# Soltanilara/av-aloha

Measured on AMD Instinct MI355X. Metric: env-steps/sec (whole node) at 4096 parallel envs, SlotInsertion-3Arms, higher is better.
Workload: dtype f32

## Files before the change

av_aloha_amd/csrc/avsim_phys.hip.h:

```cpp
#pragma once
#include <hip/hip_runtime.h>

#include <cstddef>
#include <cstring>
#include <string>
#include <type_traits>
#include <vector>

#include "avsim_collide.hip.h"
#include "avsim_dev.h"
#include "avsim_math.hip.h"
#include "avsim_model.h"
#include "avsim_phys_layout.h"

namespace avs {

enum { J_FREE = 0, J_BALL = 1, J_SLIDE = 2, J_HINGE = 3 };
enum { R_EQ = 0, R_FLOSS = 1, R_LIMIT = 2, R_CONTACT = 3 };
constexpr int TREE_W = 8;
constexpr int ROW_W = 2 * TREE_W;
constexpr int ROW_S = ROW_W;
constexpr int CAND_MAX = 256;
constexpr int PROF_W = 26;
constexpr int NEAR_MAX = 512;

#define AVSIM_HEAD_INTS(X)                                                                                                              \
    X(nq) X(nv) X(nu) X(nbody) X(njnt) X(ngeom) X(npair) X(ntree) X(neq) X(nfloss) X(nlimited) X(nment) X(task_id) X(nj) X(msize)        \
    X(noslip_iters) X(noslip_trees) X(qcqp_tridiag) X(newton_early_exit) X(newton_component) X(noslip_per_tree) X(solver) X(newton_iters) \
    X(ls_iterations)
#define AVSIM_BODY_INTS(X) X(nobj) X(hull_ovf)
template <typename real>
struct DevHead {
    int nq, nv, nu, nbody, njnt, ngeom, npair, ntree, neq, nfloss, nlimited, nment, task_id, nj, msize;
    real timestep, gravity[3], impratio, grip_lo, grip_hi;
    int noslip_iters;
    int noslip_trees;
    int qcqp_tridiag;
    int newton_early_exit;
    int newton_component;
    int noslip_per_tree;
    int solver, newton_iters;
    real newton_tol, nscale;
    real ls_tolerance;
    int ls_iterations;
};
template <typename real, typename SPEC>
struct FixedHead {
    int pad_dims_[15];
    real timestep, gravity[3], impratio, grip_lo, grip_hi;
    int pad_flags_[8];
    real newton_tol, nscale;
    real ls_tolerance;
    int pad_tail_;
#define AVS_FIXED_INT(x) static constexpr int x = SPEC::x;
    AVSIM_HEAD_INTS(AVS_FIXED_INT)
#undef AVS_FIXED_INT
};
template <typename real, typename HEAD>
struct DevModelT : HEAD {
    GLB_PTR(const int) body_parent;
    GLB_PTR(const int) body_jntadr;
    GLB_PTR(const int) body_jntnum;
    GLB_PTR(const int) body_dofadr;
    GLB_PTR(const int) body_dofnum;
    GLB_PTR(const int) body_tree;
    GLB_PTR(const int) body_dofmask;
    GLB_PTR(const int) body_last;
    GLB_PTR(const real) body_pos;
    GLB_PTR(const real) body_quat;
    GLB_PTR(const real) body_mass;
    GLB_PTR(const real) body_ipos;
    GLB_PTR(const real) body_inertia;
    GLB_PTR(const real) body_invweight0;
    GLB_PTR(const real) static_xpos;
    GLB_PTR(const real) static_xmat;
    GLB_PTR(const int) tree_bodyadr;
    GLB_PTR(const int) tree_bodylist;
    GLB_PTR(const int) tree_dofadr;
    GLB_PTR(const int) tree_dofnum;
    GLB_PTR(const int) tree_madr;
    GLB_PTR(const int) jnt_type;
    GLB_PTR(const int) jnt_qposadr;
    GLB_PTR(const int) jnt_dofadr;
    GLB_PTR(const int) jnt_actfrclimited;
    GLB_PTR(const int) limited_jnt;
    GLB_PTR(const real) jnt_pos;
    GLB_PTR(const real) jnt_axis;
    GLB_PTR(const real) jnt_range;
    GLB_PTR(const real) jnt_actfrcrange;
    GLB_PTR(const real) jnt_solref;
    GLB_PTR(const real) jnt_solimp;
    GLB_PTR(const real) jnt_margin;
    GLB_PTR(const int) dof_body;
    GLB_PTR(const int) dof_parent;
    GLB_PTR(const int) dof_tree;
    GLB_PTR(const int) dof_jnt;
    GLB_PTR(const int) floss_dof;
    GLB_PTR(const int) ment_i;
    GLB_PTR(const int) ment_j;
    GLB_PTR(const real) dof_armature;
    GLB_PTR(const real) dof_damping;
    GLB_PTR(const real) dof_frictionloss;
    GLB_PTR(const real) dof_invweight0;
    GLB_PTR(const real) dof_solref;
    GLB_PTR(const real) dof_solimp;
    GLB_PTR(const int) act_dof;
    GLB_PTR(const int) act_qposadr;
    GLB_PTR(const int) act_ctrllimited;
    GLB_PTR(const real) act_kp;
    GLB_PTR(const real) act_kv;
    GLB_PTR(const real) act_gear;
    GLB_PTR(const real) act_ctrlrange;
    GLB_PTR(const int) eq_dof1;
    GLB_PTR(const int) eq_dof2;
    GLB_PTR(const int) eq_qpos1;
    GLB_PTR(const int) eq_qpos2;
    GLB_PTR(const real) eq_polycoef;
    GLB_PTR(const real) eq_solref;
    GLB_PTR(const real) eq_solimp;
    GLB_PTR(const real) qpos0;
    GLB_PTR(const real) qpos_home;
    int nobj;
    GLB_PTR(const int) obj_qadr;
    const double* obj_reset;
    GLB_PTR(const int) geom_type;
    GLB_PTR(const int) geom_body;
    GLB_PTR(const int) geom_hull;
    GLB_PTR(const int) geom_class;
    GLB_PTR(const int) geom_static;
    GLB_PTR(const real) geom_pos;
    GLB_PTR(const real) geom_mat;
    GLB_PTR(const real) geom_size;
    GLB_PTR(const real) geom_cpos;
    GLB_PTR(const real) geom_rbound;
    GLB_PTR(const real) geom_xpos0;
    GLB_PTR(const real) geom_xmat0;
    GLB_PTR(const real) geom_cen0;
    GLB_PTR(const real) geom_aabb0;
    GLB_PTR(const real) geom_lbox;
    GLB_PTR(const real) hull_vert;
    int hull_ovf;
    GLB_PTR(const int) pair_geom;
    GLB_PTR(const int) pair_condim;
    GLB_PTR(const real) pair_friction;
    GLB_PTR(const real) pair_solref;
    GLB_PTR(const real) pair_solimp;
    GLB_PTR(const real) pair_margin;
    GLB_PTR(const real) pair_gap;
    real* rJ_glob;
    real* rB_glob;
    real* gA_glob;
    int* near_glob;
    int* cand_glob;
    real* gref_glob;
    real* bxo_glob;
    GLB_PTR(const int) obs_qposadr;
    GLB_PTR(const real) obs_offset;
    GLB_PTR(const real) obs_scale;
};

template <typename real> using DevModel = DevModelT<real, DevHead<real>>;

static_assert(NARROW_SCR_W == 64 * SLOT_W + 4 * 56, "avsim_phys_layout.h: narrow-phase scratch");

template <typename real>
struct KArgs {
    DevModel<real> m;
    Layout lay;
    MOff mo;
};
template <typename real>
using KPtr = const KArgs<real> __attribute__((address_space(4)))*;

struct GenericSpec {};
template <typename SPEC> constexpr bool spec_fixed = !std::is_same<SPEC, GenericSpec>::value;
template <typename real, typename SPEC>
struct KFixed {
    using Model = DevModelT<real, FixedHead<real, SPEC>>;
    using FH = FixedHead<real, SPEC>;
    using DH = DevHead<real>;
    static_assert(sizeof(FH) == sizeof(DH) && alignof(FH) == alignof(DH) && sizeof(Model) == sizeof(DevModel<real>) && offsetof(FH, timestep) == offsetof(DH, timestep) &&
                      offsetof(FH, newton_tol) == offsetof(DH, newton_tol) && offsetof(FH, pad_tail_) == offsetof(DH, ls_iterations),
                  "FixedHead: the words of DevHead");
    KPtr<real> p;
    struct View {
        const Model __attribute__((address_space(4)))& m;
        static constexpr Layout lay = SPEC::lay;
        static constexpr MOff mo = SPEC::mo;
        AVS_DEV const View* operator->() const { return this; }
    };
    AVS_DEV KFixed(KPtr<real> p_) : p(p_) {}
    AVS_DEV explicit KFixed(unsigned long long v) : p((KPtr<real>)v) {}
    AVS_DEV explicit operator unsigned long long() const { return (unsigned long long)p; }
    AVS_DEV View operator->() const { return View{reinterpret_cast<const Model __attribute__((address_space(4)))&>(p->m)}; }
};
template <typename real, typename SPEC> struct KRefOf { using type = KFixed<real, SPEC>; };
template <typename real> struct KRefOf<real, GenericSpec> { using type = KPtr<real>; };
template <typename real, typename SPEC> using KRef = typename KRefOf<real, SPEC>::type;
#define PHASE_LAUNDER()                                                                                \
    do {                                                                                               \
        const unsigned long long p_ = (unsigned long long)ka;                                          \
        unsigned lo_ = __builtin_amdgcn_readfirstlane((unsigned)p_), hi_ = __builtin_amdgcn_readfirstlane((unsigned)(p_ >> 32)); \
        asm volatile("" : "+s"(lo_), "+s"(hi_));                                                       \
        ka = (decltype(ka))(((unsigned long long)hi_ << 32) | lo_);                                    \
    } while (0)
#if defined(__HIP_DEVICE_COMPILE__)
#define AVS_ASSUME_LDS(p) __builtin_assume(__builtin_amdgcn_is_shared((const void*)(p)))
#else
#define AVS_ASSUME_LDS(p) ((void)(p))
#endif
template <typename T>
AVS_DEV T* lds_at(unsigned byte_off) { return (T*)(__attribute__((address_space(3))) T*)(size_t)byte_off; }
#define LDS_BASES()                                                                       \
    real* const r = this->r; AVS_ASSUME_LDS(r);     \
    int* const ii = this->ii; AVS_ASSUME_LDS(ii);   \
    (void)r; (void)ii
#define PHASE_BEGIN() PHASE_LAUNDER(); LDS_BASES()



#ifndef AVS_SYNC_SCOPE
#define AVS_SYNC_SCOPE "workgroup"
#endif
#define GSYNC()                                              \
    do {                                                     \
        __builtin_amdgcn_fence(__ATOMIC_ACQ_REL, AVS_SYNC_SCOPE); \
        __builtin_amdgcn_wave_barrier();                     \
    } while (0)

AVS_DEV float row16_sum(float x) {
    asm volatile("" : "+v"(x));
    x += __builtin_bit_cast(float, __builtin_amdgcn_mov_dpp(__builtin_bit_cast(int, x), 0x128, 0xf, 0xf, true));
    x += __builtin_bit_cast(float, __builtin_amdgcn_mov_dpp(__builtin_bit_cast(int, x), 0x124, 0xf, 0xf, true));
    x += __builtin_bit_cast(float, __builtin_amdgcn_mov_dpp(__builtin_bit_cast(int, x), 0x122, 0xf, 0xf, true));
    x += __builtin_bit_cast(float, __builtin_amdgcn_mov_dpp(__builtin_bit_cast(int, x), 0x121, 0xf, 0xf, true));
    return x;
}
AVS_DEV double row16_sum(double x) {
    x += __shfl_xor(x, 8, 16);
    x += __shfl_xor(x, 4, 16);
    x += __shfl_xor(x, 2, 16);
    x += __shfl_xor(x, 1, 16);
    return x;
}

AVS_DEV float wave_sum(float x) {
    x = row16_sum(x);
    int xi = __builtin_bit_cast(int, x);
    x += __builtin_bit_cast(float, __builtin_amdgcn_update_dpp(0, xi, 0x142, 0xa, 0xf, false));
    xi = __builtin_bit_cast(int, x);
    x += __builtin_bit_cast(float, __builtin_amdgcn_update_dpp(0, xi, 0x143, 0xc, 0xf, false));
    return __builtin_bit_cast(float, __builtin_amdgcn_readlane(__builtin_bit_cast(int, x), 63));
}
AVS_DEV double wave_sum(double x) {
    for (int o = 32; o > 0; o >>= 1) x += __shfl_xor(x, o, 64);
    return x;
}

#define LDS_PTR(T) __attribute__((address_space(3))) T*

template <typename real>
struct RowS {
    real aref, R, inv, invn, lo, hi, f, muinv;
};

AVS_DEV float oct_sum(float x) {
    asm volatile("" : "+v"(x));
    x += __builtin_bit_cast(float, __builtin_amdgcn_mov_dpp(__builtin_bit_cast(int, x), 0xB1, 0xf, 0xf, true));
    x += __builtin_bit_cast(float, __builtin_amdgcn_mov_dpp(__builtin_bit_cast(int, x), 0x4E, 0xf, 0xf, true));
    x += __builtin_bit_cast(float, __builtin_amdgcn_mov_dpp(__builtin_bit_cast(int, x), 0x141, 0xf, 0xf, true));
    return x;
}
AVS_DEV double oct_sum(double x) {
    x += __shfl_xor(x, 1, 8);
    x += __shfl_xor(x, 2, 8);
    x += __shfl_xor(x, 4, 8);
    return x;
}
template <int J>
AVS_DEV int oct_bcast_i(int x) {
    constexpr int q = J & 3, ctrl = q | (q << 2) | (q << 4) | (q << 6);
    const int a = __builtin_amdgcn_mov_dpp(x, ctrl, 0xf, 0xf, true);
    const int b = __builtin_amdgcn_mov_dpp(a, 0x141, 0xf, 0xf, true);
    const bool hi = (threadIdx.x & 4) != 0;
    return hi == (J >= 4) ? a : b;
}
template <int J> AVS_DEV float oct_bcast(float x) { return __builtin_bit_cast(float, oct_bcast_i<J>(__builtin_bit_cast(int, x))); }
template <int J> AVS_DEV double oct_bcast(double x) {
    const long long b = __builtin_bit_cast(long long, x);
    const unsigned lo = (unsigned)oct_bcast_i<J>((int)(unsigned)b), hi = (unsigned)oct_bcast_i<J>((int)(unsigned)(b >> 32));
    return __builtin_bit_cast(double, ((long long)hi << 32) | (long long)lo);
}
template <typename T>
AVS_DEV T oct_bcast_n(T x, int j) {
    switch (j & 7) {
        case 0: return oct_bcast<0>(x); case 1: return oct_bcast<1>(x); case 2: return oct_bcast<2>(x); case 3: return oct_bcast<3>(x);
        case 4: return oct_bcast<4>(x); case 5: return oct_bcast<5>(x); case 6: return oct_bcast<6>(x); default: return oct_bcast<7>(x);
    }
}
AVS_DEV float lane_get(float x, int l) { return __builtin_bit_cast(float, __builtin_amdgcn_readlane(__builtin_bit_cast(int, x), l)); }
AVS_DEV double lane_get(double x, int l) {
    const long long b = __builtin_bit_cast(long long, x);
    const unsigned lo = (unsigned)__builtin_amdgcn_readlane((int)(unsigned)b, l), hi = (unsigned)__builtin_amdgcn_readlane((int)(unsigned)(b >> 32), l);
    return __builtin_bit_cast(double, ((long long)hi << 32) | (long long)lo);
}

constexpr int GRP_MAX = 6;
constexpr int GA_W = 64, GA_Q = 16, GA_QW = 6;
template <typename T> AVS_DEV T qdiv(T t, T d, T dinv) { return sizeof(T) == 4 ? t * dinv : t / d; }
AVS_DEV float qrsqrt(float x) { return __builtin_amdgcn_rsqf(x); }
AVS_DEV double qrsqrt(double x) { return 1.0 / sqrt(x); }
template <typename T> struct QTol;
template <> struct QTol<double> { static constexpr double abs = 1e-10, rel = 0.0; };
template <> struct QTol<float> { static constexpr float abs = 1e-10f, rel = 2e-6f; };

template <bool B> struct BoolTag { static constexpr bool value = B; };

template <typename real>
struct NoslipLead {
    LDS_PTR(const real) Minv;
    LDS_PTR(const int) tadr;
    LDS_PTR(const int) tnum;
    LDS_PTR(const int) floss_dof;
    LDS_PTR(int) dmap;
    LDS_PTR(int) prof;
    int tridiag;
    int ntree, nv, neq, nfloss, nlg;
};

typedef int nl_v4 __attribute__((ext_vector_type(4)));
#define NL_PARAMS nl_v4 nl_a_, nl_v4 nl_b_, nl_v4 nl_c_
#define NL_ARGS(nl) nl_pack_a(nl), nl_pack_b(nl), nl_pack_c(nl)
#define NL_UNPACK(real) NoslipLead<real> nl = nl_unpack<real>(nl_a_, nl_b_, nl_c_)
template <typename real> AVS_DEV nl_v4 nl_pack_a(const NoslipLead<real>& n) {
    return nl_v4{(int)(__SIZE_TYPE__)n.Minv, (int)(__SIZE_TYPE__)n.tadr, (int)(__SIZE_TYPE__)n.tnum, (int)(__SIZE_TYPE__)n.floss_dof};
}
template <typename real> AVS_DEV nl_v4 nl_pack_b(const NoslipLead<real>& n) { return nl_v4{(int)(__SIZE_TYPE__)n.dmap, (int)(__SIZE_TYPE__)n.prof, n.tridiag, n.ntree}; }
template <typename real> AVS_DEV nl_v4 nl_pack_c(const NoslipLead<real>& n) { return nl_v4{n.nv, n.neq, n.nfloss, n.nlg}; }
template <typename real> AVS_DEV NoslipLead<real> nl_unpack(nl_v4 a, nl_v4 b, nl_v4 c) {
    NoslipLead<real> n;
    n.Minv = (LDS_PTR(const real))(__SIZE_TYPE__)(unsigned)a.x; n.tadr = (LDS_PTR(const int))(__SIZE_TYPE__)(unsigned)a.y; n.tnum = (LDS_PTR(const int))(__SIZE_TYPE__)(unsigned)a.z;
    n.floss_dof = (LDS_PTR(const int))(__SIZE_TYPE__)(unsigned)a.w; n.dmap = (LDS_PTR(int))(__SIZE_TYPE__)(unsigned)b.x; n.prof = (LDS_PTR(int))(__SIZE_TYPE__)(unsigned)b.y;
    n.tridiag = b.z; n.ntree = b.w; n.nv = c.x; n.neq = c.y; n.nfloss = c.z; n.nlg = c.w;
    return n;
}

template <typename T> AVS_DEV LDS_PTR(T) uni_lds(LDS_PTR(T) p) {
    return (LDS_PTR(T))(unsigned long long)(unsigned)__builtin_amdgcn_readfirstlane((int)(unsigned)(unsigned long long)p);
}
template <typename T> AVS_DEV GLB_PTR(T) uni_glb(GLB_PTR(T) p) {
    const unsigned long long v = (unsigned long long)p;
    return (GLB_PTR(T))(((unsigned long long)(unsigned)__builtin_amdgcn_readfirstlane((int)(unsigned)(v >> 32)) << 32) | (unsigned)__builtin_amdgcn_readfirstlane((int)(unsigned)v));
}

template <typename T> AVS_DEV T secular_step(T val, T r2, T r, T yw) {
    const T yy = val + r2, ny = sqrt(yy);
    return val * yy / ((ny + r) * r * yw);
}

template <typename real>
__device__ AVS_OUTLINE_2 void pgs_groups(LDS_PTR(real) rowS, LDS_PTR(const int) rowI, GLB_PTR(const real) rJ, GLB_PTR(const real) rB,
                                                     LDS_PTR(real) q, LDS_PTR(const int) gI, GLB_PTR(const real) gA, int ngrp, int iters,
                                                     int noslip_iters, real noslip_tol_scaled, NL_PARAMS) {
    NL_UNPACK(real);
    const long long tent = __builtin_readcyclecounter();
    rowS = uni_lds(rowS); rowI = uni_lds(rowI); q = uni_lds(q); gI = uni_lds(gI);
    rJ = uni_glb(rJ); rB = uni_glb(rB); gA = uni_glb(gA);
    ngrp = __builtin_amdgcn_readfirstlane(ngrp); iters = __builtin_amdgcn_readfirstlane(iters); noslip_iters = __builtin_amdgcn_readfirstlane(noslip_iters);
    noslip_tol_scaled = lane_get(noslip_tol_scaled, 0);
    nl.Minv = uni_lds(nl.Minv); nl.tadr = uni_lds(nl.tadr); nl.tnum = uni_lds(nl.tnum); nl.floss_dof = uni_lds(nl.floss_dof); nl.dmap = uni_lds(nl.dmap); nl.prof = uni_lds(nl.prof);
    nl.ntree = __builtin_amdgcn_readfirstlane(nl.ntree); nl.nv = __builtin_amdgcn_readfirstlane(nl.nv); nl.neq = __builtin_amdgcn_readfirstlane(nl.neq);
    nl.nfloss = __builtin_amdgcn_readfirstlane(nl.nfloss); nl.nlg = __builtin_amdgcn_readfirstlane(nl.nlg); nl.tridiag = __builtin_amdgcn_readfirstlane(nl.tridiag);
    const int lane = threadIdx.x & 63, d = lane >> 3, k8 = lane & 7, dr = d < GRP_MAX ? d : 0;
    const int lr = lane < GRP_MAX ? lane : 0;
    const int tri = lr * (lr - 1) / 2;
    if (ngrp <= 0) return;
    const bool fl = noslip_iters > 0 && nl.nlg >= 0;
    const int ft = lane >> 3, fi = lane & 7, fgb = lane & ~7;
    bool fm = false;
    int fdof = 0, frow = -1;
    real mrow[TREE_W], faref = 0, finv = 0, fdiag = 0, flo = 0, fhi = 0;
#pragma unroll
    for (int s = 0; s < TREE_W; s++) mrow[s] = 0;
    if (fl) {
        for (int k = lane; k < nl.nv; k += 64) nl.dmap[k] = -1;
        __builtin_amdgcn_fence(__ATOMIC_ACQ_REL, "wavefront");
        __builtin_amdgcn_wave_barrier();
        for (int r = lane; r < nl.nfloss; r += 64) nl.dmap[nl.floss_dof[r]] = nl.neq + r;
        __builtin_amdgcn_fence(__ATOMIC_ACQ_REL, "wavefront");
        __builtin_amdgcn_wave_barrier();
        fm = ft < nl.ntree && fi < nl.tnum[ft < nl.ntree ? ft : 0];
        fdof = fm ? nl.tadr[ft] + fi : 0;
        frow = fm ? nl.dmap[fdof] : -1;
        if (fm) {
#pragma unroll
            for (int s = 0; s < TREE_W; s++) mrow[s] = nl.Minv[64 * ft + 8 * fi + s];
        }
        LDS_PTR(const real) FS = rowS + RS_S * (frow >= 0 ? frow : 0);
        faref = FS[0]; finv = frow >= 0 ? FS[3] : real(0); flo = FS[4]; fhi = FS[5];
        fdiag = finv != 0 ? real(1) / finv : real(0);
    }
    real imp = 0, imp_c = 0;
#ifdef AVSIM_PROBE_ROWS
    LDS_PTR(int) prof = (LDS_PTR(int))nullptr;
#else
    LDS_PTR(int) prof = nl.prof;
#endif
    const long long tq0 = prof ? __builtin_readcyclecounter() : 0;
    int nstep = 0, nsweep = 0;
    auto floss_sweep = [&]() {
        const long long tf0 = prof ? __builtin_readcyclecounter() : 0;
        real x = fm ? q[fdof] : real(0);
        LDS_PTR(real) FS = rowS + RS_S * (frow >= 0 ? frow : 0);
        real f = frow >= 0 ? FS[6] : real(0);
#pragma unroll
        for (int s = 0; s < TREE_W; s++) {
            const real res = x - faref;
            const real fs = tmin(tmax(f - res * finv, flo), fhi);
            const real dl_ = fs - f, ch = dl_ * (real(0.5) * dl_ * fdiag + res);
            const bool take = frow >= 0 && fi == s && !(ch > real(1e-10));
            if (take) { imp -= ch; f = fs; }
            const real ds = oct_bcast_n(take ? dl_ : real(0), s);
            x += mrow[s] * ds;
        }
        if (fm) q[fdof] = x;
        if (frow >= 0) FS[6] = f;
        __builtin_amdgcn_fence(__ATOMIC_ACQ_REL, "wavefront");
        __builtin_amdgcn_wave_barrier();
        nsweep++;
    };
    const int first_ns = fl ? nl.nlg : 0;
    const int per_ns = ngrp - first_ns;
    const int noslip_only = (fl && per_ns <= 0) ? noslip_iters : 0;
    if (noslip_only) noslip_iters = 0;
    auto jb_load = [&](int hdr, int win, real& ja, real& jb, real& ba, real& bb) {
        const int st = hdr & 0xffff, cn = (hdr >> 16) & 15;
        const bool in = d < cn;
        const int rw = st + (in ? d : 0);
        const bool a = in && k8 < ((win >> 6) & 15), b = in && k8 < ((win >> 19) & 15);
        GLB_PTR(const real) Jr = rJ + ROW_S * rw + k8;
        GLB_PTR(const real) Br = rB + ROW_S * rw + k8;
        (void)a; (void)b;
        const bool packed = ((hdr >> 24) & 1) && ((__builtin_amdgcn_readfirstlane(win) >> 19) & 15) == 0;
        ja = Jr[0];
        const real x = Jr[TREE_W];
        if (packed) { jb = 0; ba = x; bb = 0; }
        else { jb = x; ba = Br[0]; bb = Br[TREE_W]; }
    };
    auto nextg = [&](int gq, int itq) { return gq + 1 < ngrp ? gq + 1 : (itq + 1 >= iters ? first_ns : 0); };
    int g = iters > 0 ? 0 : first_ns, it = 0;
    if (g >= ngrp) g = 0;
    int gi = __builtin_amdgcn_readfirstlane(gI[g]);
    int gin = __builtin_amdgcn_readfirstlane(gI[nextg(g, it)]);
    int ginn = __builtin_amdgcn_readfirstlane(gI[nextg(nextg(g, it), it)]);
    int ra = rowI[(gi & 0xffff) + dr], ran = rowI[(gin & 0xffff) + dr];
    real JA, JB, BA, BB;
    jb_load(gi, ra, JA, JB, BA, BB);
    real ac[GRP_MAX - 1];
#pragma unroll
    for (int s = 0; s < GRP_MAX - 1; s++) ac[s] = gA[GA_W * g + tri + s];
    const int qr = (lane >= 1 && lane <= 5) ? lane - 1 : 0;
    real qc[GA_QW], qn[GA_QW];
#pragma unroll
    for (int s = 0; s < GA_QW; s++) qc[s] = gA[GA_W * g + GA_Q + 8 * s + qr];
    const int total = iters * ngrp + noslip_iters * per_ns;
    __builtin_amdgcn_s_waitcnt(0x0f70);
    if (fl && iters == 0 && noslip_iters > 0) floss_sweep();
    for (int step = 0; step < total; step++) {
        nstep++;
        const bool noslip = it >= iters;
        const int start = gi & 0xffff, cnt = (gi >> 16) & 15;
        const bool contact = (gi >> 24) & 1;
        const int g1 = nextg(g, it), g2 = nextg(g1, it), g3 = nextg(g2, it);
        const int ginnn_v = gI[g3];
        const int rann = rowI[(ginn & 0xffff) + dr];
        real JAn, JBn, BAn, BBn;
        jb_load(gin, ran, JAn, JBn, BAn, BBn);
        const bool inr = d < cnt;
// ... 1117 lines not shown
            if (ab && !a_table) rw = 3;
            if (cd) rw = 4;
    }
    return rw;
}
#if !defined(AVSIM_TU_F64) && !defined(AVSIM_NO_F32_LAUNCH)
__global__ void k_reward_pairs(GLB_PTR(const int) geom_class, int ngeom, int task_id, const int* __restrict__ pairs, int n, int cap, int* __restrict__ latch, int* __restrict__ reward) {
    const int i = blockIdx.x * blockDim.x + threadIdx.x;
    if (i >= n) return;
    int f = 0;
    for (int c = 0; c < cap; c++) {
        const int g1 = pairs[((size_t)i * cap + c) * 2], g2 = pairs[((size_t)i * cap + c) * 2 + 1];
        if (g1 < 0 || g2 < 0 || g1 >= ngeom || g2 >= ngeom) continue;
        f |= reward_pair_flags(geom_class[g1], geom_class[g2], task_id);
    }
    int l = latch ? latch[i] : 0;
    reward[i] = reward_from_flags(f, task_id, &l);
    if (latch) latch[i] = l;
}
#endif


template <typename real, int G, typename SPEC = GenericSpec>
struct Env {
    KRef<real, SPEC> ka;
    int env = 0;
    int diverged = 0;
    int nit_sum = 0, nit_max = 0;
    bool profiling = false;
    real* r;
    int* ii;
    int lane, grp;
    const real* lr;
    const int* li;
    long long t_broad = 0, t_narrow = 0;
    __device__ Env(KRef<real, SPEC> ka_, real* r_, int* i_, int lane_, int grp_, const real* lr_, const int* li_)
        : ka(ka_), r(r_), ii(i_), lane(lane_), grp(grp_), lr(lr_), li(li_) {}
    AVS_DEV const int* LI() const {
        const int* p = li;
        if constexpr (spec_fixed<SPEC>) p = lds_at<const int>((unsigned)(ka->mo.nreal * sizeof(real)));
        AVS_ASSUME_LDS(p);
        return p;
    }
    AVS_DEV const real* LR() const {
        const real* p = lr;
        if constexpr (spec_fixed<SPEC>) p = lds_at<const real>(0u);
        AVS_ASSUME_LDS(p);
        return p;
    }
    AVS_DEV int nobj_() const { if constexpr (spec_fixed<SPEC>) return SPEC::nobj; else return ka->m.nobj; }
    AVS_DEV int hull_ovf_() const { if constexpr (spec_fixed<SPEC>) return SPEC::hull_ovf; else return ka->m.hull_ovf; }
    AVS_DEV GLB_PTR(real) rows_() const { return (GLB_PTR(real))ka->m.rJ_glob + (size_t)env * ka->lay.gefc * ROW_S; }
    AVS_DEV GLB_PTR(real) rowsB_() const { return (GLB_PTR(real))ka->m.rB_glob + (size_t)env * ka->lay.gefc * ROW_S; }
    AVS_DEV GLB_PTR(real) coup_() const { return (GLB_PTR(real))ka->m.gA_glob + (size_t)env * ka->lay.ggrp * GA_W; }
    AVS_DEV GLB_PTR(int) near_() const { return (GLB_PTR(int))ka->m.near_glob + (size_t)env * NEAR_MAX; }
    AVS_DEV GLB_PTR(int) cand_() const { return (GLB_PTR(int))ka->m.cand_glob + (size_t)env * CAND_MAX; }
    AVS_DEV GLB_PTR(real) bxo_() const { return (GLB_PTR(real))ka->m.bxo_glob + (size_t)env * 64 * BOX_OVF_W; }
    AVS_DEV GLB_PTR(real) gref_() const { return (GLB_PTR(real))ka->m.gref_glob + (size_t)env * ka->m.ngeom * 3; }
    AVS_DEV const int* body_parent_() const { return LI() + ka->mo.body_parent; }
    AVS_DEV const int* body_jntadr_() const { return LI() + ka->mo.body_jntadr; }
    AVS_DEV const int* body_jntnum_() const { return LI() + ka->mo.body_jntnum; }
    AVS_DEV const int* body_dofadr_() const { return LI() + ka->mo.body_dofadr; }
    AVS_DEV const int* body_dofnum_() const { return LI() + ka->mo.body_dofnum; }
    AVS_DEV const int* body_tree_() const { return LI() + ka->mo.body_tree; }
    AVS_DEV const int* body_dofmask_() const { return LI() + ka->mo.body_dofmask; }
    AVS_DEV const int* body_last_() const { return LI() + ka->mo.body_last; }
    AVS_DEV const int* tree_bodyadr_() const { return LI() + ka->mo.tree_bodyadr; }
    AVS_DEV const int* tree_bodylist_() const { return LI() + ka->mo.tree_bodylist; }
    AVS_DEV const int* tree_dofadr_() const { return LI() + ka->mo.tree_dofadr; }
    AVS_DEV const int* tree_dofnum_() const { return LI() + ka->mo.tree_dofnum; }
    AVS_DEV const int* tree_madr_() const { return LI() + ka->mo.tree_madr; }
    AVS_DEV const int* jnt_type_() const { return LI() + ka->mo.jnt_type; }
    AVS_DEV const int* jnt_qposadr_() const { return LI() + ka->mo.jnt_qposadr; }
    AVS_DEV const int* jnt_dofadr_() const { return LI() + ka->mo.jnt_dofadr; }
    AVS_DEV const int* jnt_actfrclimited_() const { return LI() + ka->mo.jnt_actfrclimited; }
    AVS_DEV const int* limited_jnt_() const { return LI() + ka->mo.limited_jnt; }
    AVS_DEV const int* dof_body_() const { return LI() + ka->mo.dof_body; }
    AVS_DEV const int* dof_parent_() const { return LI() + ka->mo.dof_parent; }
    AVS_DEV const int* dof_tree_() const { return LI() + ka->mo.dof_tree; }
    AVS_DEV const int* dof_jnt_() const { return LI() + ka->mo.dof_jnt; }
    AVS_DEV const int* floss_dof_() const { return LI() + ka->mo.floss_dof; }
    AVS_DEV const int* ment_i_() const { return LI() + ka->mo.ment_i; }
    AVS_DEV const int* ment_j_() const { return LI() + ka->mo.ment_j; }
    AVS_DEV const int* act_dof_() const { return LI() + ka->mo.act_dof; }
    AVS_DEV const int* act_qposadr_() const { return LI() + ka->mo.act_qposadr; }
    AVS_DEV const int* act_ctrllimited_() const { return LI() + ka->mo.act_ctrllimited; }
    AVS_DEV const int* geom_type_() const { return LI() + ka->mo.geom_type; }
    AVS_DEV const int* geom_body_() const { return LI() + ka->mo.geom_body; }
    AVS_DEV const int* geom_static_() const { return LI() + ka->mo.geom_static; }
    AVS_DEV const real* body_pos_() const { return LR() + ka->mo.body_pos; }
    AVS_DEV const real* body_quat_() const { return LR() + ka->mo.body_quat; }
    AVS_DEV const real* body_mass_() const { return LR() + ka->mo.body_mass; }
    AVS_DEV const real* body_ipos_() const { return LR() + ka->mo.body_ipos; }
    AVS_DEV const real* body_inertia_() const { return LR() + ka->mo.body_inertia; }
    AVS_DEV const real* body_invweight0_() const { return LR() + ka->mo.body_invweight0; }
    AVS_DEV const real* jnt_pos_() const { return LR() + ka->mo.jnt_pos; }
    AVS_DEV const real* jnt_axis_() const { return LR() + ka->mo.jnt_axis; }
    AVS_DEV const real* jnt_range_() const { return LR() + ka->mo.jnt_range; }
    AVS_DEV const real* jnt_actfrcrange_() const { return LR() + ka->mo.jnt_actfrcrange; }
    AVS_DEV const real* jnt_margin_() const { return LR() + ka->mo.jnt_margin; }
    AVS_DEV const real* dof_armature_() const { return LR() + ka->mo.dof_armature; }
    AVS_DEV const real* dof_damping_() const { return LR() + ka->mo.dof_damping; }
    AVS_DEV const real* dof_frictionloss_() const { return LR() + ka->mo.dof_frictionloss; }
    AVS_DEV const real* dof_invweight0_() const { return LR() + ka->mo.dof_invweight0; }
    AVS_DEV const real* act_kp_() const { return LR() + ka->mo.act_kp; }
    AVS_DEV const real* act_kv_() const { return LR() + ka->mo.act_kv; }
    AVS_DEV const real* act_gear_() const { return LR() + ka->mo.act_gear; }
    AVS_DEV const real* act_ctrlrange_() const { return LR() + ka->mo.act_ctrlrange; }
    AVS_DEV const real* geom_cpos_() const { return LR() + ka->mo.geom_cpos; }
    AVS_DEV const real* geom_rbound_() const { return LR() + ka->mo.geom_rbound; }


    __device__ void tree_chol(const real* A, real* Ldst, const real* diag_add, real diag_scale) {
        const int t = lane >> 3, i = lane & 7, gb = lane & ~7;
        const bool act = t < ka->m.ntree;
        const int n = act ? tree_dofnum_()[t] : 0, base = act ? tree_madr_()[t] : 0, a0 = act ? tree_dofadr_()[t] : 0;
        real row[TREE_W];
#pragma unroll
        for (int k = 0; k < TREE_W; k++) row[k] = (i < n && k <= i) ? A[base + i * n + k] : (k == i ? real(1) : real(0));
        if (diag_add && i < n) {
#pragma unroll
            for (int k = 0; k < TREE_W; k++) if (k == i) row[k] += diag_scale * diag_add[a0 + i];
        }
#pragma unroll
        for (int j = 0; j < TREE_W; j++) {
            const real d = sqrt(tmax(oct_bcast_n(row[j], j), real(1e-30)));
            const real lij = i == j ? d : row[j] / d;
            row[j] = lij;
            const real mul = i > j ? lij : real(0);
#pragma unroll
            for (int k = j + 1; k < TREE_W; k++) row[k] -= mul * oct_bcast_n(lij, k);
        }
        if (i < n) {
#pragma unroll
            for (int k = 0; k < TREE_W; k++) if (k <= i) Ldst[base + i * n + k] = row[k];
        }
    }
    __device__ real tree_solve(const real* L, real x) {
        const int t = lane >> 3, i = lane & 7, gb = lane & ~7;
        const bool act = t < ka->m.ntree;
        const int n = act ? tree_dofnum_()[t] : 0, base = act ? tree_madr_()[t] : 0;
        real row[TREE_W], col[TREE_W];
#pragma unroll
        for (int k = 0; k < TREE_W; k++) {
            row[k] = (i < n && k < i) ? L[base + i * n + k] : real(0);
            col[k] = (k < n && k > i) ? L[base + k * n + i] : real(0);
        }
        const real dinv = i < n ? real(1) / L[base + i * n + i] : real(1);
        if (!(i < n)) x = 0;
#pragma unroll
        for (int j = 0; j < TREE_W; j++) {
            const real yj = oct_bcast_n(x * dinv, j);
            x = i == j ? yj : x - row[j] * yj;
        }
#pragma unroll
        for (int j = TREE_W - 1; j >= 0; j--) {
            const real xj = oct_bcast_n(x * dinv, j);
            x = i == j ? xj : x - col[j] * xj;
        }
        return x;
    }

    __device__ void kinematics() {
        PHASE_BEGIN();
        real *xpos = r + ka->lay.xpos, *xmat = r + ka->lay.xmat, *xipos = r + ka->lay.xipos, *cdof = r + ka->lay.cdof, *qpos = r + ka->lay.qpos;
        int* anc = ii + ka->lay.cand;
        const int nb = ka->m.nbody;
        for (int b = lane; b < nb; b += G) {
            real R[9], pos[3];
            int a = -1;
            if (body_tree_()[b] < 0) {
                for (int k = 0; k < 3; k++) pos[k] = ka->m.static_xpos[3 * b + k];
                for (int k = 0; k < 9; k++) R[k] = ka->m.static_xmat[9 * b + k];
            } else {
                const int p = body_parent_()[b], ja = body_jntadr_()[b], jn = body_jntnum_()[b];
                const int jt = jn > 0 ? jnt_type_()[ja] : -1;
                if (jt == J_FREE) {
                    const int qa = jnt_qposadr_()[ja];
                    real quat[4];
                    for (int k = 0; k < 3; k++) pos[k] = qpos[qa + k];
                    for (int k = 0; k < 4; k++) quat[k] = qpos[qa + 3 + k];
                    quatnorm(quat);
                    quat2mat(quat, R);
                } else {
                    real Rl[9], bq[4] = {body_quat_()[4 * b], body_quat_()[4 * b + 1], body_quat_()[4 * b + 2], body_quat_()[4 * b + 3]};
                    quat2mat(bq, Rl);
                    for (int k = 0; k < 3; k++) pos[k] = body_pos_()[3 * b + k];
                    for (int k = 0; k < 9; k++) R[k] = Rl[k];
                    if (jt == J_HINGE) {
                        const real q = qpos[jnt_qposadr_()[ja]];
                        const real ax[3] = {jnt_axis_()[3 * ja], jnt_axis_()[3 * ja + 1], jnt_axis_()[3 * ja + 2]};
                        const real jp[3] = {jnt_pos_()[3 * ja], jnt_pos_()[3 * ja + 1], jnt_pos_()[3 * ja + 2]};
                        const real sn = sin(q), co = cos(q), oc = 1 - co;
                        const real Rq[9] = {co + ax[0] * ax[0] * oc, ax[0] * ax[1] * oc - ax[2] * sn, ax[0] * ax[2] * oc + ax[1] * sn,
                                            ax[1] * ax[0] * oc + ax[2] * sn, co + ax[1] * ax[1] * oc, ax[1] * ax[2] * oc - ax[0] * sn,
                                            ax[2] * ax[0] * oc - ax[1] * sn, ax[2] * ax[1] * oc + ax[0] * sn, co + ax[2] * ax[2] * oc};
                        for (int i = 0; i < 3; i++)
                            for (int j = 0; j < 3; j++) R[3 * i + j] = Rl[3 * i] * Rq[j] + Rl[3 * i + 1] * Rq[3 + j] + Rl[3 * i + 2] * Rq[6 + j];
                        real t0[3], t1[3];
                        mulmat(Rl, jp, t0);
                        mulmat(R, jp, t1);
                        for (int k = 0; k < 3; k++) pos[k] += t0[k] - t1[k];
                    } else if (jt == J_SLIDE) {
                        const real q = qpos[jnt_qposadr_()[ja]];
                        const real ax[3] = {jnt_axis_()[3 * ja], jnt_axis_()[3 * ja + 1], jnt_axis_()[3 * ja + 2]};
                        real t0[3];
                        mulmat(Rl, ax, t0);
                        for (int k = 0; k < 3; k++) pos[k] += t0[k] * q;
                    }
                    if (body_tree_()[p] < 0) {
                        GLB_PTR(const real) Rp = ka->m.static_xmat + 9 * p;
                        real Rn[9], t0[3];
                        for (int i = 0; i < 3; i++)
                            for (int j = 0; j < 3; j++) Rn[3 * i + j] = Rp[3 * i] * R[j] + Rp[3 * i + 1] * R[3 + j] + Rp[3 * i + 2] * R[6 + j];
                        mulmat(Rp, pos, t0);
                        for (int k = 0; k < 3; k++) pos[k] = ka->m.static_xpos[3 * p + k] + t0[k];
                        for (int k = 0; k < 9; k++) R[k] = Rn[k];
                    } else a = p;
                }
            }
            for (int k = 0; k < 3; k++) xpos[3 * b + k] = pos[k];
            for (int k = 0; k < 9; k++) xmat[9 * b + k] = R[k];
            anc[b] = a;
        }
        GSYNC();
        for (int round = 0; round < 6; round++) {
            bool any = false;
            real Ra[9], pa[3];
            int a = -1, aa = -1;
            const int b = lane;
            if (b < nb) {
                a = anc[b];
                if (a >= 0) {
                    any = true;
                    aa = anc[a];
                    for (int k = 0; k < 9; k++) Ra[k] = xmat[9 * a + k];
                    for (int k = 0; k < 3; k++) pa[k] = xpos[3 * a + k];
                }
            }
            if (!__any(any)) break;
            GSYNC();
            if (a >= 0) {
                real R[9], pos[3], Rn[9], t0[3];
                for (int k = 0; k < 9; k++) R[k] = xmat[9 * b + k];
                for (int k = 0; k < 3; k++) pos[k] = xpos[3 * b + k];
                for (int i = 0; i < 3; i++)
                    for (int j = 0; j < 3; j++) Rn[3 * i + j] = Ra[3 * i] * R[j] + Ra[3 * i + 1] * R[3 + j] + Ra[3 * i + 2] * R[6 + j];
                mulmat(Ra, pos, t0);
                for (int k = 0; k < 3; k++) xpos[3 * b + k] = pa[k] + t0[k];
                for (int k = 0; k < 9; k++) xmat[9 * b + k] = Rn[k];
                anc[b] = aa;
            }
            GSYNC();
        }
        for (int b = lane; b < nb; b += G) {
            real t3[3] = {0, 0, 0};
            if (body_tree_()[b] >= 0) {
                const real ip[3] = {body_ipos_()[3 * b], body_ipos_()[3 * b + 1], body_ipos_()[3 * b + 2]};
                mulmat(xmat + 9 * b, ip, t3);
                for (int k = 0; k < 3; k++) t3[k] += xpos[3 * b + k];
            }
            for (int k = 0; k < 3; k++) xipos[3 * b + k] = t3[k];
        }
        for (int d = lane; d < ka->m.nv; d += G) {
            const int j = dof_jnt_()[d], b = dof_body_()[d], jt = jnt_type_()[j], k = d - jnt_dofadr_()[j];
            const real *R = xmat + 9 * b, *pos = xpos + 3 * b;
            real cd[6] = {0, 0, 0, 0, 0, 0};
            if (jt == J_FREE) {
                if (k < 3) cd[3 + k] = 1;
                else {
                    const real w[3] = {R[k - 3], R[3 + k - 3], R[6 + k - 3]};
                    real c[3];
                    cross3(pos, w, c);
                    for (int q = 0; q < 3; q++) { cd[q] = w[q]; cd[3 + q] = c[q]; }
                }
            } else {
                const real ax[3] = {jnt_axis_()[3 * j], jnt_axis_()[3 * j + 1], jnt_axis_()[3 * j + 2]};
                real axis[3];
                mulmat(R, ax, axis);
                if (jt == J_HINGE) {
                    const real jp[3] = {jnt_pos_()[3 * j], jnt_pos_()[3 * j + 1], jnt_pos_()[3 * j + 2]};
                    real anchor[3], c[3];
                    mulmat(R, jp, anchor);
                    for (int q = 0; q < 3; q++) anchor[q] += pos[q];
                    cross3(anchor, axis, c);
                    for (int q = 0; q < 3; q++) { cd[q] = axis[q]; cd[3 + q] = c[q]; }
                } else {
                    for (int q = 0; q < 3; q++) cd[3 + q] = axis[q];
                }
            }
            for (int q = 0; q < 6; q++) cdof[6 * d + q] = cd[q];
        }
        real* gcen = r + ka->lay.gcen;
        for (int g = lane; g < ka->m.ngeom; g += G) {
            if (geom_static_()[g]) continue;
            int b = geom_body_()[g];
            real c[3] = {geom_cpos_()[3 * g], geom_cpos_()[3 * g + 1], geom_cpos_()[3 * g + 2]}, t3[3];
            mulmat(xmat + 9 * b, c, t3);
            for (int k = 0; k < 3; k++) gcen[3 * g + k] = xpos[3 * b + k] + t3[k];
        }
        GSYNC();
    }

    __device__ void crb() {
        PHASE_BEGIN();
        real *xmat = r + ka->lay.xmat, *xipos = r + ka->lay.xipos, *cdof = r + ka->lay.cdof, *ci = r + ka->lay.cinert, *M = r + ka->lay.M, *L = r + ka->lay.L;
        for (int b = lane; b < ka->m.nbody; b += G) {
            SInert<real> s;
            if (body_tree_()[b] >= 0) body_inertia(ka, xmat, xipos, b, s);
            else { s.m = 0; for (int k = 0; k < 3; k++) s.h[k] = 0; for (int k = 0; k < 6; k++) s.I[k] = 0; }
            real *o = ci + 10 * b, *ob = r + ka->lay.binert + 10 * b;
            o[0] = ob[0] = s.m;
            for (int k = 0; k < 3; k++) o[1 + k] = ob[1 + k] = s.h[k];
            for (int k = 0; k < 6; k++) o[4 + k] = ob[4 + k] = s.I[k];
        }
        for (int i = lane; i < ka->m.msize; i += G) M[i] = 0;
        GSYNC();
        {
            real acc[10];
            const int p = lane < ka->m.nbody ? lane : 0;
            const bool dyn = lane < ka->m.nbody && body_tree_()[p] >= 0;
            for (int k = 0; k < 10; k++) acc[k] = 0;
            if (dyn)
                for (int d = p; d <= body_last_()[p]; d++)
                    for (int k = 0; k < 10; k++) acc[k] += ci[10 * d + k];
            GSYNC();
            if (dyn)
                for (int k = 0; k < 10; k++) ci[10 * p + k] = acc[k];
        }
        GSYNC();
        for (int e = lane; e < ka->m.nment; e += G) {
            int i = ment_i_()[e], j = ment_j_()[e], t = dof_tree_()[i], n = tree_dofnum_()[t], a = tree_dofadr_()[t];
            real f[6];
            inert_mul(ci + 10 * dof_body_()[i], cdof + 6 * i, f);
            real v = 0;
            for (int k = 0; k < 6; k++) v += cdof[6 * j + k] * f[k];
            if (i == j) v += dof_armature_()[i];
            real* Mb = M + tree_madr_()[t];
            Mb[(i - a) * n + (j - a)] = v;
            Mb[(j - a) * n + (i - a)] = v;
        }
        GSYNC();
        tree_chol(M, L, (const real*)nullptr, real(0));
        GSYNC();
        real* Minv = r + ka->lay.Minv;
        for (int w = lane; w < ka->m.ntree * TREE_W; w += G) {
            int t = w >> 3, j = w & 7, n = tree_dofnum_()[t];
            real x[TREE_W];
            const real* Lt = L + tree_madr_()[t];
#pragma unroll
            for (int k = 0; k < TREE_W; k++) x[k] = (k == j && j < n) ? real(1) : real(0);
#pragma unroll
            for (int i = 0; i < TREE_W; i++)
                if (i < n) {
                    real sacc = x[i];
#pragma unroll
                    for (int k = 0; k < i; k++) sacc -= Lt[i * n + k] * x[k];
                    x[i] = sacc / Lt[i * n + i];
                }
#pragma unroll
            for (int i = TREE_W - 1; i >= 0; i--)
                if (i < n) {
                    real sacc = x[i];
#pragma unroll
                    for (int k = i + 1; k < TREE_W; k++) if (k < n) sacc -= Lt[k * n + i] * x[k];
                    x[i] = sacc / Lt[i * n + i];
                }
#pragma unroll
            for (int k = 0; k < TREE_W; k++) Minv[64 * t + 8 * k + j] = (k < n && j < n) ? x[k] : real(0);
        }
        GSYNC();
    }

    __device__ void rne_bias() {
        PHASE_BEGIN();
        real *xmat = r + ka->lay.xmat, *xipos = r + ka->lay.xipos, *cdof = r + ka->lay.cdof, *qvel = r + ka->lay.qvel;
        real *cvel = r + ka->lay.cvel, *cfrc = r + ka->lay.cfrc, *bias = r + ka->lay.bias;
        real* cdd = r + ka->lay.cinert;
        const int nb = ka->m.nbody;
        for (int b = lane; b < nb; b += G) {
            real v[6] = {0, 0, 0, 0, 0, 0};
            const int t = body_tree_()[b];
            if (t >= 0) {
                const int a0 = tree_dofadr_()[t], n = tree_dofnum_()[t], mask = body_dofmask_()[b];
#pragma unroll
                for (int k = 0; k < TREE_W; k++) {
                    const bool on = k < n && ((mask >> k) & 1);
                    const int d = on ? a0 + k : a0;
                    const real qd = on ? qvel[d] : real(0);
#pragma unroll
                    for (int q = 0; q < 6; q++) v[q] += cdof[6 * d + q] * qd;
                }
            }
            for (int q = 0; q < 6; q++) cvel[6 * b + q] = v[q];
        }
        GSYNC();
        for (int d = lane; d < ka->m.nv; d += G) {
            const int j = dof_jnt_()[d], b = dof_body_()[d];
            real o[6] = {0, 0, 0, 0, 0, 0};
            if (jnt_type_()[j] == J_FREE) {
                const int d0 = jnt_dofadr_()[j];
                if (d - d0 >= 3) {
                    real vt[6] = {0, 0, 0, 0, 0, 0};
                    for (int k = 0; k < 3; k++)
                        for (int q = 0; q < 6; q++) vt[q] += cdof[6 * (d0 + k) + q] * qvel[d0 + k];
                    cross_motion(vt, cdof + 6 * d, o);
                }
            } else {
                cross_motion(cvel + 6 * b, cdof + 6 * d, o);
            }
            const real qd = qvel[d];
            for (int q = 0; q < 6; q++) cdd[6 * d + q] = o[q] * qd;
        }
        GSYNC();
        for (int b = lane; b < nb; b += G) {
            const int t = body_tree_()[b];
            real f[6] = {0, 0, 0, 0, 0, 0};
            if (t >= 0) {
                real a[6] = {0, 0, 0, -ka->m.gravity[0], -ka->m.gravity[1], -ka->m.gravity[2]}, v[6];
                const int a0 = tree_dofadr_()[t], n = tree_dofnum_()[t], mask = body_dofmask_()[b];
#pragma unroll
                for (int k = 0; k < TREE_W; k++) {
                    const bool on = k < n && ((mask >> k) & 1);
                    const int d = on ? a0 + k : a0;
#pragma unroll
                    for (int q = 0; q < 6; q++) { const real c = cdd[6 * d + q]; a[q] += on ? c : real(0); }
                }
                for (int q = 0; q < 6; q++) v[q] = cvel[6 * b + q];
                real sv[10];
                for (int q = 0; q < 10; q++) sv[q] = (r + ka->lay.binert)[10 * b + q];
                real Ia[6], Iv[6], vIv[6];
                inert_mul(sv, a, Ia);
                inert_mul(sv, v, Iv);
                cross_force(v, Iv, vIv);
                for (int q = 0; q < 6; q++) f[q] = Ia[q] + vIv[q];
            }
            for (int q = 0; q < 6; q++) cfrc[6 * b + q] = f[q];
        }
        GSYNC();
        for (int i = lane; i < ka->m.nv; i += G) {
            const int b = dof_body_()[i];
            real f[6] = {0, 0, 0, 0, 0, 0};
            for (int d = b; d <= body_last_()[b]; d++)
                for (int q = 0; q < 6; q++) f[q] += cfrc[6 * d + q];
            real sacc = 0;
            for (int q = 0; q < 6; q++) sacc += cdof[6 * i + q] * f[q];
            bias[i] = sacc;
        }
        GSYNC();
    }

    __device__ void smooth() {
        PHASE_BEGIN();
        real *qpos = r + ka->lay.qpos, *qvel = r + ka->lay.qvel, *ctrl = r + ka->lay.ctrl, *bias = r + ka->lay.bias, *fsm = r + ka->lay.fsm, *as = r + ka->lay.asm_;
        real* act = r + ka->lay.fcon;
        for (int i = lane; i < ka->m.nv; i += G) act[i] = 0;
        GSYNC();
        for (int u = lane; u < ka->m.nu; u += G) {
            real c = ctrl[u];
            if (act_ctrllimited_()[u]) c = tclamp(c, act_ctrlrange_()[2 * u], act_ctrlrange_()[2 * u + 1]);
            int dof = act_dof_()[u];
            real f = act_kp_()[u] * c - act_kp_()[u] * qpos[act_qposadr_()[u]] - act_kv_()[u] * qvel[dof];
            act[dof] += act_gear_()[u] * f;
        }
        GSYNC();
        for (int i = lane; i < ka->m.nv; i += G) {
            int j = dof_jnt_()[i];
            real a = act[i];
            if (jnt_actfrclimited_()[j] && jnt_type_()[j] != J_FREE) a = tclamp(a, jnt_actfrcrange_()[2 * j], jnt_actfrcrange_()[2 * j + 1]);
            real f = -dof_damping_()[i] * qvel[i] - bias[i] + a;
            fsm[i] = f;
            as[i] = f;
        }
        GSYNC();
        {
            const int t = lane >> 3, i = lane & 7;
            const bool mine = t < ka->m.ntree && i < tree_dofnum_()[t];
            const int k = mine ? tree_dofadr_()[t] + i : 0;
            const real x = tree_solve(r + ka->lay.L, mine ? as[k] : real(0));
            GSYNC();
            if (mine) as[k] = x;
        }
        GSYNC();
    }

    __device__ void load_shape(int g, Shape<real>& s) {
        LDS_BASES();
        real *xpos = r + ka->lay.xpos, *xmat = r + ka->lay.xmat, *gcen = r + ka->lay.gcen;
        s.type = geom_type_()[g];
        for (int k = 0; k < 3; k++) s.size[k] = ka->m.geom_size[3 * g + k];
        s.hull = ka->m.hull_vert;
        s.hbase = ka->m.geom_hull[2 * g];
        s.hR = ka->m.geom_hull[2 * g + 1];
        s.hovf = hull_ovf_();
        s.nh = 0;
        for (int k = 0; k < 3; k++) { s.lc[k] = ka->m.geom_lbox[6 * g + k]; s.lh[k] = ka->m.geom_lbox[6 * g + 3 + k]; }
        if (geom_static_()[g]) {
            for (int k = 0; k < 3; k++) { s.pos[k] = ka->m.geom_xpos0[3 * g + k]; s.center[k] = ka->m.geom_cen0[3 * g + k]; }
            for (int k = 0; k < 9; k++) s.mat[k] = ka->m.geom_xmat0[9 * g + k];
        } else {
            int b = geom_body_()[g];
            real gp[3] = {ka->m.geom_pos[3 * g], ka->m.geom_pos[3 * g + 1], ka->m.geom_pos[3 * g + 2]}, t3[3];
            mulmat(xmat + 9 * b, gp, t3);
            for (int k = 0; k < 3; k++) { s.pos[k] = xpos[3 * b + k] + t3[k]; s.center[k] = gcen[3 * g + k]; }
            const real* Rb = xmat + 9 * b;
            GLB_PTR(const real) Rg = ka->m.geom_mat + 9 * g;
            for (int i = 0; i < 3; i++)
                for (int j = 0; j < 3; j++) s.mat[3 * i + j] = Rb[3 * i] * Rg[j] + Rb[3 * i + 1] * Rg[3 + j] + Rb[3 * i + 2] * Rg[6 + j];
        }
    }

    __device__ AVS_OUTLINE_0 static void multi_perturb(KRef<real, SPEC> ka_, real* r_, int* i_, int lane_, int grp_, const real* lr_, const int* li_, int env_,
                                                                   int pga, int pgb, int src, int pert) {
        Env e(ka_, r_, i_, lane_, grp_, lr_, li_);
        e.env = env_;
        LDS_PTR(real) os = (LDS_PTR(real))(e.r + e.ka->lay.scr + SLOT_W * src);
        const real p0[3] = {os[SLOT_P], os[SLOT_P + 1], os[SLOT_P + 2]}, n0[3] = {os[SLOT_N], os[SLOT_N + 1], os[SLOT_N + 2]};
        Shape<real> a, b;
        e.load_shape(pga, a);
        e.load_shape(pgb, b);
        real dk = real(1e30), pk[3] = {0, 0, 0};
        if (!mpr_perturbed(a, b, p0, n0, pert, &dk, pk)) dk = real(1e30);
        os[1 + pert] = dk;
        for (int c = 0; c < 3; c++) os[SLOT_P + 3 * (1 + pert) + c] = pk[c];
    }

    __device__ AVS_OUTLINE void collide() {
        Env e(*this);
        e.collide_i();
        diverged = e.diverged; nit_sum = e.nit_sum; nit_max = e.nit_max; t_broad = e.t_broad; t_narrow = e.t_narrow;
    }
    __device__ __attribute__((always_inline)) void collide_i() {
        PHASE_BEGIN();
        real* gcen = r + ka->lay.gcen;
        int* misc = ii + ka->lay.misc;
        GLB_PTR(int) cand = cand_();
        int ncand = 0;
        long long tb0 = __builtin_readcyclecounter();
        const real skin = real(0.03);
        GLB_PTR(real) gref = gref_();
        GLB_PTR(int) nearl = near_();
        auto pair_hit = [&](int p, real pad) -> bool {
            int g1 = ka->m.pair_geom[2 * p], g2 = ka->m.pair_geom[2 * p + 1];
            bool s1 = geom_static_()[g1], s2 = geom_static_()[g2];
            real mg = ka->m.pair_margin[p] + pad;
            if (s1 || s2) {
                int gs = s1 ? g1 : g2, gd = s1 ? g2 : g1;
                real rd = geom_rbound_()[gd] + mg, d2 = 0;
                for (int k = 0; k < 3; k++) {
                    real c = gcen[3 * gd + k], lo = ka->m.geom_aabb0[6 * gs + k], hi = ka->m.geom_aabb0[6 * gs + 3 + k];
                    real e = c < lo ? lo - c : (c > hi ? c - hi : real(0));
                    d2 += e * e;
                }
                return !(d2 > rd * rd);
            }
            real d[3], rr = geom_rbound_()[g1] + geom_rbound_()[g2] + mg;
            sub3(gcen + 3 * g2, gcen + 3 * g1, d);
            return !(dot3(d, d) > rr * rr);
        };
        bool moved = false;
        if (misc[7]) {
            for (int g = lane; g < ka->m.ngeom; g += G)
                if (!geom_static_()[g]) {
                    const real d[3] = {gcen[3 * g] - gref[3 * g], gcen[3 * g + 1] - gref[3 * g + 1], gcen[3 * g + 2] - gref[3 * g + 2]};
                    moved |= dot3(d, d) > real(0.25) * skin * skin;
                }
        }
        bool rebuild = !misc[7] || __any(moved);
        int nnear = misc[6];
        if (rebuild) {
            nnear = 0;
#pragma unroll 1
            for (int base = 0; base < ka->m.npair; base += G) {
                int p = base + lane;
                bool hit = p < ka->m.npair && pair_hit(p, skin);
                int tot, rk = group_rank<G>(hit, grp, lane, &tot);
                if (hit && nnear + rk < NEAR_MAX) nearl[nnear + rk] = p;
                nnear += tot;
            }
            for (int i = lane; i < 3 * ka->m.ngeom; i += G) gref[i] = gcen[i];
            if (lane == 0) { misc[6] = nnear < NEAR_MAX ? nnear : NEAR_MAX; misc[7] = nnear <= NEAR_MAX; if (nnear > NEAR_MAX) misc[2] |= 8; }
            GSYNC();
        }
        if (nnear <= NEAR_MAX) {
            for (int base = 0; base < nnear; base += G) {
                int i = base + lane, p = i < nnear ? nearl[i] : 0;
                bool hit = i < nnear && pair_hit(p, real(0));
                int tot, rk = group_rank<G>(hit, grp, lane, &tot);
                if (hit && ncand + rk < CAND_MAX) cand[ncand + rk] = p;
                if (ncand + tot > CAND_MAX && lane == 0) misc[2] |= 4;
                ncand = ncand + tot < CAND_MAX ? ncand + tot : CAND_MAX;
            }
        } else {
#pragma unroll 1
            for (int base = 0; base < ka->m.npair; base += G) {
                int p = base + lane;
                bool hit = p < ka->m.npair && pair_hit(p, real(0));
                int tot, rk = group_rank<G>(hit, grp, lane, &tot);
                if (hit && ncand + rk < CAND_MAX) cand[ncand + rk] = p;
                if (ncand + tot > CAND_MAX && lane == 0) misc[2] |= 4;
                ncand = ncand + tot < CAND_MAX ? ncand + tot : CAND_MAX;
            }
        }
        if (lane == 0) misc[3] = ncand;
        GSYNC();
        long long tb1 = __builtin_readcyclecounter();
        t_broad += tb1 - tb0;
        real *cdist = r + ka->lay.cdist, *cpos = r + ka->lay.cpos, *cnrm = r + ka->lay.cnrm;
        int* cpair = ii + ka->lay.cpair;
        int ncon = 0, ovf = 0;
        int* mlist = ii + ka->lay.cand;
        GLB_PTR(real) bxo = bxo_();
        for (int base = 0; base < ncand; base += G) {
            const int ci = base + lane;
            int n = 0, p = 0, nn = 0;
            LDS_PTR(real) scr = (LDS_PTR(real))(r + ka->lay.scr + SLOT_W * lane);
            const bool valid = ci < ncand;
            if (valid) p = cand[ci];
            const int ga = ka->m.pair_geom[2 * p], gb = ka->m.pair_geom[2 * p + 1];
            const int tya = geom_type_()[ga], tyb = geom_type_()[gb];
            const bool isbox = valid && tya == G_BOX && tyb == G_BOX;
            const long long tn0_ = profiling ? __builtin_readcyclecounter() : 0;
            {
                bool boxlive = false;
                if (isbox) {
                    Shape<real> a, b;
                    load_shape(ga, a);
                    load_shape(gb, b);
                    boxlive = !boxes_separated(a, b);
                }
                int nbox, rk = group_rank<G>(boxlive, grp, lane, &nbox);
                const int row = lane >> 4;
                for (int b0 = 0; b0 < nbox; b0 += 4) {
                    int src = 0;
                    bool on = false;
#pragma unroll
                    for (int gg = 0; gg < 4; gg++) {
                        const unsigned long long mm = __ballot(boxlive && rk == b0 + gg);
                        if (row == gg && mm != 0) { src = __builtin_ctzll(mm); on = true; }
                    }
                    const int pga = __shfl(ga, src, 64), pgb = __shfl(gb, src, 64);
                    Shape<real> a, b;
                    load_shape(pga, a);
                    load_shape(pgb, b);
                    const int n16 = box_box16(a, b, (LDS_PTR(real))(r + ka->lay.scr + SLOT_W * src), (LDS_PTR(real))(r + ka->lay.scr + SLOT_W * G + 56 * row), bxo + BOX_OVF_W * src, lane, on);
                    __builtin_amdgcn_fence(__ATOMIC_ACQ_REL, "wavefront");
                    __builtin_amdgcn_wave_barrier();
                    const int got = __shfl(on ? n16 : 0, 16 * ((rk - b0) & 3), 64);
                    if (boxlive && rk >= b0 && rk < b0 + 4) nn = got;
                }
            }
            const long long tn1 = profiling ? __builtin_readcyclecounter() : 0;
            if (valid && !isbox) {
                Shape<real> a, b;
                load_shape(ga, a);
                load_shape(gb, b);
                nn = narrow(a, b, scr);
            }
            if (profiling) {
                const long long tn2 = __builtin_readcyclecounter();
                if (lane == 0) { (ii + ka->lay.nprof)[14] += (int)(tn1 - tn0_); (ii + ka->lay.nprof)[15] += (int)(tn2 - tn1); }
            }
            {
                const bool multi = valid && !isbox && nn == 1 && tya != G_SPHERE && tyb != G_SPHERE;
                int nm, mrk = group_rank<G>(multi, grp, lane, &nm);
                if (nm > 0) {
                    if (multi) mlist[mrk] = lane;
                    GSYNC();
                    for (int m0 = 0; m0 < nm; m0 += 16) {
                        const int q = m0 + (lane >> 2), pert = lane & 3;
                        const bool on = q < nm;
                        const int src = on ? mlist[q] : 0;
                        const int pga = __shfl(ga, src, 64), pgb = __shfl(gb, src, 64);
                        if (on) multi_perturb(ka, r, ii, lane, grp, lr, li, env, pga, pgb, src, pert);
                    }
                    GSYNC();
                    if (multi) {
                        const real rb1 = geom_rbound_()[ga], rb2 = geom_rbound_()[gb];
                        const real tol = MultiCcd<real>::reltol * (rb1 < rb2 ? rb1 : rb2);
                        int kept = 1;
                        for (int k = 1; k <= 4; k++) {
                            const real dk = scr[k];
                            const real pk[3] = {scr[SLOT_P + 3 * k], scr[SLOT_P + 3 * k + 1], scr[SLOT_P + 3 * k + 2]};
                            if (dk < real(1e29) && multiccd_distinct(pk, scr + SLOT_P, kept, tol)) {
                                scr[kept] = dk;
                                for (int c = 0; c < 3; c++) scr[SLOT_P + 3 * kept + c] = pk[c];
                                kept++;
                            }
                        }
                        nn = kept;
                    }
                }
            }
            int keepmask = 0;
            GLB_PTR(const real) ov = bxo + BOX_OVF_W * lane;
            if (valid) {
                real mg = ka->m.pair_margin[p];
                for (int k = 0; k < nn; k++)
                    if ((isbox && k >= BOX_SLOTC ? ov[4 * (k - BOX_SLOTC)] : scr[k]) < mg) { keepmask |= 1 << k; n++; }
            }
            int off = 0, tot = 0;
            for (int j = 1; j <= BOX_MAXC; j++) {
                int tj, rj = group_rank<G>(n >= j, grp, lane, &tj);
                if (tj == 0) break;
                off += rj;
                tot += tj;
            }
            int w = 0;
            for (int k = 0; k < BOX_MAXC; k++)
                if ((keepmask >> k) & 1) {
                    int c = ncon + off + w;
                    w++;
                    if (c < ka->lay.maxcon) {
                        const bool o = isbox && k >= BOX_SLOTC;
                        cdist[c] = o ? ov[4 * (k - BOX_SLOTC)] : scr[k];
                        cpair[c] = p;
                        for (int q = 0; q < 3; q++) { cpos[3 * c + q] = o ? ov[4 * (k - BOX_SLOTC) + 1 + q] : scr[SLOT_P + 3 * k + q]; cnrm[3 * c + q] = scr[SLOT_N + q]; }
                    }
                }
            if (ncon + tot > ka->lay.maxcon) ovf = 1;
            ncon = ncon + tot < ka->lay.maxcon ? ncon + tot : ka->lay.maxcon;
        }
        if (lane == 0) { misc[0] = ncon; misc[2] |= ovf; }
        GSYNC();
        t_narrow += __builtin_readcyclecounter() - tb1;
    }

#ifndef AVS_NO_SPLIT_PRE
    __device__ AVS_OUTLINE void pre_phases() {
        Env e(*this);
        e.kinematics(); e.crb(); e.rne_bias(); e.smooth();
    }
    __device__ AVS_OUTLINE void post_phases() {
        Env e(*this);
        e.euler(); e.check_divergence();
        diverged = e.diverged;
    }
#endif
    __device__ AVS_OUTLINE void make_constraints() {
        Env e(*this);
        e.make_constraints_i();
        diverged = e.diverged; nit_sum = e.nit_sum; nit_max = e.nit_max; t_broad = e.t_broad; t_narrow = e.t_narrow;
    }
    __device__ __attribute__((always_inline)) void make_constraints_i() {
        PHASE_BEGIN();
#ifdef AVSIM_PROBE_ROWS
        long long tpr_ = __builtin_readcyclecounter();
#define ROWPROBE(k) do { if (profiling) { const long long t_ = __builtin_readcyclecounter(); if (lane == 0) (ii + ka->lay.nprof)[8 + (k)] += (int)(t_ - tpr_); tpr_ = t_; } } while (0)
#else
#define ROWPROBE(k) ((void)0)
#endif
        real *qpos = r + ka->lay.qpos, *qvel = r + ka->lay.qvel;
        int *misc = ii + ka->lay.misc, *rmeta = ii + ka->lay.rmeta, *cpair = ii + ka->lay.cpair, *cefc = ii + ka->lay.cefc;
        real *cdist = r + ka->lay.cdist, *cpos = r + ka->lay.cpos, *cnrm = r + ka->lay.cnrm;
        int ncon = misc[0];
        int nefc = ka->m.neq + ka->m.nfloss;
        for (int i = lane; i < ka->m.neq; i += G) rmeta[i] = R_EQ | (i << 2);
        for (int i = lane; i < ka->m.nfloss; i += G) rmeta[ka->m.neq + i] = R_FLOSS | (i << 2);
        for (int base = 0; base < ka->m.nlimited; base += G) {
            int li = base + lane, lo = 0, hi = 0, j = 0;
            if (li < ka->m.nlimited) {
                j = limited_jnt_()[li];
                real q = qpos[jnt_qposadr_()[j]];
                lo = (q - jnt_range_()[2 * j]) < jnt_margin_()[j];
                hi = (jnt_range_()[2 * j + 1] - q) < jnt_margin_()[j];
            }
            int t1, t2, r1 = group_rank<G>(lo, grp, lane, &t1), r2 = group_rank<G>(hi, grp, lane, &t2);
            int pos = nefc + r1 + r2;
            if (lo && pos < ka->lay.maxefc) rmeta[pos] = R_LIMIT | (j << 2) | (0 << 12);
            if (hi && pos + lo < ka->lay.maxefc) rmeta[pos + lo] = R_LIMIT | (j << 2) | (1 << 12);
            nefc += t1 + t2;
        }
        int ovf = 0;
        if (nefc > ka->lay.maxefc) { nefc = ka->lay.maxefc; ovf = 1; }
        if (lane == 0) misc[4] = nefc;
        const int nlead0 = nefc;
        int cend = nefc;
        for (int base = 0; base < ncon; base += G) {
            int c = base + lane, dim = 0;
            if (c < ncon) {
                int p = cpair[c];
                if (cdist[c] < ka->m.pair_margin[p] - ka->m.pair_gap[p]) dim = ka->m.pair_condim[p];
            }
            int off = 0, tot = 0;
            for (int j = 1; j <= 6; j++) {
                int tj, rj = group_rank<G>(dim >= j, grp, lane, &tj);
                off += rj;
                tot += tj;
            }
            int myend = 0;
            if (c < ncon) {
                int first = nefc + off;
                if (dim > 0 && first + dim <= ka->lay.maxefc) {
                    cefc[c] = first | (dim << 16);
                    myend = first + dim;
                    for (int s = 0; s < dim; s++) rmeta[first + s] = R_CONTACT | (c << 2) | (s << 12) | (dim << 20);
                } else {
                    cefc[c] = -1;
                    if (dim > 0) ovf = 1;
                }
            }
            for (int o = 1; o < G; o <<= 1) { int x = __shfl_xor(myend, o, G); myend = x > myend ? x : myend; int y = __shfl_xor(ovf, o, G); ovf |= y; }
            cend = myend > cend ? myend : cend;
            nefc += tot;
        }
        nefc = cend;
        if (lane == 0) { misc[1] = nefc; if (ovf) misc[2] |= 2; }
        GSYNC();
        ROWPROBE(0);
        GLB_PTR(real) rJ = rows_();
        real *rowS = r + ka->lay.rowS, *warm = r + ka->lay.warm, *Minv = r + ka->lay.Minv, *asm_ = r + ka->lay.asm_;
        const bool newton = ka->m.solver == 1;
        const bool lead_slim = newton && lead_per_tree();
        int* rowI = ii + ka->lay.rowI;
        real* Lm = r + ka->lay.L;
        const int *bmask = body_dofmask_(), *tadr = tree_dofadr_(), *tnum = tree_dofnum_();
        const real* cdofp = r + ka->lay.cdof;
        const int nvm = ka->m.nv - 1;
        auto fill = [&](int i, auto lead_tag) {
            constexpr bool LEAD = decltype(lead_tag)::value;
            int meta = rmeta[i], type = meta & 3, id = (meta >> 2) & 1023, sub = (meta >> 12) & 255, dim = meta >> 20;
            real J[ROW_W];
#pragma unroll
            for (int k = 0; k < ROW_W; k++) J[k] = 0;
            int tA = -1, tB = -1;
            int j1 = -1, j2 = -1;
            real v1 = 0, v2 = 0;
            real pos = 0, margin = 0, diag0 = 0, floss = 0;
            real solref[2], solimp[5];
            bool valid = true;
            if (LEAD && type == R_EQ) {
                GLB_PTR(const real) c = ka->m.eq_polycoef + 5 * id;
                real q1 = qpos[ka->m.eq_qpos1[id]] - ka->m.qpos0[ka->m.eq_qpos1[id]], q2 = qpos[ka->m.eq_qpos2[id]] - ka->m.qpos0[ka->m.eq_qpos2[id]];
                real poly = c[0] + q2 * (c[1] + q2 * (c[2] + q2 * (c[3] + q2 * c[4])));
                real dpoly = c[1] + q2 * (2 * c[2] + q2 * (3 * c[3] + q2 * 4 * c[4]));
                int d1 = ka->m.eq_dof1[id], d2 = ka->m.eq_dof2[id];
                tA = dof_tree_()[d1];
                pos = q1 - poly;
                diag0 = dof_invweight0_()[d1] + dof_invweight0_()[d2];
                j1 = d1 - tree_dofadr_()[tA]; v1 = 1;
                j2 = d2 - tree_dofadr_()[tA]; v2 = -dpoly;
                for (int k = 0; k < 2; k++) solref[k] = ka->m.eq_solref[2 * id + k];
                for (int k = 0; k < 5; k++) solimp[k] = ka->m.eq_solimp[5 * id + k];
            } else if (LEAD && type == R_FLOSS) {
                int d = floss_dof_()[id];
                tA = dof_tree_()[d];
                diag0 = dof_invweight0_()[d];
                floss = dof_frictionloss_()[d];
                j1 = d - tree_dofadr_()[tA]; v1 = 1;
                for (int k = 0; k < 2; k++) solref[k] = ka->m.dof_solref[2 * d + k];
                for (int k = 0; k < 5; k++) solimp[k] = ka->m.dof_solimp[5 * d + k];
            } else if (LEAD && type == R_LIMIT) {
                int j = id, d = jnt_dofadr_()[j];
                real q = qpos[jnt_qposadr_()[j]];
                tA = dof_tree_()[d];
                pos = sub == 0 ? q - jnt_range_()[2 * j] : jnt_range_()[2 * j + 1] - q;
                margin = jnt_margin_()[j];
                diag0 = dof_invweight0_()[d];
                j1 = d - tree_dofadr_()[tA]; v1 = sub == 0 ? real(1) : real(-1);
                for (int k = 0; k < 2; k++) solref[k] = ka->m.jnt_solref[2 * j + k];
                for (int k = 0; k < 5; k++) solimp[k] = ka->m.jnt_solimp[5 * j + k];
            } else if (!LEAD) {
                int c = id, p = cpair[c];
                int g1 = ka->m.pair_geom[2 * p], g2 = ka->m.pair_geom[2 * p + 1], b1 = geom_body_()[g1], b2 = geom_body_()[g2];
                int t1 = body_tree_()[b1], t2 = body_tree_()[b2];
                tA = t1 >= 0 ? t1 : t2;
                tB = (t1 >= 0 && t2 >= 0 && t2 != t1) ? t2 : -1;
                real n[3] = {cnrm[3 * c], cnrm[3 * c + 1], cnrm[3 * c + 2]}, t1v[3], t2v[3], cp[3] = {cpos[3 * c], cpos[3 * c + 1], cpos[3 * c + 2]};
                make_frame(n, t1v, t2v);
                const int sm = sub % 3;
                real ax[3];
#pragma unroll
                for (int q = 0; q < 3; q++) ax[q] = sm == 0 ? n[q] : (sm == 1 ? t1v[q] : t2v[q]);
                const bool rot = sub >= 3;
                real cx[3], Wa[3], Wl[3];
                cross3(cp, ax, cx);
#pragma unroll
                for (int q = 0; q < 3; q++) { Wa[q] = rot ? ax[q] : cx[q]; Wl[q] = rot ? real(0) : ax[q]; }
                const int mA = (t1 == tA ? bmask[b1] : 0), pA = (t2 == tA ? bmask[b2] : 0);
                const int mB = (tB >= 0 && t1 == tB ? bmask[b1] : 0), pB = (tB >= 0 ? bmask[b2] : 0);
                const int aA = tadr[tA], aB = tadr[tB >= 0 ? tB : tA];
#pragma unroll
                for (int k = 0; k < TREE_W; k++) {
                    const real* ca = cdofp + 6 * (aA + k < nvm ? aA + k : nvm);
                    const real ea = Wa[0] * ca[0] + Wa[1] * ca[1] + Wa[2] * ca[2] + Wl[0] * ca[3] + Wl[1] * ca[4] + Wl[2] * ca[5];
                    J[k] = real(((pA >> k) & 1) - ((mA >> k) & 1)) * ea;
                }
                if (tB >= 0) {
#pragma unroll
                    for (int k = 0; k < TREE_W; k++) {
                        const real* cb = cdofp + 6 * (aB + k < nvm ? aB + k : nvm);
                        const real eb = Wa[0] * cb[0] + Wa[1] * cb[1] + Wa[2] * cb[2] + Wl[0] * cb[3] + Wl[1] * cb[4] + Wl[2] * cb[5];
                        J[TREE_W + k] = real(((pB >> k) & 1) - ((mB >> k) & 1)) * eb;
                    }
                }
                pos = sub == 0 ? cdist[c] : real(0);
                margin = ka->m.pair_margin[p] - ka->m.pair_gap[p];
                diag0 = body_invweight0_()[2 * b1] + body_invweight0_()[2 * b2];
                for (int k = 0; k < 2; k++) solref[k] = ka->m.pair_solref[2 * p + k];
                for (int k = 0; k < 5; k++) solimp[k] = ka->m.pair_solimp[5 * p + k];
            }
            (void)valid;
            const int j2c = j2 >= 0 ? j2 : (j1 >= 0 ? j1 : 0), j1c = j1 >= 0 ? j1 : 0;
            const real v2c = j2 >= 0 ? v2 : real(0);
            if (LEAD) {
#pragma unroll
                for (int k = 0; k < TREE_W; k++) J[k] += (k == j1 ? v1 : real(0)) + (k == j2 ? v2 : real(0));
            }
            real dmax = tclamp(solimp[1], real(0.0001), real(0.9999));
            real tc = tmax(solref[0], 2 * ka->m.timestep), dr = solref[1];
            real K = real(1) / tmax(real(1e-15), dmax * dmax * tc * tc * dr * dr), Bd = real(2) / tmax(real(1e-15), dmax * tc);
            real imp, R;
            const real imp_row = impedance(solimp, (!LEAD && sub > 0) ? cdist[id] : pos, margin);
            if (!LEAD && sub > 0) {
                int c = id, p = cpair[c];
                real imp0 = imp_row;
                real R0 = tmax(real(1e-15), (1 - imp0) * diag0 / imp0);
                real R1 = R0 / tmax(real(1e-15), ka->m.impratio);
                real mu0 = ka->m.pair_friction[5 * p], mur = ka->m.pair_friction[5 * p + sub - 1];
                R = sub == 1 ? R1 : R1 * mu0 * mu0 / tmax(real(1e-15), mur * mur);
                imp = imp0;
                K = 0;
                floss = mur;
            } else {
                imp = imp_row;
                R = tmax(real(1e-15), (1 - imp) * diag0 / imp);
            }
            real vel = 0;
            if (LEAD) {
                const int a0 = tadr[tA];
                vel = v1 * qvel[a0 + j1c] + v2c * qvel[a0 + j2c];
            } else {
                const int a0 = tadr[tA], b0 = tadr[tB >= 0 ? tB : tA];
#pragma unroll
                for (int k = 0; k < TREE_W; k++) vel += J[k] * qvel[a0 + k < nvm ? a0 + k : nvm];
                if (tB >= 0) {
#pragma unroll
                    for (int k = 0; k < TREE_W; k++) vel += J[TREE_W + k] * qvel[b0 + k < nvm ? b0 + k : nvm];
                }
            }
            const real aref = -Bd * vel - K * imp * (pos - margin);
            real dg = 0;
            real Bv[ROW_W];
            if (LEAD) {
                const real* Mi = Minv + 64 * tA;
                const real s1 = Mi[8 * j1c + j1c] * v1 + Mi[8 * j1c + j2c] * v2c, s2 = Mi[8 * j2c + j1c] * v1 + Mi[8 * j2c + j2c] * v2c;
                dg = v1 * s1 + v2c * s2;
                if (!lead_slim) {
#pragma unroll
                    for (int k = 0; k < TREE_W; k++) { Bv[k] = Mi[8 * k + j1c] * v1 + Mi[8 * k + j2c] * v2c; Bv[TREE_W + k] = 0; }
                }
            } else {
#pragma unroll
            for (int k = 0; k < TREE_W; k++) {
                real mr[TREE_W], sa = 0;
                lds_load8(Minv + 64 * tA + 8 * k, mr);
#pragma unroll
                for (int j = 0; j < TREE_W; j++) sa += mr[j] * J[j];
                dg += J[k] * sa;
                Bv[k] = sa;
                Bv[TREE_W + k] = 0;
            }
            if (tB >= 0) {
#pragma unroll
                for (int k = 0; k < TREE_W; k++) {
                    real mr[TREE_W], sb = 0;
                    lds_load8(Minv + 64 * tB + 8 * k, mr);
#pragma unroll
                    for (int j = 0; j < TREE_W; j++) sb += mr[j] * J[TREE_W + j];
                    dg += J[TREE_W + k] * sb;
                    Bv[TREE_W + k] = sb;
                }
            }
            }
            if (!LEAD && tB < 0) {
                real JB_[ROW_W];
#pragma unroll
                for (int k = 0; k < TREE_W; k++) { JB_[k] = J[k]; JB_[TREE_W + k] = Bv[k]; }
                store_row16(rJ + ROW_S * i, JB_);
            } else if (!LEAD || !lead_slim) {
                store_row16(rJ + ROW_S * i, J);
                store_row16(rowsB_() + ROW_S * i, Bv);
            }
            const int a0 = tadr[tA], nA = tnum[tA], b0 = tB >= 0 ? tadr[tB] : 0, nB = tB >= 0 ? tnum[tB] : 0;
            real jw = 0, jas = 0;
            if (LEAD) {
                jw = v1 * warm[a0 + j1c] + v2c * warm[a0 + j2c];
                jas = v1 * asm_[a0 + j1c] + v2c * asm_[a0 + j2c];
            } else {
#pragma unroll
            for (int k = 0; k < TREE_W; k++) {
                const int da = a0 + k < nvm ? a0 + k : nvm;
                jw += J[k] * warm[da];
                jas += J[k] * asm_[da];
            }
            if (tB >= 0) {
#pragma unroll
                for (int k = 0; k < TREE_W; k++) {
                    const int db = b0 + k < nvm ? b0 + k : nvm;
                    jw += J[TREE_W + k] * warm[db];
                    jas += J[TREE_W + k] * asm_[db];
                }
            }
            }
            const real big = real(1e30);
            real lo = -big, hi = big, muinv = 0;
            bool ns = false;
            if (LEAD && type == R_FLOSS) { lo = -floss; hi = floss; ns = true; }
            else if (LEAD && type == R_LIMIT) lo = 0;
            else if (!LEAD) {
                if (sub == 0) lo = 0;
                else { ns = true; muinv = real(1) / tmax(real(1e-15), floss); }
            }
            real f = -(jw - aref) / R;
            f = tmin(tmax(f, lo), hi);
            real* S = rowS + RS_S * i;
            S[0] = aref; S[1] = R; S[2] = newton ? jw - aref : real(1) / (dg + R); S[3] = ns ? real(1) / tmax(dg, real(1e-15)) : real(0);
            S[4] = lo; S[5] = hi; S[6] = f; S[7] = muinv; S[8] = jas - aref;
            const int lead_bits = !LEAD ? 0 : ((v1 < 0 ? 1 : 0) << 13) | (j1c << 26) | (j2c << 29);
            if (LEAD) S[7] = v2c;
            rowI[i] = a0 | (nA << 6) | (tA << 10) | ((b0 | (nB << 6) | ((tB >= 0 ? tB : 0) << 10)) << 13) | lead_bits;
            rmeta[i] = (meta & 0xfffff) | ((tA + 1) << 20) | ((tB + 1) << 24);
        };
        for (int i = lane; i < nlead0; i += G) fill(i, BoolTag<true>{});
        ROWPROBE(1);
        for (int i = nlead0 + lane; i < nefc; i += G) fill(i, BoolTag<false>{});
        GSYNC();
        ROWPROBE(2);
        int* gI = ii + ka->lay.gI;
        GLB_PTR(real) gA = coup_();
        const int nlead = misc[4];
        int ngrp = 0;
        for (int base = 0; base < nefc; base += G) {
            int i = base + lane;
// ... 87 lines not shown
                    for (int k = 0; k < j; k++) t -= L[i][k] * L[j][k];
                    L[i][j] = t / dd;
                }
            }
#pragma unroll
            for (int c = 0; c < 5; c++) {
                real x[5];
#pragma unroll
                for (int i = 0; i < 5; i++) { real t = (i == c) ? real(1) : real(0); for (int k = 0; k < i; k++) t -= L[i][k] * x[k]; x[i] = t / L[i][i]; }
#pragma unroll
                for (int i = 4; i >= 0; i--) { real t = x[i]; for (int k = i + 1; k < 5; k++) t -= L[k][i] * x[k]; x[i] = t / L[i][i]; }
#pragma unroll
                for (int i = 0; i < 5; i++) Inv[i][c] = x[i];
            }
#pragma unroll
            for (int j = 0; j < 5; j++) {
                GLB_PTR(real) o = gA + GA_W * g + GA_Q + j;
#pragma unroll
                for (int k = 0; k < 5; k++) o[8 * k] = mu[j] * Inv[j][k] * mu[k];
                o[40] = singular ? real(1) : real(0);
            }
        }
        GSYNC();
        ROWPROBE(5);
    }

    __device__ AVS_OUTLINE void solve(int pgs_iters, int solver, int newton_iters, real newton_tol, real scale) {
        Env e(*this);
        e.solve_i(pgs_iters, solver, newton_iters, newton_tol, scale);
        diverged = e.diverged; nit_sum = e.nit_sum; nit_max = e.nit_max; t_broad = e.t_broad; t_narrow = e.t_narrow;
    }
    __device__ __attribute__((always_inline)) void solve_i(int pgs_iters, int solver, int newton_iters, real newton_tol, real scale) {
        PHASE_BEGIN();
        if constexpr (spec_fixed<SPEC>) { solver = ka->m.solver; newton_iters = ka->m.newton_iters; }
        int *misc = ii + ka->lay.misc, *rmeta = ii + ka->lay.rmeta, *cefc = ii + ka->lay.cefc, *rowI = ii + ka->lay.rowI;
        real *qacc = r + ka->lay.qacc, *as = r + ka->lay.asm_, *rowS = r + ka->lay.rowS, *fcon = r + ka->lay.fcon;
        GLB_PTR(real) rJ = rows_();
        int nefc = misc[1], ncon = misc[0];
        real* Minv = r + ka->lay.Minv;
        if (solver == 1) {
            real* warm = r + ka->lay.warm;
            for (int k = lane; k < ka->m.nv; k += G) qacc[k] = warm[k];
            GSYNC();
            bool two_ = false;
            for (int i = lane; i < nefc; i += G) two_ = two_ || ((rowI[i] >> 19) & 15) != 0;
            const bool coupled = __any(two_) != 0 || ka->m.ntree > 8;
#define AVS_NEWTON_ARGS ka, (GLB_PTR(const real))rJ, (LDS_PTR(real))r, (LDS_PTR(int))ii, (LDS_PTR(const int))LI(), nefc, ncon, misc[4], newton_iters, newton_tol, scale, profiling ? 1 : 0
            int used = __builtin_amdgcn_readfirstlane(ncon) <= 64 ? (coupled ? newton_solve_coupled<real, 1>(AVS_NEWTON_ARGS) : newton_solve<real, 1, false>(AVS_NEWTON_ARGS))
                                                                  : (coupled ? newton_solve_coupled<real, 2>(AVS_NEWTON_ARGS) : newton_solve<real, 2, false>(AVS_NEWTON_ARGS));
#undef AVS_NEWTON_ARGS
            nit_sum += used; nit_max = used > nit_max ? used : nit_max;
            GSYNC();
            long long tn0 = profiling ? __builtin_readcyclecounter() : 0;
            int done_ = 0;
            if (ka->m.noslip_trees && lead_per_tree() && __builtin_amdgcn_readfirstlane(misc[8]) == 0)
                done_ = noslip_trees<real>((LDS_PTR(real))rowS, (LDS_PTR(const int))rowI, (LDS_PTR(const int))cefc, (GLB_PTR(const real))rJ, (LDS_PTR(real))qacc,
                                           (LDS_PTR(const int))(ii + ka->lay.gI), (GLB_PTR(const real))coup_(), ncon, nefc, ka->m.noslip_iters, real(1e-6) / ka->m.nscale, NL_ARGS(noslip_lead()));
            if (__builtin_amdgcn_readfirstlane(done_) == 2)
                done_ = noslip_trees2<real>((LDS_PTR(real))rowS, (LDS_PTR(const int))rowI, (LDS_PTR(const int))cefc, (GLB_PTR(const real))rJ, (GLB_PTR(const real))rowsB_(), (LDS_PTR(real))qacc,
                                            (LDS_PTR(const int))(ii + ka->lay.gI), (GLB_PTR(const real))coup_(), ncon, nefc, ka->m.noslip_iters, real(1e-6) / ka->m.nscale, NL_ARGS(noslip_lead()));
            if (__builtin_amdgcn_readfirstlane(done_) != 1 && lane == 0) misc[8] = 1;
            if (__builtin_amdgcn_readfirstlane(done_) != 1)
            pgs_groups<real>((LDS_PTR(real))rowS, (LDS_PTR(const int))rowI, (GLB_PTR(const real))rJ, (GLB_PTR(const real))rowsB_(), (LDS_PTR(real))qacc,
                             (LDS_PTR(const int))(ii + ka->lay.gI), (GLB_PTR(const real))coup_(), misc[5], 0, ka->m.noslip_iters, real(1e-6) / ka->m.nscale, NL_ARGS(noslip_lead()));
            if (profiling && lane == 0) (ii + ka->lay.nprof)[6] += (int)(__builtin_readcyclecounter() - tn0);
        } else {
        for (int c = lane; c < ncon; c += G) {
            int first = cefc[c];
            if (first < 0) continue;
            first &= 0xffff;
            int dim = ka->m.pair_condim[(ii + ka->lay.cpair)[c]];
            real fn = rowS[RS_S * first + 6], s2 = 0;
            for (int s = 1; s < dim; s++) { real t = rowS[RS_S * (first + s) + 6] * rowS[RS_S * (first + s) + 7]; s2 += t * t; }
            if (s2 > fn * fn) { real sc = fn / sqrt(s2); for (int s = 1; s < dim; s++) rowS[RS_S * (first + s) + 6] *= sc; }
        }
        GSYNC();
        jt_force(fcon, nefc);
        for (int k = lane; k < ka->m.nv; k += G) {
            int t = dof_tree_()[k], a0 = tree_dofadr_()[t], kk = k - a0, n = tree_dofnum_()[t];
            real s = as[k];
            for (int j = 0; j < n; j++) s += Minv[64 * t + 8 * kk + j] * fcon[a0 + j];
            qacc[k] = s;
        }
        GSYNC();
        static_assert(G == 64, "the solver maps one env to one wavefront");
        pgs_groups<real>((LDS_PTR(real))rowS, (LDS_PTR(const int))rowI, (GLB_PTR(const real))rJ, (GLB_PTR(const real))rowsB_(), (LDS_PTR(real))qacc,
                         (LDS_PTR(const int))(ii + ka->lay.gI), (GLB_PTR(const real))coup_(), misc[5], pgs_iters, ka->m.noslip_iters, real(1e-6) / ka->m.nscale, NL_ARGS(noslip_lead()));
        }
        GSYNC();
        jt_force(fcon, nefc);
    }

    AVS_DEV bool lead_per_tree() const { return ka->m.ntree <= 8 && ka->m.noslip_iters > 0 && ka->m.noslip_per_tree != 0; }
    AVS_DEV NoslipLead<real> noslip_lead() const {
        NoslipLead<real> nl;
        nl.Minv = (LDS_PTR(const real))(r + ka->lay.Minv);
        nl.tadr = (LDS_PTR(const int))tree_dofadr_(); nl.tnum = (LDS_PTR(const int))tree_dofnum_(); nl.floss_dof = (LDS_PTR(const int))floss_dof_();
        nl.dmap = (LDS_PTR(int))(r + ka->lay.ng);
        nl.ntree = ka->m.ntree; nl.nv = ka->m.nv; nl.neq = ka->m.neq; nl.nfloss = ka->m.nfloss; nl.tridiag = ka->m.qcqp_tridiag;
        nl.prof = profiling ? (LDS_PTR(int))(ii + ka->lay.nprof + 8) : (LDS_PTR(int))nullptr;
        nl.nlg = lead_per_tree() ? ((ii + ka->lay.misc)[4] + GRP_MAX - 1) / GRP_MAX : -1;
        return nl;
    }

    __device__ void check_divergence() {
        LDS_BASES();
        real *qpos = r + ka->lay.qpos, *qvel = r + ka->lay.qvel, *warm = r + ka->lay.warm;
        bool bad = false;
        for (int i = lane; i < ka->m.nq; i += G) bad |= !(fabs(qpos[i]) < real(1e6));
        for (int i = lane; i < ka->m.nv; i += G) bad |= !(fabs(qvel[i]) < real(1e6));
        if (!__any(bad)) return;
        diverged = 1;
        for (int i = lane; i < ka->m.nq; i += G) qpos[i] = ka->m.qpos_home[i];
        GSYNC();
        for (int i = lane; i < nobj_() * 7; i += G) qpos[ka->m.obj_qadr[i / 7] + i % 7] = (real)ka->m.obj_reset[((size_t)env * nobj_()) * 7 + i];
        for (int i = lane; i < ka->m.nv; i += G) { qvel[i] = 0; warm[i] = 0; }
        if (lane == 0) (ii + ka->lay.misc)[7] = 0;
        GSYNC();
    }

    __device__ __attribute__((always_inline)) void jt_force(real* out, int nefc) {
        LDS_BASES();
        AVS_ASSUME_LDS(out);
        (void)nefc;
        int* misc = ii + ka->lay.misc;
        for (int k = lane; k < ka->m.nv; k += G) out[k] = 0;
        GSYNC();
        rows_jt_force<real>((LDS_PTR(const real))(r + ka->lay.rowS), (LDS_PTR(const int))(ii + ka->lay.rowI), (LDS_PTR(const int))(ii + ka->lay.cefc),
                            (GLB_PTR(const real))rows_(), (LDS_PTR(real))out, misc[4], misc[0], lane, real(1));
        GSYNC();
    }

    __device__ void euler() {
        PHASE_BEGIN();
        real *qpos = r + ka->lay.qpos, *qvel = r + ka->lay.qvel, *warm = r + ka->lay.warm, *qacc = r + ka->lay.qacc, *fsm = r + ka->lay.fsm, *fcon = r + ka->lay.fcon;
        real *M = r + ka->lay.M, *L = r + ka->lay.L, *tmp = r + ka->lay.bias;
        real h = ka->m.timestep;
        for (int i = lane; i < ka->m.nv; i += G) { tmp[i] = fsm[i] + fcon[i]; warm[i] = qacc[i]; }
        GSYNC();
        tree_chol(M, L, dof_damping_(), h);
        GSYNC();
        {
            const int t = lane >> 3, i = lane & 7;
            const bool mine = t < ka->m.ntree && i < tree_dofnum_()[t];
            const int k = mine ? tree_dofadr_()[t] + i : 0;
            const real x = tree_solve(L, mine ? tmp[k] : real(0));
            if (mine) qvel[k] += h * x;
        }
        GSYNC();
        for (int j = lane; j < ka->m.njnt; j += G) {
            int qa = jnt_qposadr_()[j], da = jnt_dofadr_()[j];
            if (jnt_type_()[j] == J_FREE) {
                for (int k = 0; k < 3; k++) qpos[qa + k] += h * qvel[da + k];
                real q[4] = {qpos[qa + 3], qpos[qa + 4], qpos[qa + 5], qpos[qa + 6]}, w[3] = {qvel[da + 3], qvel[da + 4], qvel[da + 5]};
                real wn = sqrt(dot3(w, w)), ang = h * wn;
                if (ang > 0) {
                    real s = sin(ang / 2) / wn, qr[4] = {cos(ang / 2), s * w[0], s * w[1], s * w[2]};
                    quatmul(q, qr, q);
                }
                quatnorm(q);
                for (int k = 0; k < 4; k++) qpos[qa + 3 + k] = q[k];
            } else {
                qpos[qa] += h * qvel[da];
            }
        }
        GSYNC();
    }

    __device__ int reward(int* latch) {
        PHASE_BEGIN();
        int *misc = ii + ka->lay.misc, *cpair = ii + ka->lay.cpair;
        int ncon = misc[0];
        int f = 0;
        const int t = ka->m.task_id;
        for (int c = lane; c < ncon; c += G) {
            int p = cpair[c];
            f |= reward_pair_flags(ka->m.geom_class[ka->m.pair_geom[2 * p]], ka->m.geom_class[ka->m.pair_geom[2 * p + 1]], t);
        }
        for (int o = 1; o < G; o <<= 1) f |= __shfl_xor(f, o, G);
        return reward_from_flags(f, t, latch);
    }
};

#ifndef AVSIM_PHYS_MAXW
#define AVSIM_PHYS_MAXW 8
#endif
template <typename real, int G, int MAXW, bool RETRY, typename SPEC = GenericSpec>
#ifndef AVSIM_PHYS_ATTR
#ifdef AVSIM_TU_F64
#define AVSIM_PHYS_ATTR
#else
#define AVSIM_PHYS_ATTR __attribute__((amdgpu_waves_per_eu(2)))
#endif
#endif
__global__ void __launch_bounds__(64 * MAXW) AVSIM_PHYS_ATTR k_phys(KPtr<real> ka_small_, const real* __restrict__ img_real, const int* __restrict__ img_int, int N, int nsub, int pgs_iters, const float* __restrict__ action,
                                             int want_reward, real* __restrict__ g_qpos, real* __restrict__ g_qvel, real* __restrict__ g_ctrl,
                                             real* __restrict__ g_warm, int* __restrict__ g_latch, double* __restrict__ o_agent,
                                             int* __restrict__ o_reward, unsigned char* __restrict__ o_success, int* __restrict__ o_ncon,
                                             int* __restrict__ o_cpairs, double* __restrict__ o_cdist, int* __restrict__ o_diag, int max_reward, int export_contacts, long long* __restrict__ o_prof, float* __restrict__ o_xpose,
                                             const int* __restrict__ env_order, int* __restrict__ o_cost, int* __restrict__ work_head, int* __restrict__ work_next,
                                             int* __restrict__ retry, int retry_mode, KPtr<real> ka_big_) {
    const KRef<real, SPEC> ka_small(ka_small_), ka_big(ka_big_);
    extern __shared__ __attribute__((aligned(16))) unsigned char smem[];
    int nwork = N;
    const bool pass2 = RETRY && ((retry_mode & 7) == 2 || (retry_mode & 7) == 4);
    const bool pass1 = RETRY && ((retry_mode & 7) == 1 || (retry_mode & 7) == 3);
    if (pass2) {
        nwork = retry[(retry_mode & 7) == 4];
        if (blockIdx.x == 0 && threadIdx.x == 0) { *work_next = 0; retry[(retry_mode & 7) == 2] = 0; }
        if (nwork <= 0) return;
    }
    int* const bigflag = retry + 2 + N;
    const int cap1_con = pass2 ? (retry_mode >> 8) & 0x3ff : ka_small->lay.maxcon, cap1_efc = pass2 ? (retry_mode >> 18) & 0x3ff : ka_small->lay.maxefc;
    int* const pair_want = reinterpret_cast<int*>(smem + (size_t)(blockDim.x >> 6) * ka_small->lay.bytes_per_env + (size_t)ka_small->mo.nreal * sizeof(real) + (size_t)ka_small->mo.nint * 4);
    int* const pair_grant = pair_want + MAXW / 2;
    if (RETRY && threadIdx.x < MAXW / 2) { pair_want[threadIdx.x] = 0; pair_grant[threadIdx.x] = 0; }
    static_assert(G == 64, "one env per wavefront");
#ifdef AVSIM_NO_PROF
    o_prof = nullptr;
#endif
    const int wpb = blockDim.x >> 6;
    const int wave = threadIdx.x >> 6, lane = threadIdx.x & 63, grp = 0;
    constexpr bool FIXED = spec_fixed<SPEC>;
    static_assert(!(FIXED && RETRY), "the per-model kernels are one-pass");
    size_t rec0 = 0;
    if constexpr (FIXED) {
        rec0 = (((size_t)ka_small->mo.nreal * sizeof(real) + (size_t)ka_small->mo.nint * 4) + 15) & ~(size_t)15;
        if ((unsigned)(size_t)(LDS_PTR(unsigned char))smem != 0u) return;
    }
    real* lr = reinterpret_cast<real*>(smem + (FIXED ? (size_t)0 : (size_t)wpb * ka_small->lay.bytes_per_env));
    int* li = reinterpret_cast<int*>(lr + ka_small->mo.nreal);
    for (int i = threadIdx.x; i < ka_small->mo.nreal; i += blockDim.x) lr[i] = img_real[i];
    for (int i = threadIdx.x; i < ka_small->mo.nint; i += blockDim.x) li[i] = img_int[i];
    if (blockIdx.x == 0 && threadIdx.x == 0) *work_next = 0;
    __syncthreads();
    const int pr = wave >> 1;
    const bool paired = pass1 && (retry_mode & 8) && (wave | 1) < wpb;
    auto lds_get = [&](int* p) { int v = 0; if (lane == 0) v = __hip_atomic_load(p, __ATOMIC_ACQUIRE, __HIP_MEMORY_SCOPE_WORKGROUP); return __builtin_amdgcn_readfirstlane(v); };
    auto lds_put = [&](int* p, int v) { if (lane == 0) __hip_atomic_store(p, v, __ATOMIC_RELEASE, __HIP_MEMORY_SCOPE_WORKGROUP); };
    auto to_list = [&](int e) { if (lane == 0) retry[2 + atomicAdd(retry + ((retry_mode & 7) == 3), 1)] = e; };
    constexpr int PAIR_LEFT = -1;
    int claim_gen = 0, my_claim = 0;
    auto park = [&]() {
        for (;;) {
            const int w = lds_get(&pair_want[pr]);
            if (w == 0 || (w & 0xff) == wave + 1) break;
            lds_put(&pair_grant[pr], w);
            __builtin_amdgcn_s_sleep(32);
        }
    };
    auto claim = [&]() {
        int got = 0;
        const int c = (++claim_gen << 8) | (wave + 1);
        if (lane == 0) { int expect = 0; got = __hip_atomic_compare_exchange_strong(&pair_want[pr], &expect, c, __ATOMIC_ACQ_REL, __ATOMIC_ACQUIRE, __HIP_MEMORY_SCOPE_WORKGROUP) ? 1 : 0; }
        my_claim = c;
        return __builtin_amdgcn_readfirstlane(got) != 0;
    };
    int redo_env = -1;
  for (;;) {
    int env_ = 0;
    bool big = false;
    if (RETRY && redo_env >= 0) { env_ = redo_env; redo_env = -1; big = true; }
    else {
        if (RETRY && paired) park();
        int slot = 0;
        if (lane == 0) slot = atomicAdd(work_head, 1);
        slot = __builtin_amdgcn_readfirstlane(slot);
        if (slot >= nwork) break;
        env_ = env_order ? env_order[slot] : slot;
        if (RETRY && pass1 && (retry_mode & 8)) big = __builtin_amdgcn_readfirstlane(bigflag[env_]) != 0;
    }
    const int env = env_;
    if (RETRY && big) {
        bool mine = false;
        if (paired) mine = claim();
        if (!mine && paired) {
            for (int tries = 0; tries < 64 && !mine; tries++) {
                park();
                mine = claim();
            }
        }
        if (!mine) { to_list(env); continue; }
        int polls = 0;
        for (;; polls++) {
            const int g = lds_get(&pair_grant[pr]);
            if (g == my_claim || g == PAIR_LEFT || polls >= (1 << 15)) break;
            __builtin_amdgcn_s_sleep(32);
        }
        if (polls >= (1 << 15)) { lds_put(&pair_want[pr], 0); to_list(env); continue; }
    }
    KRef<real, SPEC> ka = (RETRY && big) ? ka_big : ka_small;
    const long long t_launch = __builtin_readcyclecounter();
    real* r = reinterpret_cast<real*>(smem + rec0 + (size_t)((RETRY && big) ? (wave & ~1) : wave) * ka_small->lay.bytes_per_env);
    int* ii = reinterpret_cast<int*>(r + ka->lay.nreal);
    bool beyond = false;
    Env<real, G, SPEC> E(ka, r, ii, lane, grp, lr, li);
    E.env = env;

    for (int i = lane; i < ka->m.nq; i += G) r[ka->lay.qpos + i] = g_qpos[(size_t)env * ka->m.nq + i];
    for (int i = lane; i < ka->m.nv; i += G) { r[ka->lay.qvel + i] = g_qvel[(size_t)env * ka->m.nv + i]; r[ka->lay.warm + i] = g_warm[(size_t)env * ka->m.nv + i]; }
    for (int i = lane; i < ka->m.nu; i += G) r[ka->lay.ctrl + i] = g_ctrl[(size_t)env * ka->m.nu + i];
    if (lane == 0) for (int k = 0; k < 8; k++) { ii[ka->lay.misc + k] = 0; ii[ka->lay.nprof + k] = 0; ii[ka->lay.nprof + 8 + k] = 0; }
    if (lane == 0) ii[ka->lay.misc + 8] = 0;
    E.profiling = o_prof != nullptr;
    GSYNC();
    if (action) {
        const float* a = action + (size_t)env * ka->m.nj;
        for (int i = lane; i < ka->m.nj; i += G) {
            real v = (real)a[i];
            if (i == 6 || i == 13) v = v * (ka->m.grip_hi - ka->m.grip_lo) + ka->m.grip_lo;
            r[ka->lay.ctrl + i] = v;
        }
        GSYNC();
    }
    long long tp[9] = {0, 0, 0, 0, 0, 0, 0, 0, 0};
#define PROF(k, stmt) do { if (o_prof) { long long t0_ = __builtin_readcyclecounter(); stmt; tp[k] += __builtin_readcyclecounter() - t0_; } else { stmt; } } while (0)
    for (int s = 0; s < nsub; s++) {
#ifndef AVS_NO_SPLIT_PRE
        PROF(0, E.pre_phases());
#else
        {
            Env<real, G, SPEC> e(E);
            PROF(0, e.kinematics());
            PROF(1, e.crb());
            PROF(2, e.rne_bias());
            PROF(3, e.smooth());
        }
#endif
        PROF(4, E.collide());
        PROF(5, E.make_constraints());
        if (RETRY) beyond = beyond || ii[ka->lay.misc + 0] > cap1_con || ii[ka->lay.misc + 1] > cap1_efc;
        PROF(6, E.solve(pgs_iters, ka->m.solver, ka->m.newton_iters, ka->m.newton_tol, ka->m.nscale));
#ifndef AVS_NO_SPLIT_PRE
        PROF(7, E.post_phases());
#else
        {
            Env<real, G, SPEC> e(E);
            PROF(7, e.euler());
            e.check_divergence();
            E.diverged = e.diverged;
        }
#endif
    }
    if (o_prof && lane == 0) {
        for (int k = 0; k < 8; k++) o_prof[(size_t)env * PROF_W + k] = tp[k];
        o_prof[(size_t)env * PROF_W + 8] = E.t_broad; o_prof[(size_t)env * PROF_W + 9] = E.t_narrow;
        for (int k = 0; k < 16; k++) o_prof[(size_t)env * PROF_W + 10 + k] = ii[ka->lay.nprof + k];
    }
    int nefc_last = ii[ka->lay.misc + 1];
    E.kinematics();
    if (o_xpose) {
        for (int b = lane; b < ka->m.nbody; b += G) {
            float* o = o_xpose + ((size_t)env * ka->m.nbody + b) * 12;
            for (int k = 0; k < 3; k++) o[k] = (float)r[ka->lay.xpos + 3 * b + k];
            for (int k = 0; k < 9; k++) o[3 + k] = (float)r[ka->lay.xmat + 9 * b + k];
        }
    }
    E.collide();
    if (RETRY && pass1 && !big && (ii[ka->lay.misc + 2] & 3)) {
        if (paired) redo_env = env; else to_list(env);
        GSYNC();
        continue;
    }
    if (RETRY) {
        beyond = beyond || ii[ka->lay.misc + 0] > cap1_con;
        if (lane == 0 && (big || pass2 || (retry_mode & 8))) bigflag[env] = beyond ? 1 : 0;
    }

    if (nsub > 0) {
        for (int i = lane; i < ka->m.nq; i += G) g_qpos[(size_t)env * ka->m.nq + i] = r[ka->lay.qpos + i];
        for (int i = lane; i < ka->m.nv; i += G) { g_qvel[(size_t)env * ka->m.nv + i] = r[ka->lay.qvel + i]; g_warm[(size_t)env * ka->m.nv + i] = r[ka->lay.warm + i]; }
    }
    if (action) for (int i = lane; i < ka->m.nu; i += G) g_ctrl[(size_t)env * ka->m.nu + i] = r[ka->lay.ctrl + i];
    if (o_agent)
        for (int i = lane; i < ka->m.nj; i += G) o_agent[(size_t)env * ka->m.nj + i] = ((double)r[ka->lay.qpos + ka->m.obs_qposadr[i]] - (double)ka->m.obs_offset[i]) * (double)ka->m.obs_scale[i];
    int ncon = ii[ka->lay.misc + 0];
    if (want_reward) {
        int latch = g_latch[env];
        int rw = E.reward(&latch);
        if (lane == 0) {
            g_latch[env] = latch;
            if (o_reward) o_reward[env] = rw;
            if (o_success) o_success[env] = (rw == max_reward);
        }
    }
    if (export_contacts)
    {
    const int expcon = RETRY ? ka->lay.expcon : ka->lay.maxcon;
    for (int c = lane; c < expcon; c += G) {
        int p = c < ncon ? ii[ka->lay.cpair + c] : -1;
        o_cpairs[((size_t)env * expcon + c) * 2] = p >= 0 ? ka->m.pair_geom[2 * p] : -1;
        o_cpairs[((size_t)env * expcon + c) * 2 + 1] = p >= 0 ? ka->m.pair_geom[2 * p + 1] : -1;
        o_cdist[(size_t)env * expcon + c] = c < ncon ? (double)r[ka->lay.cdist + c] : 0.0;
    }
    }
    if (lane == 0 && o_cost && nsub > 0) o_cost[env] = (int)((__builtin_readcyclecounter() - t_launch) >> 6);
    if (lane == 0 && !o_xpose) {
        o_ncon[env] = ncon;
        bool bad = E.diverged != 0;
        for (int i = 0; i < ka->m.nq; i++) bad |= !(fabs(r[ka->lay.qpos + i]) < real(1e6));
        o_diag[4 * env] = ncon; o_diag[4 * env + 1] = nefc_last; o_diag[4 * env + 2] = ii[ka->lay.misc + 2]; o_diag[4 * env + 3] = (bad ? 1 : 0) | ((ii[ka->lay.misc + 3] & 0xff) << 8) | ((E.nit_sum & 0xfff) << 16) | ((E.nit_max < 15 ? E.nit_max : 15) << 28);
    }
    GSYNC();
    if (RETRY && big && pass1) {
        lds_put(&pair_want[pr], 0);
    }
  }
    if (RETRY && paired) lds_put(&pair_grant[pr], PAIR_LEFT);
}

static __global__ void __launch_bounds__(1024) k_env_order(const int* __restrict__ cost, int* __restrict__ order, int N) {
    __shared__ int lo, hi, cnt[256], off[256];
    if (threadIdx.x == 0) { lo = 0x7fffffff; hi = 0; }
    if (threadIdx.x < 256) cnt[threadIdx.x] = 0;
    __syncthreads();
    int mn = 0x7fffffff, mx = 0;
    for (int i = threadIdx.x; i < N; i += 1024) { const int c = cost[i]; mn = c < mn ? c : mn; mx = c > mx ? c : mx; }
    atomicMin(&lo, mn);
    atomicMax(&hi, mx);
    __syncthreads();
    const int base = lo;
    const float scale = 255.0f / (float)(hi - lo + 1);
    auto bucket = [&](int c) { const int b = 255 - (int)((float)(c - base) * scale); return b < 0 ? 0 : (b > 255 ? 255 : b); };
    for (int i = threadIdx.x; i < N; i += 1024) atomicAdd(&cnt[bucket(cost[i])], 1);
    __syncthreads();
    if (threadIdx.x == 0) { int a = 0; for (int b = 0; b < 256; b++) { off[b] = a; a += cnt[b]; } }
    __syncthreads();
    for (int i = threadIdx.x; i < N; i += 1024) order[atomicAdd(&off[bucket(cost[i])], 1)] = i;
}

struct PhysHost;
int phys_launch_f64(PhysHost& ph, hipStream_t st, int nsub, const float* action, void* qpos, void* qvel, void* ctrl, void* warm, int* latch,
                    double* agent, int32_t* reward, uint8_t* success, std::string& err);
const void* phys_spec_kernel(const PhysHost& ph, const char** name);

struct PhysHost {
    int maxcon = 48, maxefc = 144, pgs_iters = 20, group = 64, export_contacts = 1, force_reward = 0, wpb_override = 0;
    int maxcon1 = 48, maxefc1 = 144;
    bool f64 = false;
    int specialised = 1;
    bool host_only = false;
    int N = 0, max_reward = 0;
    DevArena arena;
    DevModel<float> mf;
    DevModel<double> md;
    Layout lay, lay2;
    bool two_pass() const { return maxcon1 < maxcon || maxefc1 < maxefc; }
    int pair_waves = 1;
    int* d_retry = nullptr;
    unsigned long long retry_parity = 0;
    DevBuf kargs2;
    double *d_qpos_home = nullptr, *d_ctrl_home = nullptr, *d_obj_reset = nullptr;
    int* d_obj_qadr = nullptr;
    int *d_ncon = nullptr, *d_diag = nullptr;
    int *d_cost = nullptr, *d_order = nullptr;
    int order_envs = 1;
    bool have_cost = false;
    long long* d_prof = nullptr;
    float* d_xpose = nullptr;
    DevBuf cpairs, cdist;

    std::vector<int> img_int;
    std::vector<double> img_real;
    MOff moff;
    void* d_img_real = nullptr;
    int* d_img_int = nullptr;
    DevBuf kargs;
    bool kargs_dirty = true;
    unsigned attr_done = 0;
    int num_cu = 256;
    int persist_over = 1;
    DevBuf head;
    unsigned long long launch_count = 0;
    template <typename T>
    struct DevPtr {
        T* p;
        operator T*() const { return p; }
        operator GLB_PTR(T)() const { return (GLB_PTR(T))p; }
        operator GLB_PTR(const T)() const { return (GLB_PTR(const T))p; }
    };
    template <typename T>
    DevPtr<T> up(const std::vector<T>& v) {
        if (host_only) return DevPtr<T>{nullptr};
        T* p = arena.upload(v);
        if (!p) throw std::runtime_error(arena.error() == hipErrorOutOfMemory ? "hipMalloc failed while uploading the model" : "hipMemcpy failed while uploading the model");
        return DevPtr<T>{p};
    }
    template <typename real>
    DevPtr<real> upr(const std::vector<double>& v) {
        std::vector<real> w(v.begin(), v.end());
        return up(w);
    }

    template <typename real>
    void build(const Blob& b, DevModel<real>& m) {
        auto I = [&](const char* n) { return b.i(n); };
        auto F = [&](const char* n) { return b.f(n); };
        m.nq = b.scalar("nq"); m.nv = b.scalar("nv"); m.nu = b.scalar("nu"); m.nbody = b.scalar("nbody"); m.njnt = b.scalar("njnt");
        m.ngeom = b.scalar("ngeom"); m.npair = b.scalar("npair"); m.ntree = b.scalar("ntree"); m.neq = b.scalar("neq");
        m.task_id = b.scalar("task_id");
        m.nj = b.scalar("num_arms") == 3 ? 21 : 14;
        auto opt = F("opt");
        m.timestep = (real)opt[0]; m.gravity[0] = (real)opt[1]; m.gravity[1] = (real)opt[2]; m.gravity[2] = (real)opt[3];
        m.impratio = (real)opt[4]; m.noslip_iters = (int)opt[5]; m.noslip_per_tree = 1; m.noslip_trees = 1; m.newton_component = 1; m.newton_early_exit = 1; m.qcqp_tridiag = sizeof(real) == 4 ? 2 : 0;
        m.solver = 1; m.newton_iters = 100; m.newton_tol = sizeof(real) == 8 ? (real)1e-8 : (real)1e-6; m.ls_tolerance = sizeof(real) == 8 ? (real)1e-10 : (real)1e-4; m.ls_iterations = 50;
        m.nscale = (real)(1.0 / ((opt.size() > 7 && opt[7] > 0 ? opt[7] : 1.0) * std::max(1, m.nv)));
        auto gr = F("grip_range");
        m.grip_lo = (real)gr[0]; m.grip_hi = (real)gr[1];
        auto body_parent = I("body_parent"), body_dofadr = I("body_dofadr"), body_dofnum = I("body_dofnum"), body_tree = I("body_tree");
        auto dof_parent = I("dof_parent"), dof_tree = I("dof_tree"), tree_dofadr = I("tree_dofadr"), tree_dofnum = I("tree_dofnum");
        auto dof_body = I("dof_body");
        int nb = m.nbody, nv = m.nv, nt = m.ntree;
        for (int t = 0; t < nt; t++) if (tree_dofnum[t] > TREE_W) throw std::runtime_error("kinematic tree with more than 8 dofs");
        if (nb > 64) throw std::runtime_error("more than 64 bodies (kinematics maps one body per lane)");
        if (nt > 8) throw std::runtime_error("more than 8 kinematic trees (the per-tree solves map 8 lanes to a tree)");
        { auto jn = I("body_jntnum"); for (int bb = 0; bb < nb; bb++) if (jn[bb] > 1) throw std::runtime_error("body with more than one joint"); }
        std::vector<int> tba(nt + 1, 0), tbl;
        for (int t = 0; t < nt; t++) {
            tba[t] = (int)tbl.size();
            for (int bb = 1; bb < nb; bb++) if (body_tree[bb] == t) tbl.push_back(bb);
        }
        tba[nt] = (int)tbl.size();
        auto bpos = F("body_pos"), bquat = F("body_quat");
        std::vector<double> sx(3 * nb, 0.0), sm(9 * nb, 0.0);
        sm[0] = sm[4] = sm[8] = 1;
        auto q2m = [](const double* q, double* R) {
            double w = q[0], x = q[1], y = q[2], z = q[3];
            R[0] = 1 - 2 * (y * y + z * z); R[1] = 2 * (x * y - w * z); R[2] = 2 * (x * z + w * y);
            R[3] = 2 * (x * y + w * z); R[4] = 1 - 2 * (x * x + z * z); R[5] = 2 * (y * z - w * x);
            R[6] = 2 * (x * z - w * y); R[7] = 2 * (y * z + w * x); R[8] = 1 - 2 * (x * x + y * y);
        };
        for (int bb = 1; bb < nb; bb++) {
            if (body_tree[bb] >= 0) { sm[9 * bb] = sm[9 * bb + 4] = sm[9 * bb + 8] = 1; continue; }
            int p = body_parent[bb];
            double Rl[9];
            q2m(&bquat[4 * bb], Rl);
            for (int i = 0; i < 3; i++) {
                sx[3 * bb + i] = sx[3 * p + i] + sm[9 * p + 3 * i] * bpos[3 * bb] + sm[9 * p + 3 * i + 1] * bpos[3 * bb + 1] + sm[9 * p + 3 * i + 2] * bpos[3 * bb + 2];
                for (int j = 0; j < 3; j++) sm[9 * bb + 3 * i + j] = sm[9 * p + 3 * i] * Rl[j] + sm[9 * p + 3 * i + 1] * Rl[3 + j] + sm[9 * p + 3 * i + 2] * Rl[6 + j];
            }
        }
        std::vector<int> mask(nb, 0);
        for (int bb = 1; bb < nb; bb++) {
            int t = body_tree[bb];
            if (t < 0) continue;
            int c = bb;
            while (c > 0 && body_dofnum[c] == 0) c = body_parent[c];
            if (c == 0) continue;
            for (int d = body_dofadr[c] + body_dofnum[c] - 1; d >= 0; d = dof_parent[d]) mask[bb] |= 1 << (d - tree_dofadr[t]);
        }
        std::vector<int> mi, mj, madr(nt, 0);
        int ms = 0;
        for (int t = 0; t < nt; t++) { madr[t] = ms; ms += tree_dofnum[t] * tree_dofnum[t]; }
        for (int i = 0; i < nv; i++) for (int j = i; j >= 0; j = dof_parent[j]) { mi.push_back(i); mj.push_back(j); }
        m.msize = ms;
        m.nment = (int)mi.size();
        std::vector<int> fl, lj;
        auto floss = F("dof_frictionloss");
        for (int i = 0; i < nv; i++) if (floss[i] > 0) fl.push_back(i);
        auto jl = I("jnt_limited");
        for (int j = 0; j < m.njnt; j++) if (jl[j]) lj.push_back(j);
        m.nfloss = (int)fl.size();
        m.nlimited = (int)lj.size();
        m.body_parent = up(body_parent); moff.body_parent = (int)img_int.size(); { auto v_ = body_parent; img_int.insert(img_int.end(), v_.begin(), v_.end()); } m.body_jntadr = up(I("body_jntadr")); moff.body_jntadr = (int)img_int.size(); { auto v_ = I("body_jntadr"); img_int.insert(img_int.end(), v_.begin(), v_.end()); } m.body_jntnum = up(I("body_jntnum")); moff.body_jntnum = (int)img_int.size(); { auto v_ = I("body_jntnum"); img_int.insert(img_int.end(), v_.begin(), v_.end()); }
        m.body_dofadr = up(body_dofadr); moff.body_dofadr = (int)img_int.size(); { auto v_ = body_dofadr; img_int.insert(img_int.end(), v_.begin(), v_.end()); } m.body_dofnum = up(body_dofnum); moff.body_dofnum = (int)img_int.size(); { auto v_ = body_dofnum; img_int.insert(img_int.end(), v_.begin(), v_.end()); } m.body_tree = up(body_tree); moff.body_tree = (int)img_int.size(); { auto v_ = body_tree; img_int.insert(img_int.end(), v_.begin(), v_.end()); } m.body_dofmask = up(mask); moff.body_dofmask = (int)img_int.size(); { auto v_ = mask; img_int.insert(img_int.end(), v_.begin(), v_.end()); }
        {
            std::vector<int> last(nb);
            for (int bb = 0; bb < nb; bb++) last[bb] = bb;
            for (int bb = nb - 1; bb > 0; bb--) { int pp = body_parent[bb]; if (last[bb] > last[pp]) last[pp] = last[bb]; }
            for (int bb = 1; bb < nb; bb++) { int pp = body_parent[bb]; if (!(pp < bb && bb <= last[pp])) throw std::runtime_error("bodies are not in depth-first order"); }
            for (int pp = 0; pp < nb; pp++) for (int d = pp + 1; d <= last[pp]; d++) { int a = d; while (a > pp) a = body_parent[a]; if (a != pp) throw std::runtime_error("bodies are not in depth-first order"); }
            m.body_last = up(last); moff.body_last = (int)img_int.size(); img_int.insert(img_int.end(), last.begin(), last.end());
        }
        m.body_pos = upr<real>(bpos); moff.body_pos = (int)img_real.size(); { auto v_ = bpos; img_real.insert(img_real.end(), v_.begin(), v_.end()); } m.body_quat = upr<real>(bquat); moff.body_quat = (int)img_real.size(); { auto v_ = bquat; img_real.insert(img_real.end(), v_.begin(), v_.end()); } m.body_mass = upr<real>(F("body_mass")); moff.body_mass = (int)img_real.size(); { auto v_ = F("body_mass"); img_real.insert(img_real.end(), v_.begin(), v_.end()); } m.body_ipos = upr<real>(F("body_ipos")); moff.body_ipos = (int)img_real.size(); { auto v_ = F("body_ipos"); img_real.insert(img_real.end(), v_.begin(), v_.end()); }
        m.body_inertia = upr<real>(F("body_inertia")); moff.body_inertia = (int)img_real.size(); { auto v_ = F("body_inertia"); img_real.insert(img_real.end(), v_.begin(), v_.end()); } m.body_invweight0 = upr<real>(F("body_invweight0")); moff.body_invweight0 = (int)img_real.size(); { auto v_ = F("body_invweight0"); img_real.insert(img_real.end(), v_.begin(), v_.end()); }
        m.static_xpos = upr<real>(sx); m.static_xmat = upr<real>(sm);
        m.tree_bodyadr = up(tba); moff.tree_bodyadr = (int)img_int.size(); { auto v_ = tba; img_int.insert(img_int.end(), v_.begin(), v_.end()); } m.tree_bodylist = up(tbl); moff.tree_bodylist = (int)img_int.size(); { auto v_ = tbl; img_int.insert(img_int.end(), v_.begin(), v_.end()); } m.tree_dofadr = up(tree_dofadr); moff.tree_dofadr = (int)img_int.size(); { auto v_ = tree_dofadr; img_int.insert(img_int.end(), v_.begin(), v_.end()); } m.tree_dofnum = up(tree_dofnum); moff.tree_dofnum = (int)img_int.size(); { auto v_ = tree_dofnum; img_int.insert(img_int.end(), v_.begin(), v_.end()); } m.tree_madr = up(madr); moff.tree_madr = (int)img_int.size(); { auto v_ = madr; img_int.insert(img_int.end(), v_.begin(), v_.end()); }
        m.jnt_type = up(I("jnt_type")); moff.jnt_type = (int)img_int.size(); { auto v_ = I("jnt_type"); img_int.insert(img_int.end(), v_.begin(), v_.end()); } m.jnt_qposadr = up(I("jnt_qposadr")); moff.jnt_qposadr = (int)img_int.size(); { auto v_ = I("jnt_qposadr"); img_int.insert(img_int.end(), v_.begin(), v_.end()); } m.jnt_dofadr = up(I("jnt_dofadr")); moff.jnt_dofadr = (int)img_int.size(); { auto v_ = I("jnt_dofadr"); img_int.insert(img_int.end(), v_.begin(), v_.end()); }
        m.jnt_actfrclimited = up(I("jnt_actfrclimited")); moff.jnt_actfrclimited = (int)img_int.size(); { auto v_ = I("jnt_actfrclimited"); img_int.insert(img_int.end(), v_.begin(), v_.end()); } m.limited_jnt = up(lj); moff.limited_jnt = (int)img_int.size(); { auto v_ = lj; img_int.insert(img_int.end(), v_.begin(), v_.end()); }
        m.jnt_pos = upr<real>(F("jnt_pos")); moff.jnt_pos = (int)img_real.size(); { auto v_ = F("jnt_pos"); img_real.insert(img_real.end(), v_.begin(), v_.end()); } m.jnt_axis = upr<real>(F("jnt_axis")); moff.jnt_axis = (int)img_real.size(); { auto v_ = F("jnt_axis"); img_real.insert(img_real.end(), v_.begin(), v_.end()); } m.jnt_range = upr<real>(F("jnt_range")); moff.jnt_range = (int)img_real.size(); { auto v_ = F("jnt_range"); img_real.insert(img_real.end(), v_.begin(), v_.end()); }
        m.jnt_actfrcrange = upr<real>(F("jnt_actfrcrange")); moff.jnt_actfrcrange = (int)img_real.size(); { auto v_ = F("jnt_actfrcrange"); img_real.insert(img_real.end(), v_.begin(), v_.end()); } m.jnt_solref = upr<real>(F("jnt_solref")); m.jnt_solimp = upr<real>(F("jnt_solimp"));
        m.jnt_margin = upr<real>(F("jnt_margin")); moff.jnt_margin = (int)img_real.size(); { auto v_ = F("jnt_margin"); img_real.insert(img_real.end(), v_.begin(), v_.end()); }
        m.dof_body = up(dof_body); moff.dof_body = (int)img_int.size(); { auto v_ = dof_body; img_int.insert(img_int.end(), v_.begin(), v_.end()); } m.dof_parent = up(dof_parent); moff.dof_parent = (int)img_int.size(); { auto v_ = dof_parent; img_int.insert(img_int.end(), v_.begin(), v_.end()); } m.dof_tree = up(dof_tree); moff.dof_tree = (int)img_int.size(); { auto v_ = dof_tree; img_int.insert(img_int.end(), v_.begin(), v_.end()); } m.dof_jnt = up(I("dof_jnt")); moff.dof_jnt = (int)img_int.size(); { auto v_ = I("dof_jnt"); img_int.insert(img_int.end(), v_.begin(), v_.end()); }
        m.floss_dof = up(fl); moff.floss_dof = (int)img_int.size(); { auto v_ = fl; img_int.insert(img_int.end(), v_.begin(), v_.end()); } m.ment_i = up(mi); moff.ment_i = (int)img_int.size(); { auto v_ = mi; img_int.insert(img_int.end(), v_.begin(), v_.end()); } m.ment_j = up(mj); moff.ment_j = (int)img_int.size(); { auto v_ = mj; img_int.insert(img_int.end(), v_.begin(), v_.end()); }
        m.dof_armature = upr<real>(F("dof_armature")); moff.dof_armature = (int)img_real.size(); { auto v_ = F("dof_armature"); img_real.insert(img_real.end(), v_.begin(), v_.end()); } m.dof_damping = upr<real>(F("dof_damping")); moff.dof_damping = (int)img_real.size(); { auto v_ = F("dof_damping"); img_real.insert(img_real.end(), v_.begin(), v_.end()); } m.dof_frictionloss = upr<real>(floss); moff.dof_frictionloss = (int)img_real.size(); { auto v_ = floss; img_real.insert(img_real.end(), v_.begin(), v_.end()); }
        m.dof_invweight0 = upr<real>(F("dof_invweight0")); moff.dof_invweight0 = (int)img_real.size(); { auto v_ = F("dof_invweight0"); img_real.insert(img_real.end(), v_.begin(), v_.end()); } m.dof_solref = upr<real>(F("dof_solref")); m.dof_solimp = upr<real>(F("dof_solimp"));
        m.act_dof = up(I("act_dof")); moff.act_dof = (int)img_int.size(); { auto v_ = I("act_dof"); img_int.insert(img_int.end(), v_.begin(), v_.end()); } m.act_qposadr = up(I("act_qposadr")); moff.act_qposadr = (int)img_int.size(); { auto v_ = I("act_qposadr"); img_int.insert(img_int.end(), v_.begin(), v_.end()); } m.act_ctrllimited = up(I("act_ctrllimited")); moff.act_ctrllimited = (int)img_int.size(); { auto v_ = I("act_ctrllimited"); img_int.insert(img_int.end(), v_.begin(), v_.end()); }
        m.act_kp = upr<real>(F("act_kp")); moff.act_kp = (int)img_real.size(); { auto v_ = F("act_kp"); img_real.insert(img_real.end(), v_.begin(), v_.end()); } m.act_kv = upr<real>(F("act_kv")); moff.act_kv = (int)img_real.size(); { auto v_ = F("act_kv"); img_real.insert(img_real.end(), v_.begin(), v_.end()); } m.act_gear = upr<real>(F("act_gear")); moff.act_gear = (int)img_real.size(); { auto v_ = F("act_gear"); img_real.insert(img_real.end(), v_.begin(), v_.end()); } m.act_ctrlrange = upr<real>(F("act_ctrlrange")); moff.act_ctrlrange = (int)img_real.size(); { auto v_ = F("act_ctrlrange"); img_real.insert(img_real.end(), v_.begin(), v_.end()); }
        m.eq_dof1 = up(I("eq_dof1")); m.eq_dof2 = up(I("eq_dof2")); m.eq_qpos1 = up(I("eq_qpos1")); m.eq_qpos2 = up(I("eq_qpos2"));
        m.eq_polycoef = upr<real>(F("eq_polycoef")); m.eq_solref = upr<real>(F("eq_solref")); m.eq_solimp = upr<real>(F("eq_solimp"));
        m.qpos0 = upr<real>(F("qpos0"));
        m.qpos_home = upr<real>(F("qpos_home"));
        m.obj_qadr = up(I("objects_qposadr")); m.nobj = (int)I("objects_qposadr").size();
        {
            auto home = F("qpos_home"); auto oa = I("objects_qposadr");
            std::vector<double> o((size_t)N * oa.size() * 7);
            for (int e = 0; e < N; e++) for (size_t k = 0; k < oa.size(); k++) for (int c = 0; c < 7; c++) o[((size_t)e * oa.size() + k) * 7 + c] = home[oa[k] + c];
            d_obj_reset = up(o); m.obj_reset = d_obj_reset;
        }
        auto gbody = I("geom_body");
        auto gpos = F("geom_pos"), gquat = F("geom_quat"), gbc = F("geom_bcenter");
        int ng = m.ngeom;
        std::vector<double> gmat(9 * ng), gcp(3 * ng), gx0(3 * ng, 0.0), gm0(9 * ng, 0.0), gc0(3 * ng, 0.0);
        std::vector<int> gstat(ng);
        std::vector<double> gaabb(6 * ng, 0.0), glbox(6 * ng, 0.0);
        auto ghull = I("geom_chull"); auto gtype = I("geom_type"); auto gsize = F("geom_size"); auto hv = F("chull_vert");
        for (int g = 0; g < ng; g++) {
            q2m(&gquat[4 * g], &gmat[9 * g]);
            for (int i = 0; i < 3; i++)
                gcp[3 * g + i] = gpos[3 * g + i] + gmat[9 * g + 3 * i] * gbc[3 * g] + gmat[9 * g + 3 * i + 1] * gbc[3 * g + 1] + gmat[9 * g + 3 * i + 2] * gbc[3 * g + 2];
            {
                double lo[3] = {1e30, 1e30, 1e30}, hi[3] = {-1e30, -1e30, -1e30};
                if (gtype[g] == G_MESH) {
                    for (int v = 0; v < ghull[2 * g + 1]; v++)
                        for (int k = 0; k < 3; k++) { double x = hv[3 * (ghull[2 * g] + v) + k]; if (x < lo[k]) lo[k] = x; if (x > hi[k]) hi[k] = x; }
                } else {
                    double ex[3] = {gsize[3 * g], gsize[3 * g + 1], gsize[3 * g + 2]};
                    if (gtype[g] == G_SPHERE) ex[1] = ex[2] = ex[0];
                    if (gtype[g] == G_CYLINDER) { ex[2] = ex[1]; ex[1] = ex[0]; }
                    for (int k = 0; k < 3; k++) { lo[k] = -ex[k]; hi[k] = ex[k]; }
                }
                for (int k = 0; k < 3; k++) { glbox[6 * g + k] = 0.5 * (lo[k] + hi[k]); glbox[6 * g + 3 + k] = 0.5 * (hi[k] - lo[k]); }
            }
            int bb = gbody[g];
            gstat[g] = body_tree[bb] < 0;
            if (gstat[g]) {
                for (int i = 0; i < 3; i++) {
                    gx0[3 * g + i] = sx[3 * bb + i] + sm[9 * bb + 3 * i] * gpos[3 * g] + sm[9 * bb + 3 * i + 1] * gpos[3 * g + 1] + sm[9 * bb + 3 * i + 2] * gpos[3 * g + 2];
                    gc0[3 * g + i] = sx[3 * bb + i] + sm[9 * bb + 3 * i] * gcp[3 * g] + sm[9 * bb + 3 * i + 1] * gcp[3 * g + 1] + sm[9 * bb + 3 * i + 2] * gcp[3 * g + 2];
                    for (int j = 0; j < 3; j++)
                        gm0[9 * g + 3 * i + j] = sm[9 * bb + 3 * i] * gmat[9 * g + j] + sm[9 * bb + 3 * i + 1] * gmat[9 * g + 3 + j] + sm[9 * bb + 3 * i + 2] * gmat[9 * g + 6 + j];
                }
                std::vector<double> pts;
                if (gtype[g] == G_MESH) {
                    for (int v = 0; v < ghull[2 * g + 1]; v++) for (int k = 0; k < 3; k++) pts.push_back(hv[3 * (ghull[2 * g] + v) + k]);
                } else {
                    double ex[3] = {gsize[3 * g], gsize[3 * g + 1], gsize[3 * g + 2]};
                    if (gtype[g] == G_SPHERE) ex[1] = ex[2] = ex[0];
                    if (gtype[g] == G_CYLINDER) { ex[2] = ex[1]; ex[1] = ex[0]; }
                    for (int c = 0; c < 8; c++) for (int k = 0; k < 3; k++) pts.push_back(((c >> k) & 1) ? ex[k] : -ex[k]);
                }
                for (int k = 0; k < 3; k++) { gaabb[6 * g + k] = 1e30; gaabb[6 * g + 3 + k] = -1e30; }
                for (size_t v = 0; v < pts.size() / 3; v++)
                    for (int i = 0; i < 3; i++) {
                        double w = gx0[3 * g + i] + gm0[9 * g + 3 * i] * pts[3 * v] + gm0[9 * g + 3 * i + 1] * pts[3 * v + 1] + gm0[9 * g + 3 * i + 2] * pts[3 * v + 2];
                        if (w < gaabb[6 * g + i]) gaabb[6 * g + i] = w;
                        if (w > gaabb[6 * g + 3 + i]) gaabb[6 * g + 3 + i] = w;
                    }
            }
        }
        m.geom_type = up(I("geom_type")); moff.geom_type = (int)img_int.size(); { auto v_ = I("geom_type"); img_int.insert(img_int.end(), v_.begin(), v_.end()); } m.geom_body = up(gbody); moff.geom_body = (int)img_int.size(); { auto v_ = gbody; img_int.insert(img_int.end(), v_.begin(), v_.end()); } m.geom_hull = up(I("geom_ctab")); m.geom_class = up(I("geom_class")); m.geom_static = up(gstat); moff.geom_static = (int)img_int.size(); { auto v_ = gstat; img_int.insert(img_int.end(), v_.begin(), v_.end()); }
        m.geom_pos = upr<real>(gpos); m.geom_mat = upr<real>(gmat); m.geom_size = upr<real>(F("geom_size")); m.geom_cpos = upr<real>(gcp); moff.geom_cpos = (int)img_real.size(); { auto v_ = gcp; img_real.insert(img_real.end(), v_.begin(), v_.end()); }
        m.geom_rbound = upr<real>(F("geom_rbound")); moff.geom_rbound = (int)img_real.size(); { auto v_ = F("geom_rbound"); img_real.insert(img_real.end(), v_.begin(), v_.end()); } m.geom_xpos0 = upr<real>(gx0); m.geom_xmat0 = upr<real>(gm0); m.geom_cen0 = upr<real>(gc0); m.geom_aabb0 = upr<real>(gaabb); m.geom_lbox = upr<real>(glbox);
        {
            auto ctab = I("geom_ctab"), cells = I("chull_cells"), cand = I("chull_cand");
            const size_t ncell = cells.size();
            std::vector<double> tab(32 * ncell, 0.0), ovf;
            std::vector<char> done(ncell, 0);
            for (int g = 0; g < ng; g++) {
                if (gtype[g] != G_MESH) continue;
                const int cb = ctab[2 * g], R = ctab[2 * g + 1], adr = ghull[2 * g];
                for (int c = 0; c < 6 * R * R; c++) {
                    if (done[cb + c]) continue;
                    done[cb + c] = 1;
                    const int rec = cells[cb + c], off = rec >> 8, cnt = rec & 255;
                    if (cnt < 1) throw std::runtime_error("support table: empty cell");
                    double* o = &tab[32 * (size_t)(cb + c)];
                    for (int k = 0; k < 8; k++) {
                        const int v = cand[off + (k < cnt ? k : cnt - 1)];
                        if (v < 0 || v >= ghull[2 * g + 1]) throw std::runtime_error("support table: candidate index outside its hull");
                        for (int q = 0; q < 3; q++) o[4 * k + q] = hv[3 * (size_t)(adr + v) + q];
                        o[4 * k + 3] = (double)v;
                    }
                    o[3] = (double)cnt;
                    o[7] = (double)(ovf.size() / 4);
                    for (int k = 8; k < cnt; k++) {
                        const int v = cand[off + k];
                        if (v < 0 || v >= ghull[2 * g + 1]) throw std::runtime_error("support table: candidate index outside its hull");
                        for (int q = 0; q < 3; q++) ovf.push_back(hv[3 * (size_t)(adr + v) + q]);
                        ovf.push_back((double)v);
                    }
                }
            }
            if (ovf.size() / 4 >= (1u << 24)) throw std::runtime_error("support table: overflow part too large");
            m.hull_ovf = (int)(tab.size() / 4);
            tab.insert(tab.end(), ovf.begin(), ovf.end());
            if (tab.empty()) tab.assign(4, 0.0);
            m.hull_vert = upr<real>(tab);
        }
        m.pair_geom = up(I("pair_geom")); m.pair_condim = up(I("pair_condim"));
        m.pair_friction = upr<real>(F("pair_friction")); m.pair_solref = upr<real>(F("pair_solref")); m.pair_solimp = upr<real>(F("pair_solimp"));
        m.pair_margin = upr<real>(F("pair_margin")); m.pair_gap = upr<real>(F("pair_gap"));
        m.obs_qposadr = up(I("obs_qposadr")); m.obs_offset = upr<real>(F("obs_offset")); m.obs_scale = upr<real>(F("obs_scale"));
        while (img_real.size() % 4) img_real.push_back(0.0);
        while (img_int.size() % 4) img_int.push_back(0);
        moff.nreal = (int)img_real.size();
        moff.nint = (int)img_int.size();
        d_img_real = (void*)upr<real>(img_real);
        d_img_int = up(img_int);
    }

    const void* spec_kernel(const char** name) const {
        if (f64 || specialised == 0 || two_pass()) return nullptr;
        return phys_spec_kernel(*this, name);
    }
    bool refuses(std::string& err) const {
        if (specialised != 2 || spec_kernel(nullptr)) return false;
        err = std::string("phys_specialised = 2: no kernel compiled for this handle's model and layout (") +
              (f64 ? "f64 handle" : two_pass() ? "two capacity tiers" : "Layout, table offsets, dims or solver options (solver, noslip_*, qcqp_tridiag, newton_*, ls_iterations, num_joints) match no spec of avsim_phys_specs.h") + "); the launch would take the generic k_phys";
        return true;
    }
    int spec_note = 0;

    void make_layout(int nq, int nv, int nu, int nb, int ng, int msize, int ntree) {
        if (maxcon1 > maxcon) maxcon1 = maxcon;
        if (maxefc1 > maxefc) maxefc1 = maxefc;
        make_layout_of(lay, maxcon1, maxefc1, nq, nv, nu, nb, ng, msize, ntree);
        make_layout_of(lay2, maxcon, maxefc, nq, nv, nu, nb, ng, msize, ntree);
    }
    void make_layout_of(Layout& L, const int maxcon, const int maxefc, int nq, int nv, int nu, int nb, int ng, int msize, int ntree) {
        kargs_dirty = true;
        L = avs::make_layout_of(maxcon, maxefc, this->maxcon, this->maxefc, nq, nv, nu, nb, ng, msize, ntree, f64 ? 8 : 4);
        if (getenv("AVSIM_DEBUG_LAYOUT")) {
            const int pb = L.rowS + RS_S * maxefc > L.scr + NARROW_SCR_W ? L.rowS + RS_S * maxefc : L.scr + NARROW_SCR_W;
            fprintf(stderr, "avsim layout: %d reals + %d ints = %d B per env (U at %d: phase A %d, phase B %d words); tables %zu B\n", L.nreal, L.nint,
                    L.bytes_per_env, L.U, 38 * nb, pb - L.U, (size_t)moff.nreal * (f64 ? 8 : 4) + (size_t)moff.nint * 4);
        }
    }

    int dims[7] = {0, 0, 0, 0, 0, 0, 0};
    size_t lds_bytes() const { return (size_t)lay.bytes_per_env + (size_t)moff.nreal * (f64 ? 8 : 4) + (size_t)moff.nint * 4; }
    DevBuf rows, coup, near, gref;
    void alloc_contacts() {
        if (host_only) return;
        if (rows.alloc((size_t)N * maxefc * ROW_S * (f64 ? 8 : 4) * 2) != hipSuccess) throw std::runtime_error("hipMalloc of the constraint row buffers failed");
        mf.rJ_glob = rows.as<float>(); md.rJ_glob = rows.as<double>();
        mf.rB_glob = mf.rJ_glob + (size_t)N * maxefc * ROW_S; md.rB_glob = md.rJ_glob + (size_t)N * maxefc * ROW_S;
        if (gref.alloc(((size_t)N * dims[4] * 3 + (size_t)N * 64 * BOX_OVF_W) * (f64 ? 8 : 4)) != hipSuccess) throw std::runtime_error("hipMalloc of the Verlet reference buffer failed");
        mf.gref_glob = gref.as<float>(); md.gref_glob = gref.as<double>();
        mf.bxo_glob = mf.gref_glob + (size_t)N * dims[4] * 3; md.bxo_glob = md.gref_glob + (size_t)N * dims[4] * 3;
        if (coup.alloc((size_t)N * lay2.maxgrp * GA_W * (f64 ? 8 : 4)) != hipSuccess || near.alloc((size_t)N * (NEAR_MAX + CAND_MAX) * 4) != hipSuccess)
            throw std::runtime_error("hipMalloc of the coupling / neighbour buffers failed");
        int* const d_near = near.as<int>();
        mf.gA_glob = coup.as<float>(); md.gA_glob = coup.as<double>(); mf.near_glob = d_near; md.near_glob = d_near; mf.cand_glob = md.cand_glob = d_near + (size_t)N * NEAR_MAX;
        kargs_dirty = true;
        if (cpairs.alloc((size_t)N * maxcon * 8) != hipSuccess || cdist.alloc((size_t)N * maxcon * 8) != hipSuccess)
            throw std::runtime_error("hipMalloc of the contact export buffers failed");
        (void)hipMemset(cpairs.ptr(), 0xff, (size_t)N * maxcon * 8);
        (void)hipMemset(cdist.ptr(), 0, (size_t)N * maxcon * 8);
    }
    bool init(const Blob& b, int N_, bool f64_, std::string& err) {
        N = N_;
        f64 = f64_;
        try {
            if (f64) build(b, md); else build(b, mf);
            static const int mx[5] = {4, 4, 5, 3, 4};
            max_reward = mx[b.scalar("task_id")];
            int ms = f64 ? md.msize : mf.msize;
            const int *cap_efc = CAP_EFC, *cap_con = CAP_CON, *cap_efc1 = CAP_EFC1, *cap_con1 = CAP_CON1;
            maxefc = cap_efc[b.scalar("task_id")];
            maxcon = cap_con[b.scalar("task_id")];
            maxefc1 = cap_efc1[b.scalar("task_id")];
            maxcon1 = cap_con1[b.scalar("task_id")];
            dims[0] = b.scalar("nq"); dims[1] = b.scalar("nv"); dims[2] = b.scalar("nu"); dims[3] = b.scalar("nbody"); dims[4] = b.scalar("ngeom"); dims[5] = ms; dims[6] = b.scalar("ntree");
            make_layout(dims[0], dims[1], dims[2], dims[3], dims[4], dims[5], dims[6]);
            d_qpos_home = up(b.f("qpos_home"));
            d_ctrl_home = up(b.f("ctrl_home"));
            d_obj_qadr = up(b.i("objects_qposadr"));
            d_ncon = up(std::vector<int>((size_t)N, 0));
            d_diag = up(std::vector<int>((size_t)N * 4, 0));
            d_cost = up(std::vector<int>((size_t)N, 0));
            d_order = up(std::vector<int>((size_t)N, 0));
            d_retry = up(std::vector<int>(2 * (size_t)N + 2, 0));
            alloc_contacts();
        } catch (const std::exception& e) {
            err = std::string("physics init: ") + e.what();
            return false;
        }
        return true;
    }
    bool set_option(const char* name, double v) {
        std::string n(name);
        kargs_dirty = true;
        if (n == "pgs_iters") { pgs_iters = (int)v; return true; }
        if (n == "solver") { if (v != 0 && v != 1) return false; mf.solver = md.solver = (int)v; return true; }
        if (n == "newton_iters") { if (v < 1 || v > 100) return false; mf.newton_iters = md.newton_iters = (int)v; return true; }
        if (n == "newton_tol") { if (v < 0) return false; mf.newton_tol = (float)v; md.newton_tol = v; return true; }
        if (n == "ls_tolerance") { if (!(v > 0) || v >= 1) return false; mf.ls_tolerance = (float)v; md.ls_tolerance = v; return true; }
        if (n == "ls_iterations") { if (v < 1 || v > 1000) return false; mf.ls_iterations = md.ls_iterations = (int)v; return true; }
        if (n == "export_contacts") { export_contacts = v != 0; return true; }
        if (n == "num_joints") { if (v != 14 && v != 21) return false; mf.nj = md.nj = (int)v; return true; }
        if (n == "order_envs") { order_envs = v != 0; return true; }
        if (n == "phys_specialised") { if (v != 0 && v != 1 && v != 2) return false; specialised = (int)v; return true; }
        if (n == "pair_waves") { pair_waves = v != 0; return true; }
        if (n == "qcqp_tridiag") { mf.qcqp_tridiag = md.qcqp_tridiag = v < 0 ? 0 : (v > 2 ? 2 : (int)v); return true; }
        if (n == "noslip_iters") { if (v < 0 || v > 100) return false; mf.noslip_iters = md.noslip_iters = (int)v; return true; }
        if (n == "noslip_per_tree") { mf.noslip_per_tree = md.noslip_per_tree = v != 0; return true; }
        if (n == "noslip_trees") { mf.noslip_trees = md.noslip_trees = v != 0; return true; }
        if (n == "newton_component") { mf.newton_component = md.newton_component = v != 0; return true; }
        if (n == "newton_early_exit") { mf.newton_early_exit = md.newton_early_exit = v != 0; return true; }
        if (n == "persist_blocks") { int x = (int)v; if (x >= 1 && x <= 64) { persist_over = x; return true; } return false; }
        if (n == "waves_per_block") { int x = (int)v; if (x >= 0 && x <= AVSIM_PHYS_MAXW) { wpb_override = x; return true; } return false; }
        if (n == "profile_phases") {
            if (v != 0 && !d_prof) d_prof = up(std::vector<long long>((size_t)N * PROF_W, 0));
            if (v == 0) d_prof = nullptr;
            return true;
        }
        if (n == "maxefc" || n == "maxcon" || n == "maxefc_first" || n == "maxcon_first") {
            int x = (int)v;
            if (x < 16 || x > 1000) return false;
            (void)hipDeviceSynchronize();
            if (n == "maxefc") maxefc = maxefc1 = x; else if (n == "maxcon") maxcon = maxcon1 = x;
            else if (n == "maxefc_first") maxefc1 = x < maxefc ? x : maxefc; else maxcon1 = x < maxcon ? x : maxcon;
            make_layout(dims[0], dims[1], dims[2], dims[3], dims[4], dims[5], dims[6]);
            alloc_contacts();
            return true;
        }
        return false;
    }

    template <typename real, int MAXW>
    int waves_per_block(const Layout& L) const {
        const size_t tables = (size_t)moff.nreal * sizeof(real) + (size_t)moff.nint * 4;
        int wpb = tables < 160 * 1024 ? (int)((160 * 1024 - tables) / (size_t)L.bytes_per_env) : 0;
        if (wpb > MAXW) wpb = MAXW;
        if (wpb_override > 0) wpb = wpb_override < MAXW ? wpb_override : MAXW;
        return wpb < 1 ? 1 : wpb;
    }

    template <typename real, int G, int MAXW>
    int launch_t(hipStream_t st, const DevModel<real>& m, int nsub, const float* action, void* qpos, void* qvel, void* ctrl, void* warm,
                 int* latch, double* agent, int32_t* reward, uint8_t* success, std::string& err) {
        const size_t tables = (size_t)moff.nreal * sizeof(real) + (size_t)moff.nint * 4;
        auto kern1 = k_phys<real, G, MAXW, false>;
        auto kern2 = k_phys<real, G, MAXW, true>;
        const char* spec_name = nullptr;
        const void* kspec = sizeof(real) == 4 && MAXW == AVSIM_PHYS_MAXW ? spec_kernel(&spec_name) : nullptr;
        if (refuses(err)) return -1;
        if (spec_note != (kspec ? 1 : 2) && getenv("AVSIM_DEBUG_LAYOUT")) {
            fprintf(stderr, "avsim: k_phys %s%s\n", kspec ? "specialised for " : "generic", kspec ? spec_name : "");
            spec_note = kspec ? 1 : 2;
        }
        if (!attr_done) {
            hipError_t e = hipFuncSetAttribute((const void*)kern1, hipFuncAttributeMaxDynamicSharedMemorySize, 160 * 1024);
            if (e == hipSuccess) e = hipFuncSetAttribute((const void*)kern2, hipFuncAttributeMaxDynamicSharedMemorySize, 160 * 1024);
            if (e != hipSuccess) { err = std::string("hipFuncSetAttribute: ") + hipGetErrorString(e); return -3; }
            int dev = 0;
            hipDeviceProp_t prop;
            if (hipGetDevice(&dev) == hipSuccess && hipGetDeviceProperties(&prop, dev) == hipSuccess && prop.multiProcessorCount > 0) num_cu = prop.multiProcessorCount;
            if (!head) {
                if (head.reserve(2 * sizeof(int)) != hipSuccess) { err = "hipMalloc(work counters) failed"; return -3; }
                (void)hipMemset(head.ptr(), 0, 2 * sizeof(int));
            }
            attr_done = 1;
        }
        if (kspec) {
            if (!(attr_done & 2)) {
                const hipError_t e = hipFuncSetAttribute(kspec, hipFuncAttributeMaxDynamicSharedMemorySize, 160 * 1024);
                if (e != hipSuccess) { err = std::string("hipFuncSetAttribute(") + spec_name + "): " + hipGetErrorString(e); return -3; }
                attr_done |= 2;
            }
            kern1 = (decltype(kern1))kspec;
        }
        const bool two = two_pass();
        int wpb = waves_per_block<real, MAXW>(lay);
        const int wpb2 = waves_per_block<real, MAXW>(lay2);
        if (!two && wpb_override <= 0 && num_cu > 0 && N < num_cu * wpb) { wpb = (N + num_cu - 1) / num_cu; if (wpb < 1) wpb = 1; }
        const size_t pairflags = two ? 2 * (MAXW / 2 > 0 ? MAXW / 2 : 1) * sizeof(int) : 0;
        const size_t shmem = (size_t)lay.bytes_per_env * wpb + tables + pairflags, shmem2 = (size_t)lay2.bytes_per_env * wpb2 + tables + pairflags;
        const int pairing = (two && wpb >= 2 && lay2.bytes_per_env <= 2 * lay.bytes_per_env && pair_waves) ? 8 : 0;
        if (shmem > 160 * 1024 || (two && shmem2 > 160 * 1024)) { err = "per-block LDS exceeds 160 KiB; lower maxefc/maxcon"; return -1; }
        const int per_cu = (int)((160 * 1024) / shmem) > 0 ? (int)((160 * 1024) / shmem) : 1;
        int nblk = num_cu * per_cu * (persist_over > 0 ? persist_over : 1);
        if (nblk > (N + wpb - 1) / wpb) nblk = (N + wpb - 1) / wpb;
        if (kargs_dirty) {
            KArgs<real> ka{m, lay, moff}, ka2{m, lay2, moff};
            if (kargs.reserve(sizeof(KArgs<double>)) != hipSuccess || kargs2.reserve(sizeof(KArgs<double>)) != hipSuccess) { err = "hipMalloc(kernel arguments) failed"; return -3; }
            (void)hipStreamSynchronize(st);
            if (hipMemcpy(kargs.ptr(), &ka, sizeof(ka), hipMemcpyHostToDevice) != hipSuccess || hipMemcpy(kargs2.ptr(), &ka2, sizeof(ka2), hipMemcpyHostToDevice) != hipSuccess) { err = "hipMemcpy(kernel arguments) failed"; return -3; }
            kargs_dirty = false;
        }
        static_assert((8 | 7) < (1 << 8), "retry_mode: mode bits and pairing flag below bit 8");
        if (two && (maxcon1 >= 1024 || maxefc1 >= 1024 || maxcon1 < 0 || maxefc1 < 0)) { err = "first-tier capacities do not fit the 10-bit fields of retry_mode (maxcon_first / maxefc_first < 1024)"; return -1; }
        const int* order = nullptr;
        if (order_envs && have_cost && nsub > 0 && N > wpb) {
            hipLaunchKernelGGL(k_env_order, dim3(1), dim3(1024), 0, st, (const int*)d_cost, d_order, N);
            order = d_order;
        }
        const int want_reward = (reward || success) && (nsub > 0 || force_reward) ? 1 : 0;
        const int par = (int)(retry_parity & 1);
        int* const rlist = d_retry + 2;
        {
            int* head = this->head.as<int>() + (launch_count & 1);
            int* next = this->head.as<int>() + ((launch_count + 1) & 1);
            launch_count++;
            hipLaunchKernelGGL(two ? kern2 : kern1, dim3(nblk), dim3(64 * wpb), shmem, st, (KPtr<real>)kargs.ptr(), (const real*)d_img_real, (const int*)d_img_int, N, nsub, pgs_iters, action, want_reward,
                               (real*)qpos, (real*)qvel, (real*)ctrl, (real*)warm, latch, agent, (int*)reward, (unsigned char*)success, d_ncon,
                               cpairs.as<int>(), cdist.as<double>(), d_diag, max_reward, export_contacts, d_prof, d_xpose, order, order_envs ? d_cost : (int*)nullptr, head, next,
                               d_retry, two ? (1 + 2 * par) | pairing : 0, (KPtr<real>)kargs2.ptr());
        }
        if (two) {
            int* head = this->head.as<int>() + (launch_count & 1);
            int* next = this->head.as<int>() + ((launch_count + 1) & 1);
            launch_count++;
            retry_parity++;
            int nblk2 = num_cu;
            if (nblk2 > (N + wpb2 - 1) / wpb2) nblk2 = (N + wpb2 - 1) / wpb2;
            hipLaunchKernelGGL(kern2, dim3(nblk2), dim3(64 * wpb2), shmem2, st, (KPtr<real>)kargs2.ptr(), (const real*)d_img_real, (const int*)d_img_int, N, nsub, pgs_iters, action, want_reward,
                               (real*)qpos, (real*)qvel, (real*)ctrl, (real*)warm, latch, agent, (int*)reward, (unsigned char*)success, d_ncon,
                               cpairs.as<int>(), cdist.as<double>(), d_diag, max_reward, export_contacts, d_prof, d_xpose, (const int*)rlist, order_envs ? d_cost : (int*)nullptr, head, next,
                               d_retry, (2 + 2 * par) | (maxcon1 << 8) | (maxefc1 << 18), (KPtr<real>)kargs2.ptr());
        }
        if (nsub > 0) have_cost = true;
        hipError_t e = hipGetLastError();
        if (e != hipSuccess) { err = std::string("physics kernel launch: ") + hipGetErrorString(e); return -3; }
        return 0;
    }

#if !defined(AVSIM_TU_F64) && !defined(AVSIM_NO_F32_LAUNCH)
    int launch(hipStream_t st, int N_, int nsub, const float* action, int nj, void* qpos, void* qvel, void* ctrl, void* warm, int* latch,
               double* agent, int32_t* reward, uint8_t* success, std::string& err) {
        (void)N_; (void)nj;
        if (f64) return phys_launch_f64(*this, st, nsub, action, qpos, qvel, ctrl, warm, latch, agent, reward, success, err);
        return launch_t<float, 64, AVSIM_PHYS_MAXW>(st, mf, nsub, action, qpos, qvel, ctrl, warm, latch, agent, reward, success, err);
    }
#endif
};

template <typename SPEC>
inline bool spec_matches(const PhysHost& ph) {
    static_assert(sizeof(Layout) == LAYOUT_WORDS * sizeof(int) && sizeof(MOff) == MOFF_WORDS * sizeof(int), "structs of ints, no padding");
    static constexpr Layout lay = SPEC::lay;
    static constexpr MOff mo = SPEC::mo;
    static_assert(((size_t)mo.nreal * sizeof(float) + (size_t)mo.nint * 4) % 16 == 0, "the records behind the table image start 16-byte aligned without padding");
    if (std::memcmp(&ph.lay, &lay, sizeof(Layout)) != 0 || std::memcmp(&ph.lay2, &lay, sizeof(Layout)) != 0 || std::memcmp(&ph.moff, &mo, sizeof(MOff)) != 0 ||
        std::memcmp(ph.dims, SPEC::dims, sizeof(ph.dims)) != 0)
        return false;
#define AVSIM_SPEC_INT(x) if (ph.mf.x != SPEC::x) return false;
    AVSIM_HEAD_INTS(AVSIM_SPEC_INT)
    AVSIM_BODY_INTS(AVSIM_SPEC_INT)
#undef AVSIM_SPEC_INT
    return true;
}

}
```

av_aloha_amd/csrc/avsim_phys_layout.h:

```cpp
#pragma once

namespace avs {

constexpr int RS_S = 9;
constexpr int ANC_MAX = 64;
constexpr int NARROW_SCR_W = 64 * 24 + 4 * 56;

struct MOff {
    int nreal, nint;
    int body_parent;
    int body_jntadr;
    int body_jntnum;
    int body_dofadr;
    int body_dofnum;
    int body_tree;
    int body_dofmask;
    int body_last;
    int tree_bodyadr;
    int tree_bodylist;
    int tree_dofadr;
    int tree_dofnum;
    int tree_madr;
    int jnt_type;
    int jnt_qposadr;
    int jnt_dofadr;
    int jnt_actfrclimited;
    int limited_jnt;
    int dof_body;
    int dof_parent;
    int dof_tree;
    int dof_jnt;
    int floss_dof;
    int ment_i;
    int ment_j;
    int act_dof;
    int act_qposadr;
    int act_ctrllimited;
    int geom_type;
    int geom_body;
    int geom_static;
    int body_pos;
    int body_quat;
    int body_mass;
    int body_ipos;
    int body_inertia;
    int body_invweight0;
    int jnt_pos;
    int jnt_axis;
    int jnt_range;
    int jnt_actfrcrange;
    int jnt_margin;
    int dof_armature;
    int dof_damping;
    int dof_frictionloss;
    int dof_invweight0;
    int act_kp;
    int act_kv;
    int act_gear;
    int act_ctrlrange;
    int geom_cpos;
    int geom_rbound;
};
constexpr int MOFF_WORDS = sizeof(MOff) / sizeof(int);

struct Layout {
    int qpos, qvel, ctrl, warm, xpos, xmat, xipos, cdof, gcen, M, L, Minv, bias, fsm, asm_, qacc, fcon, nH, ng, ndl, njv, U, nreal;
    int cinert, cvel, cacc, cfrc, binert;
    int cdist, cpos, cnrm, rowS, scr;
    int cand, cpair, cefc, rmeta, rowI, gI, misc, nprof, nint;
    int maxgrp;
    int maxcon, maxefc;
    int expcon;
    int gefc, ggrp;
    int bytes_per_env;
};
constexpr int LAYOUT_WORDS = sizeof(Layout) / sizeof(int);

constexpr Layout make_layout_of(int maxcon, int maxefc, int full_maxcon, int full_maxefc, int nq, int nv, int nu, int nb, int ng, int msize,
                                int ntree, int real_bytes) {
    Layout L{};
    int o = 0;
    L.qpos = o; o += nq; L.qvel = o; o += nv; L.ctrl = o; o += nu; L.warm = o; o += nv;
    L.xpos = o; o += 3 * nb; L.xmat = o; o += 9 * nb; L.xipos = o; o += 3 * nb; L.cdof = o; o += 6 * nv; L.gcen = o; o += 3 * ng;
    L.M = o; o += msize; L.L = o; o += msize; o = (o + 3) & ~3; L.Minv = o; o += 64 * ntree;
    L.bias = o; o += nv; L.fsm = o; o += nv; L.asm_ = o; o += nv; L.qacc = o; o += nv; L.fcon = o; o += nv;
    {
        const int nvh = nv * (nv + 1) / 2, need1 = nvh + 2 * nv, need2 = need1 + maxefc, avail = 15 * nb + 6 * nv + 3 * ng;
        int base = L.xpos;
        if (!(need1 <= avail)) { base = o; o += need1; }
        L.nH = base; L.ng = base + nvh; L.ndl = L.ng + nv;
        if (need2 <= avail) L.njv = L.ndl + nv;
        else { L.njv = o; o += maxefc; }
    }
    L.U = o;
    int a = o;
    L.cinert = a; a += 10 * nb; L.binert = a; a += 10 * nb; L.cvel = a; a += 6 * nb; L.cacc = a; a += 6 * nb; L.cfrc = a; a += 6 * nb;
    int bq = o;
    L.cdist = bq; bq += maxcon; L.cpos = bq; bq += 3 * maxcon; L.cnrm = bq; bq += 3 * maxcon;
    bq = (bq + 3) & ~3; L.rowS = bq; L.scr = bq; bq += RS_S * maxefc;
    L.maxgrp = maxefc / 3 + 8;
    if (bq < L.scr + NARROW_SCR_W) bq = L.scr + NARROW_SCR_W;
    o = a > bq ? a : bq;
    L.nreal = (o + 3) & ~3;
    int io = 0;
    L.cand = io; io += ANC_MAX; L.cpair = io; io += maxcon; L.cefc = io; io += maxcon; L.rmeta = io; io += maxefc; L.rowI = io; io += maxefc;
    L.gI = io; io += maxefc / 3 + 8; L.misc = io; io += 12; L.nprof = io; io += 16;
    L.nint = (io + 3) & ~3;
    L.maxcon = maxcon;
    L.maxefc = maxefc;
    L.expcon = full_maxcon;
    L.gefc = full_maxefc;
    L.ggrp = full_maxefc / 3 + 8;
    L.bytes_per_env = (int)(((unsigned long long)L.nreal * (unsigned)real_bytes + (unsigned long long)L.nint * 4 + 15) & ~15ull);
    return L;
}

constexpr int CAP_EFC[5] = {176, 176, 336, 480, 176}, CAP_CON[5] = {48, 48, 72, 96, 48};
constexpr int CAP_EFC1[5] = {176, 176, 224, 288, 176}, CAP_CON1[5] = {48, 48, 56, 64, 48};

}
```

Measured before the change: 1.043 million.

## Fuse pre-collision phases with pipelined broadphase and persist near lists across launches

Splits crb, rne_bias and smooth into sub-steps and interleaves them with a register-pipelined broadphase in one fused pre phase, so independent work shares each group barrier and fewer GSYNCs run per substep. Broadphase pair records and AABBs are prefetched into registers in stages, which hides global-load latency behind the dynamics work. The near-list valid flags are saved to global memory per env and restored on the next launch, so the neighbour list need not be rebuilt every step. In exchange it raises register pressure, gives cdd its own slot sized by nv, and adds a layout check that can throw.

```diff
diff --git a/av_aloha_amd/csrc/avsim_phys.hip.h b/av_aloha_amd/csrc/avsim_phys.hip.h
--- a/av_aloha_amd/csrc/avsim_phys.hip.h
+++ b/av_aloha_amd/csrc/avsim_phys.hip.h
@@ -157,6 +157,7 @@
     GLB_PTR(const int) obs_qposadr;
     GLB_PTR(const real) obs_offset;
     GLB_PTR(const real) obs_scale;
+    int* nearv_glob;
 };
 
 template <typename real> using DevModel = DevModelT<real, DevHead<real>>;
@@ -174,6 +175,16 @@
 
 struct GenericSpec {};
 template <typename SPEC> constexpr bool spec_fixed = !std::is_same<SPEC, GenericSpec>::value;
+#if defined(AVS_NO_NEAR_KEEP)
+template <typename SPEC> constexpr bool keep_near = false;
+#else
+template <typename SPEC> constexpr bool keep_near = spec_fixed<SPEC>;
+#endif
+#if defined(AVS_PRE_SERIAL) || defined(AVS_NO_SPLIT_PRE)
+template <typename SPEC> constexpr bool fused_pre = false;
+#else
+template <typename SPEC> constexpr bool fused_pre = spec_fixed<SPEC>;
+#endif
 template <typename real, typename SPEC>
 struct KFixed {
     using Model = DevModelT<real, FixedHead<real, SPEC>>;
@@ -1897,33 +1908,33 @@
         GSYNC();
     }
 
-    __device__ void crb() {
-        PHASE_BEGIN();
-        real *xmat = r + ka->lay.xmat, *xipos = r + ka->lay.xipos, *cdof = r + ka->lay.cdof, *ci = r + ka->lay.cinert, *M = r + ka->lay.M, *L = r + ka->lay.L;
+    __device__ void crb_binert(const real* __restrict__ xmat, const real* __restrict__ xipos, real* __restrict__ ci, real* __restrict__ bi, real* __restrict__ M) {
         for (int b = lane; b < ka->m.nbody; b += G) {
             SInert<real> s;
             if (body_tree_()[b] >= 0) body_inertia(ka, xmat, xipos, b, s);
             else { s.m = 0; for (int k = 0; k < 3; k++) s.h[k] = 0; for (int k = 0; k < 6; k++) s.I[k] = 0; }
-            real *o = ci + 10 * b, *ob = r + ka->lay.binert + 10 * b;
+            real *o = ci + 10 * b, *ob = bi + 10 * b;
             o[0] = ob[0] = s.m;
             for (int k = 0; k < 3; k++) o[1 + k] = ob[1 + k] = s.h[k];
             for (int k = 0; k < 6; k++) o[4 + k] = ob[4 + k] = s.I[k];
         }
         for (int i = lane; i < ka->m.msize; i += G) M[i] = 0;
-        GSYNC();
-        {
-            real acc[10];
+    }
+    __device__ bool crb_comp_sum(const real* __restrict__ ci, real (&acc)[10]) {
             const int p = lane < ka->m.nbody ? lane : 0;
             const bool dyn = lane < ka->m.nbody && body_tree_()[p] >= 0;
             for (int k = 0; k < 10; k++) acc[k] = 0;
             if (dyn)
                 for (int d = p; d <= body_last_()[p]; d++)
                     for (int k = 0; k < 10; k++) acc[k] += ci[10 * d + k];
-            GSYNC();
+            return dyn;
+    }
+    __device__ void crb_comp_put(real* __restrict__ ci, const real (&acc)[10], bool dyn) {
+            const int p = lane < ka->m.nbody ? lane : 0;
             if (dyn)
                 for (int k = 0; k < 10; k++) ci[10 * p + k] = acc[k];
-        }
-        GSYNC();
+    }
+    __device__ void crb_ment(const real* __restrict__ ci, const real* __restrict__ cdof, real* __restrict__ M) {
         for (int e = lane; e < ka->m.nment; e += G) {
             int i = ment_i_()[e], j = ment_j_()[e], t = dof_tree_()[i], n = tree_dofnum_()[t], a = tree_dofadr_()[t];
             real f[6];
@@ -1935,10 +1946,8 @@
             Mb[(i - a) * n + (j - a)] = v;
             Mb[(j - a) * n + (i - a)] = v;
         }
-        GSYNC();
-        tree_chol(M, L, (const real*)nullptr, real(0));
-        GSYNC();
-        real* Minv = r + ka->lay.Minv;
+    }
+    __device__ void crb_minv(const real* __restrict__ L, real* __restrict__ Minv) {
         for (int w = lane; w < ka->m.ntree * TREE_W; w += G) {
             int t = w >> 3, j = w & 7, n = tree_dofnum_()[t];
             real x[TREE_W];
@@ -1964,16 +1973,9 @@
 #pragma unroll
             for (int k = 0; k < TREE_W; k++) Minv[64 * t + 8 * k + j] = (k < n && j < n) ? x[k] : real(0);
         }
-        GSYNC();
-    }
-
-    __device__ void rne_bias() {
-        PHASE_BEGIN();
-        real *xmat = r + ka->lay.xmat, *xipos = r + ka->lay.xipos, *cdof = r + ka->lay.cdof, *qvel = r + ka->lay.qvel;
-        real *cvel = r + ka->lay.cvel, *cfrc = r + ka->lay.cfrc, *bias = r + ka->lay.bias;
-        real* cdd = r + ka->lay.cinert;
-        const int nb = ka->m.nbody;
-        for (int b = lane; b < nb; b += G) {
+    }
+    __device__ void rne_cvel(const real* __restrict__ cdof, const real* __restrict__ qvel, real* __restrict__ cvel) {
+        for (int b = lane; b < ka->m.nbody; b += G) {
             real v[6] = {0, 0, 0, 0, 0, 0};
             const int t = body_tree_()[b];
             if (t >= 0) {
@@ -1989,7 +1991,8 @@
             }
             for (int q = 0; q < 6; q++) cvel[6 * b + q] = v[q];
         }
-        GSYNC();
+    }
+    __device__ void rne_cdd(const real* __restrict__ cdof, const real* __restrict__ qvel, const real* __restrict__ cvel, real* __restrict__ cdd) {
         for (int d = lane; d < ka->m.nv; d += G) {
             const int j = dof_jnt_()[d], b = dof_body_()[d];
             real o[6] = {0, 0, 0, 0, 0, 0};
@@ -2007,8 +2010,9 @@
             const real qd = qvel[d];
             for (int q = 0; q < 6; q++) cdd[6 * d + q] = o[q] * qd;
         }
-        GSYNC();
-        for (int b = lane; b < nb; b += G) {
+    }
+    __device__ void rne_cfrc(const real* __restrict__ cdd, const real* __restrict__ cvel, const real* __restrict__ bi, real* __restrict__ cfrc) {
+        for (int b = lane; b < ka->m.nbody; b += G) {
             const int t = body_tree_()[b];
             real f[6] = {0, 0, 0, 0, 0, 0};
             if (t >= 0) {
@@ -2023,7 +2027,7 @@
                 }
                 for (int q = 0; q < 6; q++) v[q] = cvel[6 * b + q];
                 real sv[10];
-                for (int q = 0; q < 10; q++) sv[q] = (r + ka->lay.binert)[10 * b + q];
+                for (int q = 0; q < 10; q++) sv[q] = bi[10 * b + q];
                 real Ia[6], Iv[6], vIv[6];
                 inert_mul(sv, a, Ia);
                 inert_mul(sv, v, Iv);
@@ -2032,7 +2036,8 @@
             }
             for (int q = 0; q < 6; q++) cfrc[6 * b + q] = f[q];
         }
-        GSYNC();
+    }
+    __device__ void rne_tau(const real* __restrict__ cdof, const real* __restrict__ cfrc, real* __restrict__ bias) {
         for (int i = lane; i < ka->m.nv; i += G) {
             const int b = dof_body_()[i];
             real f[6] = {0, 0, 0, 0, 0, 0};
@@ -2042,15 +2047,11 @@
             for (int q = 0; q < 6; q++) sacc += cdof[6 * i + q] * f[q];
             bias[i] = sacc;
         }
-        GSYNC();
-    }
-
-    __device__ void smooth() {
-        PHASE_BEGIN();
-        real *qpos = r + ka->lay.qpos, *qvel = r + ka->lay.qvel, *ctrl = r + ka->lay.ctrl, *bias = r + ka->lay.bias, *fsm = r + ka->lay.fsm, *as = r + ka->lay.asm_;
-        real* act = r + ka->lay.fcon;
+    }
+    __device__ void sm_act0(real* __restrict__ act) {
         for (int i = lane; i < ka->m.nv; i += G) act[i] = 0;
-        GSYNC();
+    }
+    __device__ void sm_act(const real* __restrict__ qpos, const real* __restrict__ qvel, const real* __restrict__ ctrl, real* __restrict__ act) {
         for (int u = lane; u < ka->m.nu; u += G) {
             real c = ctrl[u];
             if (act_ctrllimited_()[u]) c = tclamp(c, act_ctrlrange_()[2 * u], act_ctrlrange_()[2 * u + 1]);
@@ -2058,7 +2059,8 @@
             real f = act_kp_()[u] * c - act_kp_()[u] * qpos[act_qposadr_()[u]] - act_kv_()[u] * qvel[dof];
             act[dof] += act_gear_()[u] * f;
         }
-        GSYNC();
+    }
+    __device__ void sm_fsm(const real* __restrict__ qvel, const real* __restrict__ bias, const real* __restrict__ act, real* __restrict__ fsm, real* __restrict__ as) {
         for (int i = lane; i < ka->m.nv; i += G) {
             int j = dof_jnt_()[i];
             real a = act[i];
@@ -2067,6 +2069,52 @@
             fsm[i] = f;
             as[i] = f;
         }
+    }
+
+    __device__ void crb() {
+        PHASE_BEGIN();
+        real *xmat = r + ka->lay.xmat, *xipos = r + ka->lay.xipos, *cdof = r + ka->lay.cdof, *ci = r + ka->lay.cinert, *M = r + ka->lay.M, *L = r + ka->lay.L;
+        crb_binert(xmat, xipos, ci, r + ka->lay.binert, M);
+        GSYNC();
+        {
+            real acc[10];
+            const bool dyn = crb_comp_sum(ci, acc);
+            GSYNC();
+            crb_comp_put(ci, acc, dyn);
+        }
+        GSYNC();
+        crb_ment(ci, cdof, M);
+        GSYNC();
+        tree_chol(M, L, (const real*)nullptr, real(0));
+        GSYNC();
+        crb_minv(L, r + ka->lay.Minv);
+        GSYNC();
+    }
+
+    __device__ void rne_bias() {
+        PHASE_BEGIN();
+        real *cdof = r + ka->lay.cdof, *qvel = r + ka->lay.qvel;
+        real *cvel = r + ka->lay.cvel, *cfrc = r + ka->lay.cfrc, *bias = r + ka->lay.bias;
+        real* cdd = r + ka->lay.cdd;
+        rne_cvel(cdof, qvel, cvel);
+        GSYNC();
+        rne_cdd(cdof, qvel, cvel, cdd);
+        GSYNC();
+        rne_cfrc(cdd, cvel, r + ka->lay.binert, cfrc);
+        GSYNC();
+        rne_tau(cdof, cfrc, bias);
+        GSYNC();
+    }
+
+    __device__ void smooth() {
+        PHASE_BEGIN();
+        real *qpos = r + ka->lay.qpos, *qvel = r + ka->lay.qvel, *ctrl = r + ka->lay.ctrl, *bias = r + ka->lay.bias, *fsm = r + ka->lay.fsm, *as = r + ka->lay.asm_;
+        real* act = r + ka->lay.fcon;
+        sm_act0(act);
+        GSYNC();
+        sm_act(qpos, qvel, ctrl, act);
+        GSYNC();
+        sm_fsm(qvel, bias, act, fsm, as);
         GSYNC();
         {
             const int t = lane >> 3, i = lane & 7;
@@ -2120,87 +2168,205 @@
         for (int c = 0; c < 3; c++) os[SLOT_P + 3 * (1 + pert) + c] = pk[c];
     }
 
+    struct PairRec { int g1, g2; real mg; };
+    AVS_DEV PairRec pair_fetch(int p) const {
+        PairRec q;
+        q.g1 = ka->m.pair_geom[2 * p]; q.g2 = ka->m.pair_geom[2 * p + 1];
+        q.mg = ka->m.pair_margin[p];
+        return q;
+    }
+    template <bool ALWAYS = false>
+    AVS_DEV void pair_box(const PairRec& q, real (&bb)[6]) const {
+        const bool s1 = geom_static_()[q.g1], s2 = geom_static_()[q.g2];
+        if (!ALWAYS) for (int k = 0; k < 6; k++) bb[k] = 0;
+        if (ALWAYS || s1 || s2) {
+            const int gs = s1 ? q.g1 : q.g2;
+            for (int k = 0; k < 6; k++) bb[k] = ka->m.geom_aabb0[6 * gs + k];
+        }
+    }
+    AVS_DEV bool pair_test(const PairRec& q, const real (&bb)[6], const real* gcen, real pad) const {
+        const int g1 = q.g1, g2 = q.g2;
+        bool s1 = geom_static_()[g1], s2 = geom_static_()[g2];
+        real mg = q.mg + pad;
+        if (s1 || s2) {
+            int gd = s1 ? g2 : g1;
+            real rd = geom_rbound_()[gd] + mg, d2 = 0;
+            for (int k = 0; k < 3; k++) {
+                real c = gcen[3 * gd + k], lo = bb[k], hi = bb[3 + k];
+                real e = c < lo ? lo - c : (c > hi ? c - hi : real(0));
+                d2 += e * e;
+            }
+            return !(d2 > rd * rd);
+        }
+        real d[3], rr = geom_rbound_()[g1] + geom_rbound_()[g2] + mg;
+        sub3(gcen + 3 * g2, gcen + 3 * g1, d);
+        return !(dot3(d, d) > rr * rr);
+    }
+    AVS_DEV bool pair_hit(int p, real pad, const real* gcen) const {
+        const PairRec q = pair_fetch(p);
+        real bb[6];
+        pair_box(q, bb);
+        return pair_test(q, bb, gcen, pad);
+    }
+    static constexpr real broad_skin() { return real(0.03); }
+    AVS_DEV bool geom_moved(const real* gcen, int g, const real (&gr)[3]) const {
+        const real skin = broad_skin();
+        const real d[3] = {gcen[3 * g] - gr[0], gcen[3 * g + 1] - gr[1], gcen[3 * g + 2] - gr[2]};
+        return dot3(d, d) > real(0.25) * skin * skin;
+    }
+    __device__ int broad_rebuild(const real* gcen, int* misc) {
+        GLB_PTR(real) gref = gref_();
+        GLB_PTR(int) nearl = near_();
+        int nnear = 0;
+#pragma unroll 1
+        for (int base = 0; base < ka->m.npair; base += G) {
+            int p = base + lane;
+            bool hit = p < ka->m.npair && pair_hit(p, broad_skin(), gcen);
+            int tot, rk = group_rank<G>(hit, grp, lane, &tot);
+            if (hit && nnear + rk < NEAR_MAX) nearl[nnear + rk] = p;
+            nnear += tot;
+        }
+        for (int i = lane; i < 3 * ka->m.ngeom; i += G) gref[i] = gcen[i];
+        if (lane == 0) { misc[6] = nnear < NEAR_MAX ? nnear : NEAR_MAX; misc[7] = nnear <= NEAR_MAX; if (nnear > NEAR_MAX) misc[2] |= 8; }
+        GSYNC();
+        return nnear;
+    }
+    AVS_DEV void cand_push(bool hit, int p, int& ncand, int* misc) {
+        GLB_PTR(int) cand = cand_();
+        int tot, rk = group_rank<G>(hit, grp, lane, &tot);
+        if (hit && ncand + rk < CAND_MAX) cand[ncand + rk] = p;
+        if (ncand + tot > CAND_MAX && lane == 0) misc[2] |= 4;
+        ncand = ncand + tot < CAND_MAX ? ncand + tot : CAND_MAX;
+    }
+    __device__ int broad_exact(const real* gcen, int* misc, int nnear) {
+        GLB_PTR(int) nearl = near_();
+        int ncand = 0;
+        if (nnear <= NEAR_MAX) {
+            for (int base = 0; base < nnear; base += G) {
+                int i = base + lane, p = i < nnear ? nearl[i] : 0;
+                bool hit = i < nnear && pair_hit(p, real(0), gcen);
+                cand_push(hit, p, ncand, misc);
+            }
+        } else {
+#pragma unroll 1
+            for (int base = 0; base < ka->m.npair; base += G) {
+                int p = base + lane;
+                bool hit = p < ka->m.npair && pair_hit(p, real(0), gcen);
+                cand_push(hit, p, ncand, misc);
+            }
+        }
+        return ncand;
+    }
+    __device__ int broad_serial(const real* gcen, int* misc) {
+        GLB_PTR(real) gref = gref_();
+        bool moved = false;
+        if (misc[7]) {
+            for (int g = lane; g < ka->m.ngeom; g += G)
+                if (!geom_static_()[g]) {
+                    const real gr[3] = {gref[3 * g], gref[3 * g + 1], gref[3 * g + 2]};
+                    moved |= geom_moved(gcen, g, gr);
+                }
+        }
+        bool rebuild = !misc[7] || __any(moved);
+        int nnear = misc[6];
+        if (rebuild) nnear = broad_rebuild(gcen, misc);
+        const int ncand = broad_exact(gcen, misc, nnear);
+        if (lane == 0) misc[3] = ncand;
+        return ncand;
+    }
+    static constexpr int BROAD_KP = 4;
+    template <typename S> static constexpr int spec_ngeom() { if constexpr (spec_fixed<S>) return S::ngeom; else return G; }
+    static constexpr int BROAD_NGP = (spec_ngeom<SPEC>() + G - 1) / G;
+    struct BroadPipe {
+        int valid = 0, nnear = 0;
+        bool piped = false;
+        int p[BROAD_KP];
+        PairRec q[BROAD_KP];
+        real bb[BROAD_KP][6];
+        real gr[BROAD_NGP][3];
+    };
+    AVS_DEV void broad_fetch_near(BroadPipe& B) {
+        GLB_PTR(int) nearl = near_();
+#pragma unroll
+        for (int k = 0; k < BROAD_KP; k++) B.p[k] = nearl[k * G + lane];
+    }
+    AVS_DEV void broad_fetch_ref(BroadPipe& B, const int* misc) {
+        static_assert(BROAD_KP * G <= NEAR_MAX, "the pipelined passes lie inside the near list");
+        GLB_PTR(real) gref = gref_();
+#pragma unroll
+        for (int j = 0; j < BROAD_NGP; j++) {
+            const int g = j * G + lane < ka->m.ngeom ? j * G + lane : ka->m.ngeom - 1;
+            for (int k = 0; k < 3; k++) B.gr[j][k] = gref[3 * g + k];
+        }
+        broad_fetch_near(B);
+        B.valid = __builtin_amdgcn_readfirstlane(misc[7]);
+        B.nnear = __builtin_amdgcn_readfirstlane(misc[6]);
+    }
+    AVS_DEV void broad_moved(BroadPipe& B, const real* gcen, int* misc) {
+        bool moved = false;
+        if (B.valid) {
+#pragma unroll
+            for (int j = 0; j < BROAD_NGP; j++) {
+                const int g = j * G + lane;
+                if (g < ka->m.ngeom && !geom_static_()[g]) moved |= geom_moved(gcen, g, B.gr[j]);
+            }
+        }
+        const bool rebuild = !B.valid || __any(moved);
+        if (rebuild) {
+            B.nnear = broad_rebuild(gcen, misc);
+            broad_fetch_near(B);
+        }
+        B.piped = B.nnear <= BROAD_KP * G;
+    }
+    AVS_DEV void broad_fetch_pair(BroadPipe& B) {
+#pragma unroll
+        for (int k = 0; k < BROAD_KP; k++) {
+            B.p[k] = k * G + lane < B.nnear ? B.p[k] : 0;
+            B.q[k] = pair_fetch(B.p[k]);
+        }
+    }
+    AVS_DEV void broad_fetch_box(BroadPipe& B) {
+#pragma unroll
+        for (int k = 0; k < BROAD_KP; k++) pair_box<true>(B.q[k], B.bb[k]);
+    }
+    AVS_DEV void broad_finish(BroadPipe& B, const real* gcen, int* misc) {
+        int ncand = 0;
+        if (B.piped) {
+#pragma unroll
+            for (int k = 0; k < BROAD_KP; k++)
+                if (k * G < B.nnear) {
+                    const int i = k * G + lane;
+                    const bool hit = i < B.nnear && pair_test(B.q[k], B.bb[k], gcen, real(0));
+                    cand_push(hit, B.p[k], ncand, misc);
+                }
+        } else ncand = broad_exact(gcen, misc, B.nnear);
+        if (lane == 0) misc[3] = ncand;
+    }
+
     __device__ AVS_OUTLINE void collide() {
         Env e(*this);
-        e.collide_i();
+        e.template collide_i<false>();
         diverged = e.diverged; nit_sum = e.nit_sum; nit_max = e.nit_max; t_broad = e.t_broad; t_narrow = e.t_narrow;
     }
+    __device__ AVS_OUTLINE void collide_narrow() {
+        Env e(*this);
+        e.template collide_i<true>();
+        diverged = e.diverged; nit_sum = e.nit_sum; nit_max = e.nit_max; t_broad = e.t_broad; t_narrow = e.t_narrow;
+    }
+    template <bool BROAD_DONE>
     __device__ __attribute__((always_inline)) void collide_i() {
         PHASE_BEGIN();
         real* gcen = r + ka->lay.gcen;
         int* misc = ii + ka->lay.misc;
         GLB_PTR(int) cand = cand_();
-        int ncand = 0;
         long long tb0 = __builtin_readcyclecounter();
-        const real skin = real(0.03);
-        GLB_PTR(real) gref = gref_();
-        GLB_PTR(int) nearl = near_();
-        auto pair_hit = [&](int p, real pad) -> bool {
-            int g1 = ka->m.pair_geom[2 * p], g2 = ka->m.pair_geom[2 * p + 1];
-            bool s1 = geom_static_()[g1], s2 = geom_static_()[g2];
-            real mg = ka->m.pair_margin[p] + pad;
-            if (s1 || s2) {
-                int gs = s1 ? g1 : g2, gd = s1 ? g2 : g1;
-                real rd = geom_rbound_()[gd] + mg, d2 = 0;
-                for (int k = 0; k < 3; k++) {
-                    real c = gcen[3 * gd + k], lo = ka->m.geom_aabb0[6 * gs + k], hi = ka->m.geom_aabb0[6 * gs + 3 + k];
-                    real e = c < lo ? lo - c : (c > hi ? c - hi : real(0));
-                    d2 += e * e;
-                }
-                return !(d2 > rd * rd);
-            }
-            real d[3], rr = geom_rbound_()[g1] + geom_rbound_()[g2] + mg;
-            sub3(gcen + 3 * g2, gcen + 3 * g1, d);
-            return !(dot3(d, d) > rr * rr);
-        };
-        bool moved = false;
-        if (misc[7]) {
-            for (int g = lane; g < ka->m.ngeom; g += G)
-                if (!geom_static_()[g]) {
-                    const real d[3] = {gcen[3 * g] - gref[3 * g], gcen[3 * g + 1] - gref[3 * g + 1], gcen[3 * g + 2] - gref[3 * g + 2]};
-                    moved |= dot3(d, d) > real(0.25) * skin * skin;
-                }
-        }
-        bool rebuild = !misc[7] || __any(moved);
-        int nnear = misc[6];
-        if (rebuild) {
-            nnear = 0;
-#pragma unroll 1
-            for (int base = 0; base < ka->m.npair; base += G) {
-                int p = base + lane;
-                bool hit = p < ka->m.npair && pair_hit(p, skin);
-                int tot, rk = group_rank<G>(hit, grp, lane, &tot);
-                if (hit && nnear + rk < NEAR_MAX) nearl[nnear + rk] = p;
-                nnear += tot;
-            }
-            for (int i = lane; i < 3 * ka->m.ngeom; i += G) gref[i] = gcen[i];
-            if (lane == 0) { misc[6] = nnear < NEAR_MAX ? nnear : NEAR_MAX; misc[7] = nnear <= NEAR_MAX; if (nnear > NEAR_MAX) misc[2] |= 8; }
+        int ncand;
+        if constexpr (!BROAD_DONE) {
+            ncand = broad_serial(gcen, misc);
             GSYNC();
-        }
-        if (nnear <= NEAR_MAX) {
-            for (int base = 0; base < nnear; base += G) {
-                int i = base + lane, p = i < nnear ? nearl[i] : 0;
-                bool hit = i < nnear && pair_hit(p, real(0));
-                int tot, rk = group_rank<G>(hit, grp, lane, &tot);
-                if (hit && ncand + rk < CAND_MAX) cand[ncand + rk] = p;
-                if (ncand + tot > CAND_MAX && lane == 0) misc[2] |= 4;
-                ncand = ncand + tot < CAND_MAX ? ncand + tot : CAND_MAX;
-            }
-        } else {
-#pragma unroll 1
-            for (int base = 0; base < ka->m.npair; base += G) {
-                int p = base + lane;
-                bool hit = p < ka->m.npair && pair_hit(p, real(0));
-                int tot, rk = group_rank<G>(hit, grp, lane, &tot);
-                if (hit && ncand + rk < CAND_MAX) cand[ncand + rk] = p;
-                if (ncand + tot > CAND_MAX && lane == 0) misc[2] |= 4;
-                ncand = ncand + tot < CAND_MAX ? ncand + tot : CAND_MAX;
-            }
-        }
-        if (lane == 0) misc[3] = ncand;
-        GSYNC();
+        } else ncand = __builtin_amdgcn_readfirstlane(misc[3]);
         long long tb1 = __builtin_readcyclecounter();
-        t_broad += tb1 - tb0;
+        if constexpr (!BROAD_DONE) t_broad += tb1 - tb0;
         real *cdist = r + ka->lay.cdist, *cpos = r + ka->lay.cpos, *cnrm = r + ka->lay.cnrm;
         int* cpair = ii + ka->lay.cpair;
         int ncon = 0, ovf = 0;
@@ -2325,6 +2491,51 @@
     __device__ AVS_OUTLINE void pre_phases() {
         Env e(*this);
         e.kinematics(); e.crb(); e.rne_bias(); e.smooth();
+    }
+    __device__ AVS_OUTLINE void pre_fused() {
+        Env e(*this);
+        e.kinematics();
+        e.pre_fused_i();
+    }
+    __device__ __attribute__((always_inline)) void pre_fused_i() {
+        PHASE_BEGIN();
+        real *qpos = r + ka->lay.qpos, *qvel = r + ka->lay.qvel, *ctrl = r + ka->lay.ctrl, *xmat = r + ka->lay.xmat, *xipos = r + ka->lay.xipos, *cdof = r + ka->lay.cdof;
+        real *gcen = r + ka->lay.gcen, *M = r + ka->lay.M, *L = r + ka->lay.L, *bias = r + ka->lay.bias, *fsm = r + ka->lay.fsm, *as = r + ka->lay.asm_, *act = r + ka->lay.fcon;
+        real *ci = r + ka->lay.cinert, *bi = r + ka->lay.binert, *cvel = r + ka->lay.cvel, *cdd = r + ka->lay.cdd, *cfrc = r + ka->lay.cfrc;
+        int* misc = ii + ka->lay.misc;
+        BroadPipe B;
+        broad_fetch_ref(B, misc);
+        crb_binert(xmat, xipos, ci, bi, M);
+        rne_cvel(cdof, qvel, cvel);
+        sm_act0(act);
+        broad_moved(B, gcen, misc);
+        GSYNC();
+        broad_fetch_pair(B);
+        real acc[10];
+        const bool dyn = crb_comp_sum(ci, acc);
+        rne_cdd(cdof, qvel, cvel, cdd);
+        sm_act(qpos, qvel, ctrl, act);
+        GSYNC();
+        broad_fetch_box(B);
+        crb_comp_put(ci, acc, dyn);
+        rne_cfrc(cdd, cvel, bi, cfrc);
+        broad_finish(B, gcen, misc);
+        GSYNC();
+        crb_ment(ci, cdof, M);
+        rne_tau(cdof, cfrc, bias);
+        GSYNC();
+        tree_chol(M, L, (const real*)nullptr, real(0));
+        sm_fsm(qvel, bias, act, fsm, as);
+        GSYNC();
+        {
+            const int t = lane >> 3, i = lane & 7;
+            const bool mine = t < ka->m.ntree && i < tree_dofnum_()[t];
+            const int k = mine ? tree_dofadr_()[t] + i : 0;
+            const real x = tree_solve(L, mine ? as[k] : real(0));
+            crb_minv(L, r + ka->lay.Minv);
+            if (mine) as[k] = x;
+        }
+        GSYNC();
     }
     __device__ AVS_OUTLINE void post_phases() {
         Env e(*this);
@@ -3018,6 +3229,8 @@
     for (int i = lane; i < ka->m.nu; i += G) r[ka->lay.ctrl + i] = g_ctrl[(size_t)env * ka->m.nu + i];
     if (lane == 0) for (int k = 0; k < 8; k++) { ii[ka->lay.misc + k] = 0; ii[ka->lay.nprof + k] = 0; ii[ka->lay.nprof + 8 + k] = 0; }
     if (lane == 0) ii[ka->lay.misc + 8] = 0;
+    if constexpr (keep_near<SPEC>)
+        if (lane == 0) { ii[ka->lay.misc + 6] = ka->m.nearv_glob[2 * (size_t)env]; ii[ka->lay.misc + 7] = ka->m.nearv_glob[2 * (size_t)env + 1]; }
     E.profiling = o_prof != nullptr;
     GSYNC();
     if (action) {
@@ -3033,7 +3246,8 @@
 #define PROF(k, stmt) do { if (o_prof) { long long t0_ = __builtin_readcyclecounter(); stmt; tp[k] += __builtin_readcyclecounter() - t0_; } else { stmt; } } while (0)
     for (int s = 0; s < nsub; s++) {
 #ifndef AVS_NO_SPLIT_PRE
-        PROF(0, E.pre_phases());
+        if constexpr (fused_pre<SPEC>) PROF(0, E.pre_fused());
+        else PROF(0, E.pre_phases());
 #else
         {
             Env<real, G, SPEC> e(E);
@@ -3043,7 +3257,8 @@
             PROF(3, e.smooth());
         }
 #endif
-        PROF(4, E.collide());
+        if constexpr (fused_pre<SPEC>) PROF(4, E.collide_narrow());
+        else PROF(4, E.collide());
         PROF(5, E.make_constraints());
         if (RETRY) beyond = beyond || ii[ka->lay.misc + 0] > cap1_con || ii[ka->lay.misc + 1] > cap1_efc;
         PROF(6, E.solve(pgs_iters, ka->m.solver, ka->m.newton_iters, ka->m.newton_tol, ka->m.nscale));
@@ -3061,6 +3276,7 @@
     if (o_prof && lane == 0) {
         for (int k = 0; k < 8; k++) o_prof[(size_t)env * PROF_W + k] = tp[k];
         o_prof[(size_t)env * PROF_W + 8] = E.t_broad; o_prof[(size_t)env * PROF_W + 9] = E.t_narrow;
+        if constexpr (fused_pre<SPEC>) o_prof[(size_t)env * PROF_W + 1] = -1;
         for (int k = 0; k < 16; k++) o_prof[(size_t)env * PROF_W + 10 + k] = ii[ka->lay.nprof + k];
     }
     int nefc_last = ii[ka->lay.misc + 1];
@@ -3110,6 +3326,8 @@
         o_cdist[(size_t)env * expcon + c] = c < ncon ? (double)r[ka->lay.cdist + c] : 0.0;
     }
     }
+    if constexpr (keep_near<SPEC>)
+        if (lane == 0) { ka->m.nearv_glob[2 * (size_t)env] = ii[ka->lay.misc + 6]; ka->m.nearv_glob[2 * (size_t)env + 1] = ii[ka->lay.misc + 7]; }
     if (lane == 0 && o_cost && nsub > 0) o_cost[env] = (int)((__builtin_readcyclecounter() - t_launch) >> 6);
     if (lane == 0 && !o_xpose) {
         o_ncon[env] = ncon;
@@ -3437,16 +3655,18 @@
     void make_layout_of(Layout& L, const int maxcon, const int maxefc, int nq, int nv, int nu, int nb, int ng, int msize, int ntree) {
         kargs_dirty = true;
         L = avs::make_layout_of(maxcon, maxefc, this->maxcon, this->maxefc, nq, nv, nu, nb, ng, msize, ntree, f64 ? 8 : 4);
+        const int pb = L.rowS + RS_S * maxefc > L.scr + NARROW_SCR_W ? L.rowS + RS_S * maxefc : L.scr + NARROW_SCR_W;
+        if (L.cfrc + 6 * nb > pb) throw std::runtime_error("avsim layout: phase A of the scratch union outgrows phase B (bytes_per_env would change)");
         if (getenv("AVSIM_DEBUG_LAYOUT")) {
-            const int pb = L.rowS + RS_S * maxefc > L.scr + NARROW_SCR_W ? L.rowS + RS_S * maxefc : L.scr + NARROW_SCR_W;
             fprintf(stderr, "avsim layout: %d reals + %d ints = %d B per env (U at %d: phase A %d, phase B %d words); tables %zu B\n", L.nreal, L.nint,
-                    L.bytes_per_env, L.U, 38 * nb, pb - L.U, (size_t)moff.nreal * (f64 ? 8 : 4) + (size_t)moff.nint * 4);
+                    L.bytes_per_env, L.U, 32 * nb + 6 * nv, pb - L.U, (size_t)moff.nreal * (f64 ? 8 : 4) + (size_t)moff.nint * 4);
         }
     }
 
     int dims[7] = {0, 0, 0, 0, 0, 0, 0};
     size_t lds_bytes() const { return (size_t)lay.bytes_per_env + (size_t)moff.nreal * (f64 ? 8 : 4) + (size_t)moff.nint * 4; }
-    DevBuf rows, coup, near, gref;
+    DevBuf rows, coup, near, gref, nearv;
+    bool nearv_live = false;
     void alloc_contacts() {
         if (host_only) return;
         if (rows.alloc((size_t)N * maxefc * ROW_S * (f64 ? 8 : 4) * 2) != hipSuccess) throw std::runtime_error("hipMalloc of the constraint row buffers failed");
@@ -3457,6 +3677,10 @@
         mf.bxo_glob = mf.gref_glob + (size_t)N * dims[4] * 3; md.bxo_glob = md.gref_glob + (size_t)N * dims[4] * 3;
         if (coup.alloc((size_t)N * lay2.maxgrp * GA_W * (f64 ? 8 : 4)) != hipSuccess || near.alloc((size_t)N * (NEAR_MAX + CAND_MAX) * 4) != hipSuccess)
             throw std::runtime_error("hipMalloc of the coupling / neighbour buffers failed");
+        if (nearv.alloc((size_t)N * 2 * sizeof(int)) != hipSuccess) throw std::runtime_error("hipMalloc of the neighbour lists' valid flags failed");
+        (void)hipMemset(nearv.ptr(), 0, (size_t)N * 2 * sizeof(int));
+        nearv_live = false;
+        mf.nearv_glob = md.nearv_glob = nearv.as<int>();
         int* const d_near = near.as<int>();
         mf.gA_glob = coup.as<float>(); md.gA_glob = coup.as<double>(); mf.near_glob = d_near; md.near_glob = d_near; mf.cand_glob = md.cand_glob = d_near + (size_t)N * NEAR_MAX;
         kargs_dirty = true;
@@ -3589,6 +3813,11 @@
         const int per_cu = (int)((160 * 1024) / shmem) > 0 ? (int)((160 * 1024) / shmem) : 1;
         int nblk = num_cu * per_cu * (persist_over > 0 ? persist_over : 1);
         if (nblk > (N + wpb - 1) / wpb) nblk = (N + wpb - 1) / wpb;
+        if (nearv_live && (kargs_dirty || !kspec)) {
+            (void)hipMemsetAsync(nearv.ptr(), 0, (size_t)N * 2 * sizeof(int), st);
+            nearv_live = false;
+        }
+        if (kspec) nearv_live = true;
         if (kargs_dirty) {
             KArgs<real> ka{m, lay, moff}, ka2{m, lay2, moff};
             if (kargs.reserve(sizeof(KArgs<double>)) != hipSuccess || kargs2.reserve(sizeof(KArgs<double>)) != hipSuccess) { err = "hipMalloc(kernel arguments) failed"; return -3; }
diff --git a/av_aloha_amd/csrc/avsim_phys_layout.h b/av_aloha_amd/csrc/avsim_phys_layout.h
--- a/av_aloha_amd/csrc/avsim_phys_layout.h
+++ b/av_aloha_amd/csrc/avsim_phys_layout.h
@@ -65,7 +65,7 @@
 
 struct Layout {
     int qpos, qvel, ctrl, warm, xpos, xmat, xipos, cdof, gcen, M, L, Minv, bias, fsm, asm_, qacc, fcon, nH, ng, ndl, njv, U, nreal;
-    int cinert, cvel, cacc, cfrc, binert;
+    int cinert, cvel, cdd, cfrc, binert;
     int cdist, cpos, cnrm, rowS, scr;
     int cand, cpair, cefc, rmeta, rowI, gI, misc, nprof, nint;
     int maxgrp;
@@ -94,7 +94,7 @@
     }
     L.U = o;
     int a = o;
-    L.cinert = a; a += 10 * nb; L.binert = a; a += 10 * nb; L.cvel = a; a += 6 * nb; L.cacc = a; a += 6 * nb; L.cfrc = a; a += 6 * nb;
+    L.cinert = a; a += 10 * nb; L.binert = a; a += 10 * nb; L.cvel = a; a += 6 * nb; L.cdd = a; a += 6 * nv; L.cfrc = a; a += 6 * nb;
     int bq = o;
     L.cdist = bq; bq += maxcon; L.cpos = bq; bq += 3 * maxcon; L.cnrm = bq; bq += 3 * maxcon;
     bq = (bq + 3) & ~3; L.rowS = bq; L.scr = bq; bq += RS_S * maxefc;
```

Measured after the change: 1.052 million, median of 6. About the same (+0.9%).
